# zju3dv/LoG

Hardware: NVIDIA H100
Metric: gaussians_per_s_fwd_bwd (higher is better)
Workload: dtype f32

## Files before the change

include/log_b200_raster.h:

```cpp
#ifndef LOG_B200_RASTER_H
#define LOG_B200_RASTER_H

#include <stdint.h>

#ifdef __cplusplus
extern "C" {
#endif

#define LGR_ABI_VERSION 23
#define LGR_TILE 16

#define LGR_FILTER_ADD 0
#define LGR_FILTER_MAX 1
#define LGR_FILTER_NONE 2

#define LGR_E_BADARG (-1)
#define LGR_E_CAPACITY (-2)
#define LGR_E_UNSUPPORTED (-3)

typedef struct lgr_view {
  int32_t image_height, image_width;
  float tanfovx, tanfovy;
  float scale_modifier;
  int32_t sh_degree;
  int32_t sh_coeffs;
  int32_t filter_mode;
  int32_t want_aux;
  int32_t tile_row_begin, tile_row_end;
  int32_t num_owners;
  int32_t raw_params;
  int32_t* band_ids_d;
  int32_t* band_blk_d;
  int32_t* band_count_d;
  int32_t* band_rows_d;
  float* band_dsplat_d;
  int32_t* tile_rank_d;
  const int64_t* gather_index_d;
  const int32_t* pid_map_d;
  int32_t* contrib_id_d;
  uint32_t* contrib_entry_d;
  int32_t* contrib_count_d;
  const int32_t* last_contrib_d;
  const int32_t* region_count_d;
  int64_t region_cap;
  int32_t num_regions;
  int32_t num_channels;
  int32_t log_depth;
  float* splat_ext_d;
  const float* cov3D_precomp_d;
  float* dcov3D_d;
  const float* viewmatrix_d;
  const float* projmatrix_d;
  const float* campos_d;
  const float* bg_d;
} lgr_view;

#define LGR_SPLAT_FLOATS 12
#define LGR_GRAD_FLOATS 12
#define LGR_TILE_SCRATCH_INTS 33
#define LGR_CONTRIB_MAX_LIST (1 << 24)
#define LGR_META_INTS 8

int lgr_abi_version(void);

int lgr_compute_radius(int64_t n, const float* means3D_d, const float* scales_d, const float* rotations_d,
                       const float* projmatrix_d, const float* viewmatrix_d, float focal_x, float focal_y,
                       float tan_fovx, float tan_fovy, float* radii_d, void* stream);

int lgr_mark_visible(int64_t n, const float* means3D_d, const float* viewmatrix_d, uint8_t* visible_d, void* stream);

int lgr_forward_project(const lgr_view* view, int64_t n, const float* means3D_d, const float* opacities_d,
                        const float* scales_d, const float* rotations_d, const float* colors_precomp_d,
                        const float* shs_d, float* splat_d, int32_t* radii_d, uint8_t* clamped_d,
                        int32_t* tile_start_d, int32_t* tile_cursor_d, int32_t* meta_d, void* stream);

int lgr_forward_render(const lgr_view* view, int64_t n, int64_t num_instances, int32_t max_tile_len,
                       int32_t num_long_tiles, const float* splat_d, const int32_t* radii_d, const int32_t* tile_start_d,
                       int32_t* tile_cursor_d, uint32_t* inst_key_d, uint32_t* inst_val_d, uint32_t* inst_tmp_d,
                       int32_t* sorted_ids_d, float* image_d, float* final_T_d, int32_t* n_contrib_d,
                       int32_t* point_id_pixel_d, float* point_weight_pixel_d, float* point_weight_d,
                       int32_t* point_count_d, void* stream);
int32_t lgr_sort_smem_capacity(void);

int lgr_forward_render_device_sized(const lgr_view* view, int64_t n, int64_t instance_capacity, int32_t* meta_d,
                                    const float* splat_d, const int32_t* radii_d, int32_t* tile_start_d,
                                    int32_t* tile_cursor_d, uint32_t* inst_key_d, uint32_t* inst_val_d,
                                    int32_t* sorted_ids_d, float* image_d, float* final_T_d, int32_t* n_contrib_d,
                                    int32_t* point_id_pixel_d, float* point_weight_pixel_d, float* point_weight_d,
                                    int32_t* point_count_d, void* stream);

int lgr_backward(const lgr_view* view, int64_t n, int64_t num_instances, const float* means3D_d,
                 const float* opacities_d, const float* scales_d, const float* rotations_d,
                 const float* colors_precomp_d, const float* shs_d, const float* splat_d, const int32_t* radii_d,
                 const uint8_t* clamped_d, const int32_t* tile_start_d, const int32_t* sorted_ids_d,
                 const float* image_d, const float* dL_dimage_d, float* dsplat_d,
                 float* dmeans3D_d, float* dmeans2D_d, float* dopacities_d, float* dscales_d, float* drotations_d,
                 float* dcolors_d, float* dshs_d, float* grad_rows_d, void* const* peer_stage_d, int32_t my_rank,
                 int64_t num_rows, void* stream);

#define LGR_STAGE_HEADER_FLOATS 64
#define LGR_ROW_FLOATS 20
#define LGR_OWNER_CHUNK(n, r) ((((n) + (r) - 1) / (r) + 255) / 256 * 256)
int lgr_grad_scatter_add(int64_t num_rows, const float* rows_d, int64_t lo, int64_t hi, float* shard_d, void* stream);
int lgr_grad_scatter_add_staged(const float* stage_d, int32_t num_sources, int64_t owner_chunk, int64_t lo, int64_t hi,
                                float* shard_d, void* stream);

typedef struct lgr_shard_layout {
  int32_t num_ranks, my_rank;
  int64_t cap;
  int64_t off_count, off_splat, off_radii, off_gid, off_dsplat, off_weight, off_pcount;
} lgr_shard_layout;
#define LGR_SHARD_MAX_RANKS 32
#define LGR_SHARD_SEND_INTS(n_local, r) (2 * (int64_t)(r) * ((((n_local) > 0 ? (n_local) : 1) + 255) / 256) + (r))

int lgr_shard_send(const lgr_view* view, const lgr_shard_layout* layout, int64_t n_local, int64_t gid_base,
                   const float* splat_d, const int32_t* radii_d, int32_t* send_scratch_d, void* const* peer_base_d,
                   void* stream);

int lgr_shard_recv_bin(const lgr_view* view, const lgr_shard_layout* layout, float* exchange_d, float* dsplat_d,
                       int32_t* tile_start_d, int32_t* tile_cursor_d, int32_t* meta_d, void* stream);

int lgr_blend_backward(const lgr_view* view, int64_t n, int64_t num_instances, const float* splat_d,
                       const int32_t* tile_start_d, const int32_t* sorted_ids_d, const float* image_d,
                       const float* dL_dimage_d, float* dsplat_d, void* stream);

int lgr_shard_return_rows(const lgr_shard_layout* layout, const float* exchange_d, int64_t total_rows, const void* rows_d,
                          int32_t row_floats, int64_t dst_offset_floats, void* const* peer_base_d, void* stream);

int lgr_shard_gather(const lgr_view* view, const lgr_shard_layout* layout, int64_t n_local, const float* splat_d,
                     const int32_t* radii_d, const int32_t* send_scratch_d, const float* exchange_d,
                     float* dsplat_local_d, float* point_weight_d, int32_t* point_count_d, void* stream);

int lgr_shard_recv_bin_aux(const lgr_view* view, const lgr_shard_layout* layout, float* exchange_d, float* dsplat_d,
                           int32_t* tile_start_d, int32_t* tile_cursor_d, int32_t* meta_d, float* point_weight_rows_d,
                           int32_t* point_count_rows_d, void* stream);
int lgr_shard_return_packed(const lgr_shard_layout* layout, const float* exchange_d, const float* dsplat_rows_d,
                            const float* point_weight_rows_d, const int32_t* point_count_rows_d, void* const* peer_base_d,
                            void* stream);
int lgr_shard_gather_packed(const lgr_view* view, const lgr_shard_layout* layout, int64_t n_local, const float* splat_d,
                            const int32_t* radii_d, const int32_t* send_scratch_d, const float* exchange_d,
                            float* dsplat_local_d, float* point_weight_d, int32_t* point_count_d, void* stream);

typedef struct lgr_tree {
  int64_t num_points, num_nodes;
  int32_t max_child, max_level;
  const int32_t* node_index_d;
  const int32_t* tree_d;
} lgr_tree;
#define LGR_TREE_SCRATCH_INTS(p, s) (8 + 2 * (int64_t)(p) + (int64_t)(s) + 2 * (((int64_t)(s) + 255) / 256) + 2 + ((int64_t)(s) + 3) / 4)
int lgr_tree_traverse(const lgr_tree* tree, const float* xyz_d, const float* scaling_raw_d, const float* rotation_raw_d,
                      const float* projmatrix_d, const float* viewmatrix_d, float focal_x, float focal_y, float tan_fovx,
                      float tan_fovy, const int64_t* root_index_d, int64_t num_roots, float min_resolution_pixel,
                      int32_t max_depth, int32_t* scratch_d, int64_t* index_out_d, int64_t* count_out_d, void* stream);

typedef struct lgr_prepare {
  int64_t num_points, num_roots;
  const float* xyz_d;
  const float* full_proj_d;
  float bound_lo, bound_hi;
  const int32_t* root_index_d;
  const int32_t* node_index_d;
  const int8_t* depth_d;
  int32_t opt_all_levels, current_depth;
  uint8_t* flag_d;
  int64_t* in_range_d;
  int64_t* roots_d;
  int64_t* index_all_d, *leaf_d, *node_d;
  int64_t* result_d;
  int32_t* scratch_d;
} lgr_prepare;
// ... 106 lines not shown
```

log_b200/_capi.py:

```python
import ctypes
import os

from .build import LIB_PATH

_i32, _i64, _f32, _vp = ctypes.c_int32, ctypes.c_int64, ctypes.c_float, ctypes.c_void_p

LGR_FILTER_ADD, LGR_FILTER_MAX, LGR_FILTER_NONE = 0, 1, 2
LGR_SPLAT_FLOATS = 12
LGR_GRAD_FLOATS = 12
LGR_META_INTS = 8
LGR_TILE_SCRATCH_INTS = 33
LGR_ABI_VERSION = 23
LGR_CONTRIB_MAX_LIST = 1 << 24
LGR_STAGE_HEADER_FLOATS = 64
LGR_ROW_FLOATS = 20

EXPORTS = ('lgr_abi_version', 'lgr_sort_smem_capacity', 'lgr_compute_radius', 'lgr_forward_project',
           'lgr_forward_render', 'lgr_forward_render_device_sized', 'lgr_backward', 'lgr_grad_scatter_add', 'lgr_grad_scatter_add_staged', 'lgr_point_compact', 'lgr_sparse_adam', 'lgr_profile_enable', 'lgr_profile_collect',
           'lgr_profile_kernel_name', 'lgr_shard_send', 'lgr_shard_recv_bin', 'lgr_blend_backward', 'lgr_shard_return_rows',
           'lgr_shard_gather', 'lgr_shard_recv_bin_aux', 'lgr_shard_return_packed', 'lgr_shard_gather_packed', 'lgr_tree_traverse', 'lgr_mark_visible',
           'lgr_ssim_forward', 'lgr_ssim_backward', 'lgr_depth_loss_forward', 'lgr_depth_loss_backward', 'lgr_depth_vis',
           'lgr_counter_update', 'lgr_log_step', 'lgr_prepare_cull', 'lgr_prepare_select')
LGR_SHARD_MAX_RANKS = 32
LGR_PROFILE_KERNELS = 12


class LgrView(ctypes.Structure):
    _fields_ = [('image_height', _i32), ('image_width', _i32), ('tanfovx', _f32), ('tanfovy', _f32),
                ('scale_modifier', _f32), ('sh_degree', _i32), ('sh_coeffs', _i32), ('filter_mode', _i32),
                ('want_aux', _i32), ('tile_row_begin', _i32), ('tile_row_end', _i32),
                ('num_owners', _i32), ('raw_params', _i32), ('band_ids_d', _vp), ('band_blk_d', _vp), ('band_count_d', _vp), ('band_rows_d', _vp), ('band_dsplat_d', _vp), ('tile_rank_d', _vp), ('gather_index_d', _vp), ('pid_map_d', _vp), ('contrib_id_d', _vp), ('contrib_entry_d', _vp), ('contrib_count_d', _vp), ('last_contrib_d', _vp),
                ('region_count_d', _vp), ('region_cap', _i64), ('num_regions', _i32), ('num_channels', _i32), ('log_depth', _i32), ('splat_ext_d', _vp), ('cov3D_precomp_d', _vp), ('dcov3D_d', _vp),
                ('viewmatrix_d', _vp), ('projmatrix_d', _vp), ('campos_d', _vp), ('bg_d', _vp)]


class LgrShardLayout(ctypes.Structure):
    _fields_ = [('num_ranks', _i32), ('my_rank', _i32), ('cap', _i64), ('off_count', _i64), ('off_splat', _i64),
                ('off_radii', _i64), ('off_gid', _i64), ('off_dsplat', _i64), ('off_weight', _i64), ('off_pcount', _i64)]


class LgrTree(ctypes.Structure):
    _fields_ = [('num_points', _i64), ('num_nodes', _i64), ('max_child', _i32), ('max_level', _i32),
                ('node_index_d', _vp), ('tree_d', _vp)]


def tree_scratch_ints(num_points, slots):
    return 8 + 2 * num_points + slots + 2 * ((slots + 255) // 256) + 2 + (slots + 3) // 4


class LgrPrepare(ctypes.Structure):
    _fields_ = [('num_points', _i64), ('num_roots', _i64), ('xyz_d', _vp), ('full_proj_d', _vp), ('bound_lo', _f32),
                ('bound_hi', _f32), ('root_index_d', _vp), ('node_index_d', _vp), ('depth_d', _vp), ('opt_all_levels', _i32),
                ('current_depth', _i32), ('flag_d', _vp), ('in_range_d', _vp), ('roots_d', _vp), ('index_all_d', _vp),
                ('leaf_d', _vp), ('node_d', _vp), ('result_d', _vp), ('scratch_d', _vp)]


LGR_PREPARE_RESULTS = 8
(LGR_PREPARE_IN_RANGE, LGR_PREPARE_ROOTS, LGR_PREPARE_WALK, LGR_PREPARE_LEAVES, LGR_PREPARE_NODES, LGR_PREPARE_STATUS,
 LGR_PREPARE_INSTANCES, LGR_PREPARE_OVERFLOW) = range(8)
LGR_PREPARE_ROOT_ORDER = 1


def prepare_scratch_ints(num_points, slots):
    return 2 * num_points + 2 * ((num_points + 255) // 256) + 2 + (num_points + 3) // 4 + tree_scratch_ints(num_points, slots)


LGR_SSIM_WINDOW = 11
LGR_SSIM_TILE = 32


def ssim_scratch_doubles(b, c, h, w):
    return b * c * ((h - LGR_SSIM_WINDOW + LGR_SSIM_TILE) // LGR_SSIM_TILE) * ((w - LGR_SSIM_WINDOW + LGR_SSIM_TILE) // LGR_SSIM_TILE)


def ssim_map_floats(b, c, h, w):
    return 3 * b * c * (h - LGR_SSIM_WINDOW + 1) * (w - LGR_SSIM_WINDOW + 1)


LGR_DEPTH_PATCHES = 64
LGR_DEPTH_PATCH = 64
LGR_DEPTH_STAT_DOUBLES_PER_PATCH = 8
LGR_DEPTH_STAT_DOUBLES = LGR_DEPTH_STAT_DOUBLES_PER_PATCH * LGR_DEPTH_PATCHES + 8
LGR_DEPTH_GRAD_SCRATCH_FLOATS = LGR_DEPTH_PATCHES * LGR_DEPTH_PATCH * LGR_DEPTH_PATCH
LGR_DEPTH_VIS_GRID = 264
LGR_DEPTH_VIS_SCRATCH_FLOATS = 2 * LGR_DEPTH_VIS_GRID


def shard_send_ints(n_local, r):
    return 2 * r * ((max(n_local, 1) + 255) // 256) + r


class LgrCounter(ctypes.Structure):
    _fields_ = [('create_steps_d', _vp), ('visible_count_d', _vp), ('weights_max_d', _vp), ('weights_sum_d', _vp),
                ('radii_max_d', _vp), ('area_sum_d', _vp), ('grad_sum_d', _vp), ('radii_max_max_d', _vp)]


LGR_STEP_MAX_KEYS = 8


class LgrStepKey(ctypes.Structure):
    _fields_ = [('param_d', _vp), ('exp_avg_d', _vp), ('exp_avg_sq_d', _vp), ('max_exp_avg_sq_d', _vp), ('grad_d', _vp),
                ('row_floats', _i32), ('prefix', _i32), ('neg_step_size', _f32), ('bc2_sqrt', _f32), ('clamp', _i32)]


class LgrStep(ctypes.Structure):
    _fields_ = [('keys', LgrStepKey * LGR_STEP_MAX_KEYS), ('num_keys', _i32), ('row_floats', _i32), ('beta1', _f32),
                ('beta2', _f32), ('one_minus_beta1', _f32), ('one_minus_beta2', _f32), ('eps', _f32),
                ('radius3d_min_d', _vp), ('radius3d_max_d', _vp)]


class LgrError(RuntimeError):
    pass


_lib = None


def bind(lib):
    lib.lgr_abi_version.restype = ctypes.c_int
    lib.lgr_sort_smem_capacity.restype = _i32
    lib.lgr_mark_visible.restype = ctypes.c_int
    lib.lgr_mark_visible.argtypes = [_i64, _vp, _vp, _vp, _vp]
    lib.lgr_compute_radius.restype = ctypes.c_int
    lib.lgr_compute_radius.argtypes = [_i64, _vp, _vp, _vp, _vp, _vp, _f32, _f32, _f32, _f32, _vp, _vp]
    lib.lgr_forward_project.restype = ctypes.c_int
    lib.lgr_forward_project.argtypes = [ctypes.POINTER(LgrView), _i64] + [_vp] * 13
    lib.lgr_forward_render.restype = ctypes.c_int
    lib.lgr_forward_render.argtypes = [ctypes.POINTER(LgrView), _i64, _i64, _i32, _i32] + [_vp] * 16
    lib.lgr_forward_render_device_sized.restype = ctypes.c_int
    lib.lgr_forward_render_device_sized.argtypes = [ctypes.POINTER(LgrView), _i64, _i64] + [_vp] * 16
    lib.lgr_sparse_adam.restype = ctypes.c_int
    lib.lgr_sparse_adam.argtypes = [_i64, _i32, _vp, _vp, _vp, _vp, _vp, _vp, _i64, ctypes.c_double, ctypes.c_double,
                                    ctypes.c_double, ctypes.c_double, _vp]
    lib.lgr_point_compact.restype = ctypes.c_int
    lib.lgr_point_compact.argtypes = [_i64, _vp, _vp, _vp, _vp, _vp, _vp]
    lib.lgr_backward.restype = ctypes.c_int
    lib.lgr_backward.argtypes = [ctypes.POINTER(LgrView), _i64, _i64] + [_vp] * 23 + [_i32, _i64, _vp]
    lib.lgr_grad_scatter_add_staged.restype = ctypes.c_int
    lib.lgr_grad_scatter_add_staged.argtypes = [_vp, _i32, _i64, _i64, _i64, _vp, _vp]
    lib.lgr_grad_scatter_add.restype = ctypes.c_int
    lib.lgr_grad_scatter_add.argtypes = [_i64, _vp, _i64, _i64, _vp, _vp]
    lay = ctypes.POINTER(LgrShardLayout)
    lib.lgr_shard_send.restype = ctypes.c_int
    lib.lgr_shard_send.argtypes = [ctypes.POINTER(LgrView), lay, _i64, _i64, _vp, _vp, _vp, _vp, _vp]
    lib.lgr_shard_recv_bin.restype = ctypes.c_int
    lib.lgr_shard_recv_bin.argtypes = [ctypes.POINTER(LgrView), lay, _vp, _vp, _vp, _vp, _vp, _vp]
    lib.lgr_blend_backward.restype = ctypes.c_int
    lib.lgr_blend_backward.argtypes = [ctypes.POINTER(LgrView), _i64, _i64, _vp, _vp, _vp, _vp, _vp, _vp, _vp]
    lib.lgr_shard_return_rows.restype = ctypes.c_int
    lib.lgr_shard_return_rows.argtypes = [lay, _vp, _i64, _vp, _i32, _i64, _vp, _vp]
    lib.lgr_shard_gather.restype = ctypes.c_int
    lib.lgr_shard_gather.argtypes = [ctypes.POINTER(LgrView), lay, _i64, _vp, _vp, _vp, _vp, _vp, _vp, _vp, _vp]
    lib.lgr_shard_recv_bin_aux.restype = ctypes.c_int
    lib.lgr_shard_recv_bin_aux.argtypes = [ctypes.POINTER(LgrView), lay, _vp, _vp, _vp, _vp, _vp, _vp, _vp, _vp]
    lib.lgr_shard_return_packed.restype = ctypes.c_int
    lib.lgr_shard_return_packed.argtypes = [lay, _vp, _vp, _vp, _vp, _vp, _vp]
    lib.lgr_shard_gather_packed.restype = ctypes.c_int
    lib.lgr_shard_gather_packed.argtypes = [ctypes.POINTER(LgrView), lay, _i64, _vp, _vp, _vp, _vp, _vp, _vp, _vp, _vp]
    lib.lgr_tree_traverse.restype = ctypes.c_int
    lib.lgr_tree_traverse.argtypes = [ctypes.POINTER(LgrTree), _vp, _vp, _vp, _vp, _vp, _f32, _f32, _f32, _f32, _vp, _i64, _f32,
                                      _i32, _vp, _vp, _vp, _vp]
    lib.lgr_prepare_cull.restype = ctypes.c_int
    lib.lgr_prepare_cull.argtypes = [ctypes.POINTER(LgrPrepare), _vp]
    lib.lgr_prepare_select.restype = ctypes.c_int
    lib.lgr_prepare_select.argtypes = [ctypes.POINTER(LgrPrepare), ctypes.POINTER(LgrTree), _vp, _vp, _vp, _vp, _f32, _f32, _f32, _f32,
                                       _f32, _i32, _vp, _vp, _vp]
    lib.lgr_ssim_forward.restype = ctypes.c_int
    lib.lgr_ssim_forward.argtypes = [_i32, _i32, _i32, _i32, _vp, _vp, _vp, _vp, _vp, _vp, _vp, _vp]
    lib.lgr_ssim_backward.restype = ctypes.c_int
    lib.lgr_ssim_backward.argtypes = [_i32, _i32, _i32, _i32, _vp, _vp, _vp, _vp, _vp, _vp, _vp, _vp]
    lib.lgr_depth_loss_forward.restype = ctypes.c_int
    lib.lgr_depth_loss_forward.argtypes = [_i32, _i32, _i32, _i32] + [_vp] * 11
    lib.lgr_depth_loss_backward.restype = ctypes.c_int
    lib.lgr_depth_loss_backward.argtypes = [_i32, _i32, _i32, _i32] + [_vp] * 13
    lib.lgr_depth_vis.restype = ctypes.c_int
    lib.lgr_depth_vis.argtypes = [_i32, _i32] + [_vp] * 7
    lib.lgr_counter_update.restype = ctypes.c_int
    lib.lgr_counter_update.argtypes = [ctypes.POINTER(LgrCounter), _i64, _i64] + [_vp] * 6 + [_i64, _vp, _vp, _i32, _i32,
                                                                                              _vp, _vp]
    lib.lgr_log_step.restype = ctypes.c_int
    lib.lgr_log_step.argtypes = [ctypes.POINTER(LgrStep), _i64, _i64, _vp, _vp, _vp, _vp]
    lib.lgr_profile_enable.restype = ctypes.c_int
    lib.lgr_profile_enable.argtypes = [ctypes.c_int]
    lib.lgr_profile_collect.restype = ctypes.c_int
    lib.lgr_profile_collect.argtypes = [_vp, _vp, _i32]
    lib.lgr_profile_kernel_name.restype = ctypes.c_char_p
    lib.lgr_profile_kernel_name.argtypes = [ctypes.c_int]
    return lib


def load():
    global _lib
    if _lib is not None:
        return _lib
    if not os.path.exists(LIB_PATH):
        raise LgrError(f'{LIB_PATH} not found: run `python -m log_b200.build` (or __graft_entry__.build()). '
                       'log_b200 has no CPU fallback.')
    lib = bind(ctypes.CDLL(LIB_PATH))
    if lib.lgr_abi_version() != LGR_ABI_VERSION:
        raise LgrError('liblog_b200_raster.so ABI version mismatch: rebuild with `python -m log_b200.build --force`')
    _lib = lib
    return lib


def current_stream(device=None):
    import torch
    return ctypes.c_void_p(torch.cuda.current_stream(device).cuda_stream)


def require_cuda(t, name):
    if not t.is_cuda:
        raise LgrError(f'{name} is on {t.device}: log_b200 rasterises on CUDA only (no CPU fallback)')

# ... 25 lines not shown
```

log_b200/csrc/lgr_bin.cu:

```cuda
#include "lgr_common.cuh"
#include "lgr_prof.cuh"

namespace lgr {

constexpr int SCAN_THREADS = 1024;
constexpr int SORT_CAP_SMALL_FWD = 4096;

__global__ void __launch_bounds__(SCAN_THREADS)
tile_scan_kernel(int ntiles, int32_t* __restrict__ tile_start ,
                 int32_t* __restrict__ cursor ,
                 int32_t* __restrict__ meta, int small_cap, int ranked) {
  __shared__ int warp_sum[SCAN_THREADS / 32];
  __shared__ int carry_s, maxl_s, nbig_s;
  const int tid = threadIdx.x, lane = tid & 31, wid = tid >> 5;
  if (tid == 0) { carry_s = 0; maxl_s = 0; nbig_s = 0; }
  __syncthreads();
  int local_max = 0;
  for (int base = 0; base < ntiles; base += SCAN_THREADS) {
    const int i = base + tid;
    const int c = (i < ntiles) ? cursor[i * CSTRIDE] + cursor[i * CSTRIDE + 1] : 0;
    local_max = max(local_max, c);
    int x = c;
#pragma unroll
    for (int o = 1; o < 32; o <<= 1) { const int y = __shfl_up_sync(0xffffffffu, x, o); if (lane >= o) x += y; }
    if (lane == 31) warp_sum[wid] = x;
    __syncthreads();
    if (wid == 0) {
      int w = warp_sum[lane];
#pragma unroll
      for (int o = 1; o < 32; o <<= 1) { const int y = __shfl_up_sync(0xffffffffu, w, o); if (lane >= o) w += y; }
      warp_sum[lane] = w;
    }
    __syncthreads();
    const int carry = carry_s;
    const int excl = carry + (wid ? warp_sum[wid - 1] : 0) + x - c;
    if (i < ntiles) {
      tile_start[i] = excl; cursor[i * CSTRIDE + ranked] = 0;
      if (c > small_cap) cursor[CSTRIDE * ntiles + atomicAdd(&nbig_s, 1)] = i;
    }
    __syncthreads();
    if (tid == SCAN_THREADS - 1) carry_s = carry + warp_sum[31];
    __syncthreads();
  }
#pragma unroll
  for (int o = 16; o > 0; o >>= 1) local_max = max(local_max, __shfl_xor_sync(0xffffffffu, local_max, o));
  if (lane == 0) atomicMax(&maxl_s, local_max);
  __syncthreads();
  if (tid == 0) { tile_start[ntiles] = carry_s; meta[0] = carry_s; meta[1] = maxl_s; meta[5] = nbig_s; }
}

constexpr int SCATTER_THREADS = 256;

__global__ void __launch_bounds__(SCATTER_THREADS)
bin_scatter_kernel(View v, int64_t n, const float* __restrict__ splat, const int32_t* __restrict__ radii,
                   const int32_t* __restrict__ tile_start, int32_t* __restrict__ cursor, uint32_t* __restrict__ inst_key,
                   uint32_t* __restrict__ inst_val, int64_t capacity ) {
  __shared__ int64_t s_first[LGR_SHARD_MAX_RANKS + 1];
  const int64_t total = v.region_count ? region_setup(v, s_first) : n;
  for (int64_t base = (int64_t)blockIdx.x * SCATTER_THREADS; base < total; base += (int64_t)gridDim.x * SCATTER_THREADS) {
  int64_t i = base + threadIdx.x;
  bool live = i < total;
  if (live && v.region_count) i = region_row(v, s_first, i);
  if (live && v.num_owners > 0) {
    const int b = (int)(i / 256), sl = (int)(i % 256);
    if (sl >= v.band_blk[b]) live = false;
    else {
      const int id = v.band_ids[i];
      v.band_rows[v.band_blk[v.band_blocks + b] + sl] = id;
      if (v.band_dsplat) {
        float4* z = reinterpret_cast<float4*>(v.band_dsplat + (int64_t)id * LGR_GRAD_FLOATS);
        z[0] = z[1] = z[2] = make_float4(0.f, 0.f, 0.f, 0.f);
      }
      i = id;
    }
  }
  int rad = 0;
  float4 r0 = make_float4(0.f, 0.f, 0.f, 0.f), r1 = r0;
  float depth = 0.f;
  int4 rk = make_int4(-1, -1, -1, -1);
  if (live) {
    rad = radii[i];
    r0 = ldg4(splat + i * LGR_SPLAT_FLOATS);
    r1 = ldg4(splat + i * LGR_SPLAT_FLOATS + 4);
    depth = __ldg(splat + i * LGR_SPLAT_FLOATS + 11);
    if (v.tile_rank) rk = __ldg(reinterpret_cast<const int4*>(v.tile_rank + 4 * i));
    live = rad > 0;
  }
  if (live && v.num_owners == 0 && v.band_dsplat) {
    float4* z = reinterpret_cast<float4*>(v.band_dsplat + i * LGR_GRAD_FLOATS);
    z[0] = z[1] = z[2] = make_float4(0.f, 0.f, 0.f, 0.f);
  }
  int x0 = 0, y0 = 0, x1 = 0, y1 = 0;
  uint32_t key = 0;
  if (live) {
    live = r1.z > 0.f;
    if (live) {
      key = __float_as_uint(depth);
      tile_rect_tight(r0.x, r0.y, rad, r1.z, r1.w, v.gx, v.gy, v.row0, v.row1, x0, y0, x1, y1);
    }
  }
  const int w = x1 - x0, cnt = live ? w * (y1 - y0) : 0;
  if (cnt > 0 && cnt <= 4) {
    int t[4], slot[4];
#pragma unroll
    for (int k = 0; k < 4; k++) {
      const int ty = y0 + k / max(w, 1), tx = x0 + k % max(w, 1);
      t[k] = k < cnt ? (ty - v.row0) * v.gx + tx : -1;
    }
    if (v.tile_rank) {
      slot[0] = rk.x; slot[1] = rk.y; slot[2] = rk.z; slot[3] = rk.w;
    } else {
#pragma unroll
      for (int k = 0; k < 4; k++) slot[k] = t[k] >= 0 ? atomicAdd(cursor + t[k] * CSTRIDE, 1) : 0;
    }
#pragma unroll
    for (int k = 0; k < 4; k++)
      if (t[k] >= 0) {
        const int pos = __ldg(tile_start + t[k]) + slot[k];
        if (pos < capacity) { inst_key[pos] = key; inst_val[pos] = (uint32_t)i; }
      }
  }
  const int lane = threadIdx.x & 31, big = v.tile_rank ? 1 : 0;
  unsigned todo = __ballot_sync(0xffffffffu, cnt > 4);
  while (todo) {
    const int src = __ffs(todo) - 1;
    todo &= todo - 1;
    const int bx0 = __shfl_sync(0xffffffffu, x0, src), by0 = __shfl_sync(0xffffffffu, y0, src);
    const int bw = __shfl_sync(0xffffffffu, w, src), bcnt = __shfl_sync(0xffffffffu, cnt, src);
    const uint32_t bkey = __shfl_sync(0xffffffffu, key, src);
    const uint32_t bid = (uint32_t)__shfl_sync(0xffffffffu, (int)i, src);
    for (int k = lane; k < bcnt; k += 32) {
      const int t = (by0 + k / bw - v.row0) * v.gx + bx0 + k % bw;
      const int pos = tile_start[t] + (big ? cursor[t * CSTRIDE] : 0) + atomicAdd(cursor + t * CSTRIDE + big, 1);
      if (pos < capacity) { inst_key[pos] = bkey; inst_val[pos] = bid; }
    }
  }
  }
}

constexpr int SORT_THREADS = 256;
constexpr int SORT_WARPS = SORT_THREADS / 32;
constexpr int RADIX_BITS = 8;
constexpr int RADIX = 1 << RADIX_BITS;
constexpr int SORT_CAP_SMALL = SORT_CAP_SMALL_FWD;
constexpr int SORT_CAP_LARGE = 13312;

__device__ __forceinline__ bool radix_pass(const uint32_t* __restrict__ kin, const uint32_t* __restrict__ vin,
                                           uint32_t* __restrict__ kout, uint32_t* __restrict__ vout, int len, int shift,
                                           bool on_val, int* __restrict__ whist) {
  const int tid = threadIdx.x, lane = tid & 31, wid = tid >> 5;
  const int seg = ((len + SORT_WARPS * 32 - 1) / (SORT_WARPS * 32)) * 32;
  const int beg = min(len, wid * seg), end = min(len, beg + seg);
  for (int j = tid; j < SORT_WARPS * RADIX; j += SORT_THREADS) whist[j] = 0;
  __syncthreads();
  int* myh = whist + wid * RADIX;
  for (int i = beg + lane; i < end; i += 32) {
    const uint32_t d = ((on_val ? vin[i] : kin[i]) >> shift) & (RADIX - 1);
    atomicAdd(myh + d, 1);
  }
  __syncthreads();
  {
    const int d = tid;
    int tot = 0;
#pragma unroll
    for (int w = 0; w < SORT_WARPS; w++) tot += whist[w * RADIX + d];
    int x = tot;
#pragma unroll
    for (int o = 1; o < 32; o <<= 1) { const int y = __shfl_up_sync(0xffffffffu, x, o); if (lane >= o) x += y; }
    __shared__ int wsum[SORT_WARPS];
    if (lane == 31) wsum[wid] = x;
    __syncthreads();
    int base = x - tot;
#pragma unroll
    for (int w = 0; w < SORT_WARPS; w++) if (w < wid) base += wsum[w];
#pragma unroll
    for (int w = 0; w < SORT_WARPS; w++) { const int c = whist[w * RADIX + d]; whist[w * RADIX + d] = base; base += c; }
    if (__syncthreads_or(tot == len)) return true;
  }
  for (int i0 = beg; i0 < end; i0 += 32) {
    const int i = i0 + lane;
    const bool ok = i < end;
    uint32_t k = 0, val = 0;
    if (ok) { k = kin[i]; val = vin[i]; }
    const uint32_t d = ok ? (((on_val ? val : k) >> shift) & (RADIX - 1)) : (RADIX + lane);
    const uint32_t peers = __match_any_sync(0xffffffffu, d);
    const int rank = __popc(peers & ((1u << lane) - 1u));
    int base = 0;
    if (ok) base = myh[d];
    __syncwarp();
    if (ok && rank == 0) myh[d] = base + __popc(peers);
    __syncwarp();
    if (ok) { kout[base + rank] = k; vout[base + rank] = val; }
  }
  __syncthreads();
  return false;
}

__device__ __forceinline__ void sort_tile(uint32_t* kA, uint32_t* vA, uint32_t* kB, uint32_t* vB, int len, int id_bits,
                                          int* whist) {
  uint32_t *ki = kA, *vi = vA, *ko = kB, *vo = vB;
  auto run = [&](int shift, bool on_val) {
    const bool ident = radix_pass(ki, vi, ko, vo, len, shift, on_val, whist);
    if (!ident) { uint32_t* t = ki; ki = ko; ko = t; t = vi; vi = vo; vo = t; }
  };
  for (int s = 0; s < 32; s += RADIX_BITS) run(s, false);
  int my_tie = 0;
  for (int i = threadIdx.x + 1; i < len; i += SORT_THREADS) if (ki[i] == ki[i - 1]) my_tie = 1;
  if (__syncthreads_or(my_tie)) {
    for (int s = 0; s < id_bits; s += RADIX_BITS) run(s, true);
    for (int s = 0; s < 32; s += RADIX_BITS) run(s, false);
  }
  if (ki != kA) {
    for (int i = threadIdx.x; i < len; i += SORT_THREADS) { kA[i] = ki[i]; vA[i] = vi[i]; }
    __syncthreads();
  }
}

#ifndef LGR_ON_LSD_FALLBACK
#define LGR_ON_LSD_FALLBACK()
#endif
constexpr int MSD_SMALL = 96;
constexpr int MSD_STACK = 512;

struct MsdShared {
  int hist[RADIX];
  int bstart[RADIX + 1];
  alignas(16) int wsum[SORT_WARPS];
  unsigned long long wmin[SORT_WARPS], wmax[SORT_WARPS];
  int stack_beg[MSD_STACK], stack_len[MSD_STACK];
  int top, shift, overflow;
};

__device__ __forceinline__ unsigned long long composite(uint32_t k, uint32_t v) { return ((unsigned long long)k << 32) | v; }

__device__ __forceinline__ bool sort_tile_msd(uint32_t* kA, uint32_t* vA, uint32_t* kB, uint32_t* vB, int len, MsdShared& sh) {
  const int tid = threadIdx.x, lane = tid & 31, wid = tid >> 5;
  if (tid == 0) { sh.stack_beg[0] = 0; sh.stack_len[0] = len; sh.top = 1; sh.overflow = 0; }
  __syncthreads();
  while (true) {
    const int top = sh.top;
    if (top == 0 || sh.overflow) break;
    const int beg = sh.stack_beg[top - 1], n = sh.stack_len[top - 1];
    __syncthreads();
    if (tid == 0) sh.top = top - 1;
    unsigned long long mn = ~0ull, mx = 0ull;
    for (int i = tid; i < n; i += SORT_THREADS) {
      const unsigned long long c = composite(kA[beg + i], vA[beg + i]);
      mn = min(mn, c); mx = max(mx, c);
    }
#pragma unroll
    for (int o = 16; o > 0; o >>= 1) {
      mn = min(mn, __shfl_xor_sync(0xffffffffu, mn, o));
      mx = max(mx, __shfl_xor_sync(0xffffffffu, mx, o));
    }
    if (lane == 0) { sh.wmin[wid] = mn; sh.wmax[wid] = mx; }
    sh.hist[tid] = 0;
    __syncthreads();
    if (tid == 0) {
      unsigned long long a = sh.wmin[0], b = sh.wmax[0];
#pragma unroll
      for (int w = 1; w < SORT_WARPS; w++) { a = min(a, sh.wmin[w]); b = max(b, sh.wmax[w]); }
      const int hb = 63 - __clzll((long long)(a ^ b));
      sh.shift = max(0, hb - (RADIX_BITS - 1));
    }
    __syncthreads();
    const int shift = sh.shift;
    for (int i = tid; i < n; i += SORT_THREADS)
      atomicAdd(&sh.hist[(int)((composite(kA[beg + i], vA[beg + i]) >> shift) & (RADIX - 1))], 1);
    __syncthreads();
    {
      const int c = sh.hist[tid];
      int x = c;
#pragma unroll
      for (int o = 1; o < 32; o <<= 1) { const int y = __shfl_up_sync(0xffffffffu, x, o); if (lane >= o) x += y; }
      if (lane == 31) sh.wsum[wid] = x;
      __syncthreads();
      int base = x - c;
#pragma unroll
      for (int w = 0; w < SORT_WARPS; w++) if (w < wid) base += sh.wsum[w];
      sh.bstart[tid] = base;
      sh.hist[tid] = base;
      if (tid == RADIX - 1) sh.bstart[RADIX] = base + c;
    }
    __syncthreads();
    for (int i = tid; i < n; i += SORT_THREADS) {
      const uint32_t k = kA[beg + i], v = vA[beg + i];
      const int slot = atomicAdd(&sh.hist[(int)((composite(k, v) >> shift) & (RADIX - 1))], 1);
      kB[beg + slot] = k; vB[beg + slot] = v;
    }
    __syncthreads();
    for (int i = tid; i < n; i += SORT_THREADS) {
      const uint32_t k = kB[beg + i], v = vB[beg + i];
      const int d = (int)((composite(k, v) >> shift) & (RADIX - 1));
      const int b0 = sh.bstart[d], bn = sh.bstart[d + 1] - b0;
      int dst = i;
      if (bn <= MSD_SMALL) {
        const uint32_t* kb = kB + beg + b0;
        const uint32_t* vb = vB + beg + b0;
        int rank = 0, eq = 0;
#pragma unroll 8
        for (int j = 0; j < bn; j++) {
          const uint32_t kj = kb[j];
          rank += (kj < k) ? 1 : 0;
          eq += (kj == k) ? 1 : 0;
        }
        if (eq > 1)
          for (int j = 0; j < bn; j++) rank += (kb[j] == k && vb[j] < v) ? 1 : 0;
        dst = b0 + rank;
      }
      kA[beg + dst] = k; vA[beg + dst] = v;
    }
    {
      const int b0 = sh.bstart[tid], bn = sh.bstart[tid + 1] - b0;
      if (bn > MSD_SMALL) {
        const int slot = atomicAdd(&sh.top, 1);
        if (slot < MSD_STACK) { sh.stack_beg[slot] = beg + b0; sh.stack_len[slot] = bn; }
// ... 50 lines not shown
  if ((int64_t)meta[0] <= capacity) return;
  for (int i = blockIdx.x * 256 + threadIdx.x; i <= ntiles; i += gridDim.x * 256) tile_start[i] = 0;
  if (blockIdx.x == 0 && threadIdx.x == 0) atomicOr(meta + 6, 1);
}


int sort_smem_capacity() { return SORT_CAP_LARGE; }

constexpr int PC_THREADS = 1024;

__global__ void __launch_bounds__(PC_THREADS)
pc_block_count_kernel(int64_t n, const int32_t* __restrict__ count, int32_t* __restrict__ blk) {
  const int64_t i = (int64_t)blockIdx.x * PC_THREADS + threadIdx.x;
  const int c = __syncthreads_count(i < n && count[i] > 0);
  if (threadIdx.x == 0) blk[blockIdx.x] = c;
}

__global__ void __launch_bounds__(1024)
pc_scan_kernel(int nb, int32_t* __restrict__ blk , int32_t* __restrict__ num_out) {
  __shared__ int warp_sum[32];
  __shared__ int carry_s;
  const int tid = threadIdx.x, lane = tid & 31, wid = tid >> 5;
  if (tid == 0) carry_s = 0;
  __syncthreads();
  for (int base = 0; base < nb; base += 1024) {
    const int b = base + tid;
    const int c = b < nb ? blk[b] : 0;
    int x = c;
#pragma unroll
    for (int o = 1; o < 32; o <<= 1) { const int y = __shfl_up_sync(0xffffffffu, x, o); if (lane >= o) x += y; }
    if (lane == 31) warp_sum[wid] = x;
    __syncthreads();
    if (wid == 0) {
      int w = warp_sum[lane];
#pragma unroll
      for (int o = 1; o < 32; o <<= 1) { const int y = __shfl_up_sync(0xffffffffu, w, o); if (lane >= o) w += y; }
      warp_sum[lane] = w;
    }
    __syncthreads();
    const int carry = carry_s;
    if (b < nb) blk[nb + b] = carry + (wid ? warp_sum[wid - 1] : 0) + x - c;
    __syncthreads();
    if (tid == 1023) carry_s = carry + warp_sum[31];
    __syncthreads();
  }
  if (tid == 0) { blk[2 * nb] = carry_s; *num_out = carry_s; }
}

__global__ void __launch_bounds__(PC_THREADS)
pc_compact_kernel(int64_t n, const int32_t* __restrict__ count, const int32_t* __restrict__ blk, int nb,
                  int32_t* __restrict__ ids_out, int32_t* __restrict__ counts_out) {
  __shared__ int wsum[PC_THREADS / 32];
  const int64_t i = (int64_t)blockIdx.x * PC_THREADS + threadIdx.x;
  const int lane = threadIdx.x & 31, wid = threadIdx.x >> 5;
  const int c = i < n ? count[i] : 0;
  const unsigned bal = __ballot_sync(0xffffffffu, c > 0);
  if (lane == 0) wsum[wid] = __popc(bal);
  __syncthreads();
  int base = blk[nb + blockIdx.x];
  for (int w = 0; w < wid; w++) base += wsum[w];
  if (c > 0) {
    const int pos = base + __popc(bal & ((1u << lane) - 1u));
    ids_out[pos] = (int32_t)i;
    counts_out[pos] = c;
  }
}

int launch_point_compact(int64_t n, const int32_t* count, int32_t* blk, int32_t* ids_out, int32_t* counts_out, int32_t* num_out,
                         cudaStream_t st) {
  const int nb = (int)((n + PC_THREADS - 1) / PC_THREADS);
  if (nb == 0) {
    cudaError_t e = cudaMemsetAsync(num_out, 0, sizeof(int32_t), st);
    return e == cudaSuccess ? 0 : (int)e;
  }
  pc_block_count_kernel<<<nb, PC_THREADS, 0, st>>>(n, count, blk);
  LGR_CHECK_LAUNCH();
  pc_scan_kernel<<<1, 1024, 0, st>>>(nb, blk, num_out);
  LGR_CHECK_LAUNCH();
  pc_compact_kernel<<<nb, PC_THREADS, 0, st>>>(n, count, blk, nb, ids_out, counts_out);
  LGR_CHECK_LAUNCH();
  return 0;
}

int launch_tile_scan(int ntiles, int32_t* tile_start, int32_t* cursor, int32_t* meta, bool ranked, cudaStream_t st) {
  ProfScope ps(K_TILE_SCAN, st);
  tile_scan_kernel<<<1, SCAN_THREADS, 0, st>>>(ntiles, tile_start, cursor, meta, SORT_CAP_SMALL_FWD, ranked ? 1 : 0);
  LGR_CHECK_LAUNCH();
  return 0;
}

constexpr int LONG_SORT_GRID = 132;

int launch_bin_and_sort(const View& v, int64_t n, int64_t num_inst, int max_len, int num_long, const float* splat,
                        const int32_t* radii, int32_t* tile_start, int32_t* cursor, uint32_t* inst_key,
                        uint32_t* inst_val, uint32_t* inst_tmp, int32_t* sorted_ids, int32_t* meta_dev, cudaStream_t st) {
  if (n == 0) return 0;
  if (meta_dev) {
    const int nt = v.gx * (v.row1 - v.row0);
    clamp_lists_kernel<<<(nt + 256) / 256, 256, 0, st>>>(nt, num_inst, tile_start, meta_dev);
    LGR_CHECK_LAUNCH();
  }
  if (num_inst == 0 && v.num_owners == 0 && v.band_dsplat == nullptr) return 0;
  const int ntiles = v.gx * (v.row1 - v.row0);
  unsigned blocks = (unsigned)((n + SCATTER_THREADS - 1) / SCATTER_THREADS);
  if (v.region_count && blocks > (unsigned)LGR_REGION_GRID) blocks = (unsigned)LGR_REGION_GRID;
  {
    ProfScope ps(K_BIN_SCATTER, st);
    bin_scatter_kernel<<<blocks, SCATTER_THREADS, 0, st>>>(v, n, splat, radii, tile_start, cursor, inst_key, inst_val,
                                                           meta_dev ? num_inst : (int64_t)0x7fffffffffffffffLL);
  }
  LGR_CHECK_LAUNCH();
  if (num_inst == 0) return 0;
  int id_bits = 8;
  while (id_bits < 32 && (n - 1) >> id_bits) id_bits += 8;
  {
    cudaError_t e = cudaFuncSetAttribute(tile_sort_kernel<0>, cudaFuncAttributeMaxDynamicSharedMemorySize, 16 * SORT_CAP_LARGE);
    if (e != cudaSuccess) return (int)e;
  }
  if (meta_dev) {
    ProfScope ps(K_TILE_SORT, st, 2);
    tile_sort_kernel<0><<<ntiles, SORT_THREADS, 16 * SORT_CAP_SMALL, st>>>(nullptr, tile_start, inst_key, inst_val, inst_tmp, sorted_ids, 0, SORT_CAP_SMALL, id_bits, nullptr, nullptr);
    LGR_CHECK_LAUNCH();
    const int32_t* long_list = cursor + CSTRIDE * ntiles;
    tile_sort_kernel<0><<<LONG_SORT_GRID, SORT_THREADS, 16 * SORT_CAP_LARGE, st>>>(long_list, tile_start, inst_key, inst_val, inst_tmp, sorted_ids, SORT_CAP_SMALL, SORT_CAP_LARGE, id_bits, meta_dev + 5, meta_dev + 6);
    LGR_CHECK_LAUNCH();
    return 0;
  }
  ProfScope ps(K_TILE_SORT, st, 1 + (num_long > 0) + (max_len > SORT_CAP_LARGE));
  const int cap_main = max(256, min(max_len, SORT_CAP_SMALL));
  tile_sort_kernel<0><<<ntiles, SORT_THREADS, 16 * cap_main, st>>>(nullptr, tile_start, inst_key, inst_val, inst_tmp, sorted_ids, 0, cap_main, id_bits, nullptr, nullptr);
  LGR_CHECK_LAUNCH();
  if (num_long > 0) {
    const int32_t* long_list = cursor + CSTRIDE * ntiles;
    const int cap = min(max_len, SORT_CAP_LARGE);
    tile_sort_kernel<0><<<num_long, SORT_THREADS, 16 * cap, st>>>(long_list, tile_start, inst_key, inst_val, inst_tmp, sorted_ids, SORT_CAP_SMALL, cap, id_bits, nullptr, nullptr);
    LGR_CHECK_LAUNCH();
    if (max_len > SORT_CAP_LARGE) {
      if (!inst_tmp) return LGR_E_CAPACITY;
      tile_sort_kernel<1><<<num_long, SORT_THREADS, 0, st>>>(long_list, tile_start, inst_key, inst_val, inst_tmp, sorted_ids, SORT_CAP_LARGE, 0, id_bits, nullptr, nullptr);
      LGR_CHECK_LAUNCH();
    }
  }
  return 0;
}

}
```

log_b200/csrc/lgr_capi.cu:

```cuda
#include "lgr_common.cuh"
#include "lgr_prof.cuh"
#include <math.h>

namespace lgr {
int launch_mark_visible(int64_t, const float*, const float*, uint8_t*, cudaStream_t);
int launch_compute_radius(int64_t, const float*, const float*, const float*, const float*, const float*, float, float,
                          float, float, float*, cudaStream_t);
int launch_project_fwd(const View&, Colour, bool, int64_t, const float*, const float*, const float*, const float*,
                       const float*, const float*, float*, int32_t*, uint8_t*, int32_t*, int32_t*, cudaStream_t);
int launch_project_bwd(const View&, Colour, bool, bool, int64_t, const float*, const float*, const float*, const float*,
                       const float*, const int32_t*, const uint8_t*, const float*, float*, float*, float*, float*, float*,
                       float*, float*, float*, void* const*, int, cudaStream_t);
int launch_grad_scatter_add(int64_t, const float*, int64_t, int64_t, float*, cudaStream_t);
int launch_grad_scatter_add_staged(const float*, int, int64_t, int64_t, int64_t, float*, cudaStream_t);
int launch_band_scan(const View&, cudaStream_t);
int launch_tile_scan(int, int32_t*, int32_t*, int32_t*, bool, cudaStream_t);
int launch_bin_and_sort(const View&, int64_t, int64_t, int, int, const float*, const int32_t*, int32_t*, int32_t*,
                        uint32_t*, uint32_t*, uint32_t*, int32_t*, int32_t*, cudaStream_t);
int sort_smem_capacity();
int launch_blend_fwd(const View&, const int32_t*, const int32_t*, const float*, float*, float*, int32_t*, int32_t*,
                     float*, float*, int32_t*, cudaStream_t);
int launch_sparse_adam(int64_t, int, const int64_t*, const float*, float*, float*, float*, float*, float, float, float, float,
                       float, float, float, cudaStream_t);
int launch_counter_update(const lgr_counter&, int64_t, int64_t, const int64_t*, const int64_t*, const int32_t*, const float*,
// ... 40 lines not shown
                            v->gather_index_d))
    return false;
  const int lists = (v->contrib_id_d != nullptr) + (v->contrib_entry_d != nullptr) + (v->contrib_count_d != nullptr);
  if (lists != 0 && lists != 3) return false;
  if (v->num_channels != 0 && v->num_channels != 3 && v->num_channels != 6) return false;
  if (v->num_channels == 6 && !v->splat_ext_d) return false;
  if (v->log_depth != 0 && (v->log_depth != 1 || v->num_channels != 6)) return false;
  return true;
}

static int six_channels_check(const lgr_view* v) {
  if (v->num_channels != 6) return 0;
  if (v->num_owners > 0 || v->region_count_d || v->pid_map_d) return LGR_E_UNSUPPORTED;
  if (!v->log_depth && (v->raw_params || v->gather_index_d)) return LGR_E_UNSUPPORTED;
  return 0;
}

static int colour_source(const lgr_view* v, int64_t n, const float* colors_precomp_d, const float* shs_d, Colour* c) {
  const bool six_precomp = v->num_channels == 6 && !v->log_depth;
  if (six_precomp && shs_d) return LGR_E_UNSUPPORTED;
  const bool log_sh = v->raw_params && colors_precomp_d && shs_d;
  if (!log_sh && (colors_precomp_d != nullptr) == (shs_d != nullptr) && n > 0) return LGR_E_BADARG;
  *c = log_sh ? Colour::LOG_SH : shs_d ? Colour::SH : six_precomp ? Colour::RGB6 : Colour::RGB;
  return 0;
}

extern "C" {

int lgr_abi_version(void) { return LGR_ABI_VERSION; }

int32_t lgr_sort_smem_capacity(void) { return sort_smem_capacity(); }

int lgr_compute_radius(int64_t n, const float* means3D_d, const float* scales_d, const float* rotations_d,
                       const float* projmatrix_d, const float* viewmatrix_d, float focal_x, float focal_y,
                       float tan_fovx, float tan_fovy, float* radii_d, void* stream) {
  if (n < 0 || (n > 0 && (!means3D_d || !scales_d || !rotations_d || !radii_d)) || !projmatrix_d || !viewmatrix_d)
    return LGR_E_BADARG;
  return launch_compute_radius(n, means3D_d, scales_d, rotations_d, projmatrix_d, viewmatrix_d, focal_x, focal_y,
                               tan_fovx, tan_fovy, radii_d, (cudaStream_t)stream);
}

int lgr_mark_visible(int64_t n, const float* means3D_d, const float* viewmatrix_d, uint8_t* visible_d, void* stream) {
  if (n < 0 || !viewmatrix_d || (n > 0 && (!means3D_d || !visible_d))) return LGR_E_BADARG;
  return launch_mark_visible(n, means3D_d, viewmatrix_d, visible_d, (cudaStream_t)stream);
}

int lgr_forward_project(const lgr_view* view, int64_t n, const float* means3D_d, const float* opacities_d,
                        const float* scales_d, const float* rotations_d, const float* colors_precomp_d,
                        const float* shs_d, float* splat_d, int32_t* radii_d, uint8_t* clamped_d,
                        int32_t* tile_start_d, int32_t* tile_cursor_d, int32_t* meta_d, void* stream) {
  if (!view_ok(view) || n < 0 || !tile_start_d || !tile_cursor_d || !meta_d) return LGR_E_BADARG;
  if (const int rc6 = six_channels_check(view)) return rc6;
  Colour c;
  if (const int rc = colour_source(view, n, colors_precomp_d, shs_d, &c)) return rc;
  if (view->raw_params && c == Colour::SH) return LGR_E_UNSUPPORTED;
  if (c == Colour::LOG_SH) {
    if (!view->campos_d) return LGR_E_BADARG;
    if (view->sh_degree < 0 || view->sh_degree > 3) return LGR_E_UNSUPPORTED;
    if (view->sh_coeffs < (view->sh_degree + 1) * (view->sh_degree + 1) - 1) return LGR_E_BADARG;
    if (view->num_owners > 0) return LGR_E_UNSUPPORTED;
  } else if (c == Colour::SH) {
    if (!view->campos_d || !clamped_d) return LGR_E_BADARG;
    if (view->sh_degree < 0 || view->sh_degree > 3) return LGR_E_UNSUPPORTED;
    if (view->sh_coeffs < (view->sh_degree + 1) * (view->sh_degree + 1)) return LGR_E_BADARG;
  }
  const bool cov3d = view->cov3D_precomp_d != nullptr;
  if (n > 0 && (!means3D_d || !opacities_d || (!cov3d && (!scales_d || !rotations_d)) || !splat_d || !radii_d)) return LGR_E_BADARG;
  if (cov3d && (view->raw_params || view->num_owners > 0)) return LGR_E_UNSUPPORTED;
  if (n > 0x7fffffffLL) return LGR_E_UNSUPPORTED;
  cudaStream_t st = (cudaStream_t)stream;
  const View v = make_view(view, n);
  const int ntiles = v.gx * (v.row1 - v.row0);
  if (v.num_owners > 0 && shs_d) return LGR_E_UNSUPPORTED;
  if (c == Colour::LOG_SH && view->sh_degree == 0) c = Colour::RGB;
  cudaError_t e = cudaMemsetAsync(tile_cursor_d, 0, sizeof(int32_t) * (size_t)ntiles * CSTRIDE, st);
  if (e != cudaSuccess) return (int)e;
  e = cudaMemsetAsync(meta_d, 0, sizeof(int32_t) * LGR_META_INTS, st);
  if (e != cudaSuccess) return (int)e;
  int rc = launch_project_fwd(v, c, cov3d, n, means3D_d, opacities_d, scales_d, rotations_d, colors_precomp_d, shs_d, splat_d,
                              radii_d, clamped_d, tile_cursor_d, meta_d, st);
  if (rc) return rc;
  rc = launch_band_scan(v, st);
  if (rc) return rc;
  return launch_tile_scan(ntiles, tile_start_d, tile_cursor_d, meta_d, view->tile_rank_d != nullptr, st);
}

int lgr_forward_render(const lgr_view* view, int64_t n, int64_t num_instances, int32_t max_tile_len,
                       int32_t num_long_tiles, const float* splat_d, const int32_t* radii_d, const int32_t* tile_start_d,
                       int32_t* tile_cursor_d, uint32_t* inst_key_d, uint32_t* inst_val_d, uint32_t* inst_tmp_d,
                       int32_t* sorted_ids_d, float* image_d, float* final_T_d, int32_t* n_contrib_d,
                       int32_t* point_id_pixel_d, float* point_weight_pixel_d, float* point_weight_d,
                       int32_t* point_count_d, void* stream) {
  if (!view_ok(view) || n < 0 || num_instances < 0 || num_long_tiles < 0 || !tile_start_d || !tile_cursor_d || !image_d || !final_T_d ||
      !n_contrib_d)
    return LGR_E_BADARG;
  if (num_instances > 0 && (!inst_key_d || !inst_val_d || !sorted_ids_d || !splat_d || !radii_d)) return LGR_E_BADARG;
  if (const int rc6 = six_channels_check(view)) return rc6;
  if (view->want_aux && (!point_id_pixel_d || !point_weight_pixel_d || (n > 0 && !point_weight_d))) return LGR_E_BADARG;
  if (num_instances > 0x7fffffffLL) return LGR_E_UNSUPPORTED;
  if (view->contrib_id_d && max_tile_len > LGR_CONTRIB_MAX_LIST) return LGR_E_UNSUPPORTED;
  cudaStream_t st = (cudaStream_t)stream;
  const View v = make_view(view, n);
  int rc = launch_bin_and_sort(v, n, num_instances, max_tile_len, num_long_tiles, splat_d, radii_d, const_cast<int32_t*>(tile_start_d), tile_cursor_d,
                               inst_key_d, inst_val_d, inst_tmp_d, sorted_ids_d, nullptr, st);
  if (rc) return rc;
  return launch_blend_fwd(v, tile_start_d, sorted_ids_d, splat_d, image_d, final_T_d, n_contrib_d, point_id_pixel_d,
                          point_weight_pixel_d, point_weight_d, view->want_aux ? point_count_d : nullptr, st);
}

int lgr_forward_render_device_sized(const lgr_view* view, int64_t n, int64_t instance_capacity, int32_t* meta_d,
                                    const float* splat_d, const int32_t* radii_d, int32_t* tile_start_d,
                                    int32_t* tile_cursor_d, uint32_t* inst_key_d, uint32_t* inst_val_d,
                                    int32_t* sorted_ids_d, float* image_d, float* final_T_d, int32_t* n_contrib_d,
                                    int32_t* point_id_pixel_d, float* point_weight_pixel_d, float* point_weight_d,
                                    int32_t* point_count_d, void* stream) {
  if (!view_ok(view) || n < 0 || instance_capacity <= 0 || !meta_d || !tile_start_d || !tile_cursor_d || !image_d || !final_T_d ||
      !n_contrib_d || !inst_key_d || !inst_val_d || !sorted_ids_d)
    return LGR_E_BADARG;
  if (n > 0 && (!splat_d || !radii_d)) return LGR_E_BADARG;
  if (const int rc6 = six_channels_check(view)) return rc6;
  if (view->want_aux && (!point_id_pixel_d || !point_weight_pixel_d || (n > 0 && !point_weight_d))) return LGR_E_BADARG;
  if (instance_capacity > 0x7fffffffLL) return LGR_E_UNSUPPORTED;
  cudaStream_t st = (cudaStream_t)stream;
  const View v = make_view(view, n);
  int rc = launch_bin_and_sort(v, n, instance_capacity, 0, 0, splat_d, radii_d, tile_start_d, tile_cursor_d, inst_key_d, inst_val_d,
                               nullptr, sorted_ids_d, meta_d, st);
  if (rc) return rc;
  return launch_blend_fwd(v, tile_start_d, sorted_ids_d, splat_d, image_d, final_T_d, n_contrib_d, point_id_pixel_d,
                          point_weight_pixel_d, point_weight_d, view->want_aux ? point_count_d : nullptr, st);
}

int lgr_backward(const lgr_view* view, int64_t n, int64_t num_instances, const float* means3D_d,
                 const float* opacities_d, const float* scales_d, const float* rotations_d,
                 const float* colors_precomp_d, const float* shs_d, const float* splat_d, const int32_t* radii_d,
                 const uint8_t* clamped_d, const int32_t* tile_start_d, const int32_t* sorted_ids_d,
                 const float* image_d, const float* dL_dimage_d, float* dsplat_d,
                 float* dmeans3D_d, float* dmeans2D_d, float* dopacities_d, float* dscales_d, float* drotations_d,
                 float* dcolors_d, float* dshs_d, float* grad_rows_d, void* const* peer_stage_d, int32_t my_rank,
                 int64_t num_rows, void* stream) {
  if (!view_ok(view) || n < 0 || !tile_start_d || !image_d || !dL_dimage_d) return LGR_E_BADARG;
  if (const int rc6 = six_channels_check(view)) return rc6;
  const bool rows_mode = grad_rows_d || peer_stage_d;
  if (view->num_channels == 6 && rows_mode) return LGR_E_UNSUPPORTED;
  Colour c;
  if (const int rc = colour_source(view, n, colors_precomp_d, shs_d, &c)) return rc;
  if (n == 0) return 0;
  if (c == Colour::LOG_SH && (!dshs_d || !view->campos_d || view->num_owners > 0)) return LGR_E_BADARG;
  const bool cov3d = view->cov3D_precomp_d != nullptr;
  if (!means3D_d || (!cov3d && (!scales_d || !rotations_d)) || !splat_d || !radii_d || !dsplat_d) return LGR_E_BADARG;
  if (cov3d && (!view->dcov3D_d || view->raw_params || view->num_owners > 0 || grad_rows_d || peer_stage_d)) return LGR_E_BADARG;
  if (view->raw_params && (!opacities_d || c == Colour::SH)) return LGR_E_BADARG;
  if (rows_mode) {
    if (view->num_owners <= 0 || c == Colour::SH) return LGR_E_BADARG;
    if (peer_stage_d && (my_rank < 0 || my_rank >= view->num_owners)) return LGR_E_BADARG;
    if (num_rows < 0 || num_rows > n) return LGR_E_BADARG;
  } else {
    if (view->num_owners > 0) return LGR_E_BADARG;
    if (!dmeans3D_d || !dmeans2D_d || !dopacities_d || (!cov3d && (!dscales_d || !drotations_d))) return LGR_E_BADARG;
    if (c == Colour::SH ? (!dshs_d || !clamped_d || !view->campos_d) : !dcolors_d) return LGR_E_BADARG;
  }
  if (num_instances > 0 && !sorted_ids_d) return LGR_E_BADARG;
  cudaStream_t st = (cudaStream_t)stream;
  const View v = make_view(view, n);
  int rc = 0;
  if (num_instances > 0) rc = launch_blend_bwd(v, tile_start_d, sorted_ids_d, splat_d, image_d, dL_dimage_d, dsplat_d, st);
  if (rc) return rc;
  return launch_project_bwd(v, c, cov3d, rows_mode, rows_mode ? num_rows : n, means3D_d, opacities_d, scales_d, rotations_d, shs_d, radii_d, clamped_d, dsplat_d,
                            dmeans3D_d, dmeans2D_d, dopacities_d, dscales_d, drotations_d, dcolors_d, dshs_d, grad_rows_d, peer_stage_d, my_rank, st);
}

int lgr_sparse_adam(int64_t rows, int32_t row_floats, const int64_t* index_d, const float* grad_d, float* param_d,
                    float* exp_avg_d, float* exp_avg_sq_d, float* max_exp_avg_sq_d, int64_t step, double lr, double beta1,
                    double beta2, double eps, void* stream) {
  if (rows < 0 || row_floats <= 0 || step < 1) return LGR_E_BADARG;
  if (rows > 0 && (!index_d || !grad_d || !param_d || !exp_avg_d || !exp_avg_sq_d)) return LGR_E_BADARG;
  const double bc1 = 1.0 - pow(beta1, (double)step), bc2 = 1.0 - pow(beta2, (double)step);
  const double step_size = lr / bc1;
  return launch_sparse_adam(rows, row_floats, index_d, grad_d, param_d, exp_avg_d, exp_avg_sq_d, max_exp_avg_sq_d,
                            (float)beta1, (float)beta2, (float)(1.0 - beta1), (float)(1.0 - beta2), (float)sqrt(bc2),
                            (float)(-step_size), (float)eps, (cudaStream_t)stream);
}

int lgr_counter_update(const lgr_counter* counter, int64_t num_leaf, int64_t num_node, const int64_t* index_leaf_d,
                       const int64_t* index_node_d, const int32_t* radii_d, const float* point_weight_d, const float* grad_d,
                       const int64_t* grad_strides, int64_t num_points, const void* point_id_d, const void* point_count_d,
                       int32_t id_bytes, int32_t count_bytes, uint8_t* flag_vis_d, void* stream) {
  if (!counter || num_leaf < 0 || num_node < 0 || num_points < 0 || !grad_strides) return LGR_E_BADARG;
  if ((id_bytes != 4 && id_bytes != 8) || (count_bytes != 4 && count_bytes != 8)) return LGR_E_BADARG;
  if ((num_leaf > 0 && !index_leaf_d) || (num_node > 0 && !index_node_d)) return LGR_E_BADARG;
  const lgr_counter& c = *counter;
  if (!c.create_steps_d || !c.visible_count_d || !c.weights_max_d || !c.weights_sum_d || !c.radii_max_d || !c.area_sum_d ||
      !c.grad_sum_d || !c.radii_max_max_d)
    return LGR_E_BADARG;
  if (num_leaf + num_node > 0 && (!radii_d || !point_weight_d || !flag_vis_d)) return LGR_E_BADARG;
  if (num_points > 0 && (!point_id_d || !point_count_d || !grad_d || grad_strides[0] < 0 || grad_strides[1] < 0))
    return LGR_E_BADARG;
  return launch_counter_update(c, num_leaf, num_node, index_leaf_d, index_node_d, radii_d, point_weight_d, grad_d,
                               grad_strides, num_points, point_id_d, point_count_d, id_bytes, count_bytes, flag_vis_d,
                               (cudaStream_t)stream);
}

int lgr_log_step(const lgr_step* step, int64_t num_leaf, int64_t num_node, const int64_t* index_leaf_d,
                 const int64_t* index_node_d, const uint8_t* flag_vis_d, void* stream) {
  if (!step || num_leaf < 0 || num_node < 0 || step->num_keys < 1 || step->num_keys > LGR_STEP_MAX_KEYS) return LGR_E_BADARG;
  if ((num_leaf > 0 && !index_leaf_d) || (num_node > 0 && !index_node_d) || (num_leaf + num_node > 0 && !flag_vis_d))
    return LGR_E_BADARG;
  int32_t prefix = 0;
  for (int k = 0; k < step->num_keys; k++) {
    const lgr_step_key& key = step->keys[k];
// ... 71 lines not shown
                               (cudaStream_t)stream);
}

int lgr_depth_vis(int32_t height, int32_t width, const float* pred_d, const int64_t* pred_strides, const float* accmap_d,
                  const int64_t* acc_strides, float* scratch_d, float* vis_d, void* stream) {
  if (height < 1 || width < 1 || !pred_d || !pred_strides || !accmap_d || !acc_strides || !scratch_d || !vis_d)
    return LGR_E_BADARG;
  for (int k = 0; k < 2; k++)
    if (pred_strides[k] < 0 || acc_strides[k] < 0) return LGR_E_BADARG;
  return launch_depth_vis(height, width, pred_d, pred_strides, accmap_d, acc_strides, scratch_d, vis_d, (cudaStream_t)stream);
}

int lgr_point_compact(int64_t n, const int32_t* point_count_d, int32_t* scratch_d, int32_t* ids_out_d,
                      int32_t* counts_out_d, int32_t* num_out_d, void* stream) {
  if (n < 0 || !num_out_d || (n > 0 && (!point_count_d || !scratch_d || !ids_out_d || !counts_out_d))) return LGR_E_BADARG;
  return launch_point_compact(n, point_count_d, scratch_d, ids_out_d, counts_out_d, num_out_d, (cudaStream_t)stream);
}

int lgr_grad_scatter_add_staged(const float* stage_d, int32_t num_sources, int64_t owner_chunk, int64_t lo, int64_t hi,
                                float* shard_d, void* stream) {
  if (!stage_d || !shard_d || num_sources <= 0 || owner_chunk <= 0 || hi < lo) return LGR_E_BADARG;
  return launch_grad_scatter_add_staged(stage_d, num_sources, owner_chunk, lo, hi, shard_d, (cudaStream_t)stream);
}

int lgr_grad_scatter_add(int64_t num_rows, const float* rows_d, int64_t lo, int64_t hi, float* shard_d, void* stream) {
  if (num_rows < 0 || hi < lo || (num_rows > 0 && (!rows_d || !shard_d))) return LGR_E_BADARG;
  return launch_grad_scatter_add(num_rows, rows_d, lo, hi, shard_d, (cudaStream_t)stream);
}

static bool layout_ok(const lgr_shard_layout* l) {
  if (!l || l->num_ranks <= 0 || l->num_ranks > LGR_SHARD_MAX_RANKS || l->my_rank < 0 || l->my_rank >= l->num_ranks) return false;
  if (l->cap <= 0 || l->cap % 256) return false;
  const int64_t offs[7] = {l->off_count, l->off_splat, l->off_radii, l->off_gid, l->off_dsplat, l->off_weight, l->off_pcount};
  for (int k = 0; k < 7; k++) if (offs[k] < 0 || offs[k] % 4) return false;
  return true;
}

static ShardLayout make_layout(const lgr_shard_layout* l) {
  ShardLayout o;
  o.R = l->num_ranks; o.me = l->my_rank; o.cap = l->cap;
  o.off_count = l->off_count; o.off_splat = l->off_splat; o.off_radii = l->off_radii; o.off_gid = l->off_gid;
  o.off_dsplat = l->off_dsplat; o.off_weight = l->off_weight; o.off_pcount = l->off_pcount;
  return o;
}

int lgr_shard_send(const lgr_view* view, const lgr_shard_layout* layout, int64_t n_local, int64_t gid_base,
                   const float* splat_d, const int32_t* radii_d, int32_t* send_scratch_d, void* const* peer_base_d,
                   void* stream) {
  if (!view_ok(view) || !layout_ok(layout) || n_local < 0 || gid_base < 0 || !send_scratch_d || !peer_base_d) return LGR_E_BADARG;
  if (view->num_channels == 6) return LGR_E_UNSUPPORTED;
  if (n_local > layout->cap || (n_local > 0 && (!splat_d || !radii_d))) return LGR_E_BADARG;
  if (view->num_owners != 0 || view->tile_row_begin != 0 || (view->tile_row_end != 0 && view->tile_row_end != (view->image_height + TILE - 1) / TILE))
    return LGR_E_BADARG;
  if (gid_base + n_local > 0x7fffffffLL) return LGR_E_UNSUPPORTED;
  return launch_shard_send(make_view(view, n_local), make_layout(layout), n_local, gid_base, splat_d, radii_d, send_scratch_d,
                           peer_base_d, (cudaStream_t)stream);
}

int lgr_shard_recv_bin(const lgr_view* view, const lgr_shard_layout* layout, float* exchange_d, float* dsplat_d,
                       int32_t* tile_start_d, int32_t* tile_cursor_d, int32_t* meta_d, void* stream) {
  return lgr_shard_recv_bin_aux(view, layout, exchange_d, dsplat_d, tile_start_d, tile_cursor_d, meta_d, nullptr, nullptr, stream);
}

int lgr_shard_recv_bin_aux(const lgr_view* view, const lgr_shard_layout* layout, float* exchange_d, float* dsplat_d,
                           int32_t* tile_start_d, int32_t* tile_cursor_d, int32_t* meta_d, float* point_weight_rows_d,
                           int32_t* point_count_rows_d, void* stream) {
  if (!view_ok(view) || !layout_ok(layout) || !exchange_d || !dsplat_d || !tile_start_d || !tile_cursor_d || !meta_d) return LGR_E_BADARG;
  if (view->num_channels == 6) return LGR_E_UNSUPPORTED;
  if (view->num_owners != 0) return LGR_E_BADARG;
  if (view->region_count_d != reinterpret_cast<const int32_t*>(exchange_d + layout->off_count) || view->region_cap != layout->cap ||
      view->num_regions != layout->num_ranks)
    return LGR_E_BADARG;
  if ((int64_t)layout->num_ranks * layout->cap > 0x7fffffffLL) return LGR_E_UNSUPPORTED;
  cudaStream_t st = (cudaStream_t)stream;
  const View v = make_view(view, (int64_t)layout->num_ranks * layout->cap);
  const int ntiles = v.gx * (v.row1 - v.row0);
  cudaError_t e = cudaMemsetAsync(tile_cursor_d, 0, sizeof(int32_t) * (size_t)(ntiles > 0 ? ntiles : 1) * CSTRIDE, st);
  if (e != cudaSuccess) return (int)e;
  e = cudaMemsetAsync(meta_d, 0, sizeof(int32_t) * LGR_META_INTS, st);
  if (e != cudaSuccess) return (int)e;
  int rc = launch_shard_recv_count(v, make_layout(layout), exchange_d, dsplat_d, tile_cursor_d, meta_d, point_weight_rows_d,
                                   point_count_rows_d, st);
  if (rc) return rc;
  return launch_tile_scan(ntiles, tile_start_d, tile_cursor_d, meta_d, view->tile_rank_d != nullptr, st);
}

int lgr_blend_backward(const lgr_view* view, int64_t n, int64_t num_instances, const float* splat_d,
                       const int32_t* tile_start_d, const int32_t* sorted_ids_d, const float* image_d,
                       const float* dL_dimage_d, float* dsplat_d, void* stream) {
  if (!view_ok(view) || n < 0 || num_instances < 0 || !tile_start_d || !image_d || !dL_dimage_d) return LGR_E_BADARG;
  if (const int rc6 = six_channels_check(view)) return rc6;
  if (num_instances == 0 || n == 0) return 0;
  if (!splat_d || !sorted_ids_d || !dsplat_d) return LGR_E_BADARG;
  return launch_blend_bwd(make_view(view, n), tile_start_d, sorted_ids_d, splat_d, image_d, dL_dimage_d, dsplat_d,
                          (cudaStream_t)stream);
}

int lgr_shard_return_rows(const lgr_shard_layout* layout, const float* exchange_d, int64_t total_rows, const void* rows_d,
                          int32_t row_floats, int64_t dst_offset_floats, void* const* peer_base_d, void* stream) {
  if (!layout_ok(layout) || !exchange_d || !peer_base_d || total_rows < 0 || row_floats <= 0) return LGR_E_BADARG;
  if (dst_offset_floats < 0 || dst_offset_floats % 4 || (total_rows > 0 && !rows_d)) return LGR_E_BADARG;
  return launch_shard_return(make_layout(layout), exchange_d, total_rows, rows_d, row_floats, dst_offset_floats, peer_base_d,
                             (cudaStream_t)stream);
}

int lgr_shard_gather(const lgr_view* view, const lgr_shard_layout* layout, int64_t n_local, const float* splat_d,
                     const int32_t* radii_d, const int32_t* send_scratch_d, const float* exchange_d,
                     float* dsplat_local_d, float* point_weight_d, int32_t* point_count_d, void* stream) {
  if (!view_ok(view) || !layout_ok(layout) || n_local < 0 || n_local > layout->cap) return LGR_E_BADARG;
  if (view->num_channels == 6) return LGR_E_UNSUPPORTED;
  if (n_local == 0) return 0;
  if (!splat_d || !radii_d || !send_scratch_d || !exchange_d || !dsplat_local_d) return LGR_E_BADARG;
  return launch_shard_gather(make_view(view, n_local), make_layout(layout), n_local, splat_d, radii_d, send_scratch_d, exchange_d,
                             dsplat_local_d, point_weight_d, point_count_d, 0, (cudaStream_t)stream);
}

int lgr_shard_gather_packed(const lgr_view* view, const lgr_shard_layout* layout, int64_t n_local, const float* splat_d,
                            const int32_t* radii_d, const int32_t* send_scratch_d, const float* exchange_d,
                            float* dsplat_local_d, float* point_weight_d, int32_t* point_count_d, void* stream) {
  if (!view_ok(view) || !layout_ok(layout) || n_local < 0 || n_local > layout->cap) return LGR_E_BADARG;
  if (view->num_channels == 6) return LGR_E_UNSUPPORTED;
  if (n_local == 0) return 0;
  if (!splat_d || !radii_d || !send_scratch_d || !exchange_d || !dsplat_local_d) return LGR_E_BADARG;
  return launch_shard_gather(make_view(view, n_local), make_layout(layout), n_local, splat_d, radii_d, send_scratch_d, exchange_d,
                             dsplat_local_d, point_weight_d, point_count_d, 1, (cudaStream_t)stream);
}

int lgr_shard_return_packed(const lgr_shard_layout* layout, const float* exchange_d, const float* dsplat_rows_d,
                            const float* point_weight_rows_d, const int32_t* point_count_rows_d, void* const* peer_base_d,
                            void* stream) {
  if (!layout_ok(layout) || !exchange_d || !dsplat_rows_d || !peer_base_d) return LGR_E_BADARG;
  return launch_shard_return_packed(make_layout(layout), exchange_d, dsplat_rows_d, point_weight_rows_d, point_count_rows_d,
                                    peer_base_d, (cudaStream_t)stream);
}

int lgr_tree_traverse(const lgr_tree* tree, const float* xyz_d, const float* scaling_raw_d, const float* rotation_raw_d,
                      const float* projmatrix_d, const float* viewmatrix_d, float focal_x, float focal_y, float tan_fovx,
                      float tan_fovy, const int64_t* root_index_d, int64_t num_roots, float min_resolution_pixel,
                      int32_t max_depth, int32_t* scratch_d, int64_t* index_out_d, int64_t* count_out_d, void* stream) {
  if (!tree || tree->num_points < 0 || tree->num_nodes < 0 || tree->max_child <= 0 || tree->max_level < 0) return LGR_E_BADARG;
  if (num_roots < 0 || num_roots > tree->num_points || max_depth < 0 || !scratch_d || !count_out_d) return LGR_E_BADARG;
  if (!projmatrix_d || !viewmatrix_d) return LGR_E_BADARG;
  if (tree->num_points > 0 && (!tree->node_index_d || !xyz_d || !scaling_raw_d || !rotation_raw_d || !index_out_d)) return LGR_E_BADARG;
  if (tree->num_nodes > 0 && !tree->tree_d) return LGR_E_BADARG;
  if (num_roots > 0 && !root_index_d) return LGR_E_BADARG;
  if (tree->num_points > 0x7fffffffLL || tree->num_nodes * tree->max_child > 0x7fffffffLL) return LGR_E_UNSUPPORTED;
  TreeArgs a;
  a.node_index = tree->node_index_d; a.tree = tree->tree_d; a.C = tree->max_child;
  a.xyz = xyz_d; a.scaling_raw = scaling_raw_d; a.rotation_raw = rotation_raw_d; a.view = viewmatrix_d; a.proj = projmatrix_d;
  a.fx = focal_x; a.fy = focal_y; a.tanfovx = tan_fovx; a.tanfovy = tan_fovy; a.min_px = min_resolution_pixel;
  const int levels = tree->max_level < max_depth ? tree->max_level : max_depth;
  return launch_tree_traverse(a, tree->num_points, tree->num_nodes, root_index_d, num_roots, nullptr, levels, scratch_d, index_out_d,
                              count_out_d, (cudaStream_t)stream);
}

static bool prepare_ok(const lgr_prepare* p) {
  if (!p || p->num_points < 0 || p->num_roots < 0 || p->num_roots > p->num_points || !p->result_d) return false;
  if (p->num_points > 0 && (!p->xyz_d || !p->full_proj_d || !p->flag_d || !p->in_range_d || !p->scratch_d)) return false;
  if (p->num_roots > 0 && !p->root_index_d) return false;
  return true;
}

int lgr_prepare_cull(const lgr_prepare* prep, void* stream) {
  if (!prepare_ok(prep)) return LGR_E_BADARG;
  if (prep->num_points > 0x7fffffffLL) return LGR_E_UNSUPPORTED;
  return launch_prepare_cull(*prep, (cudaStream_t)stream);
}
// ... 53 lines not shown
```

log_b200/csrc/lgr_common.cuh:

```cuda
#pragma once
#include <cuda_runtime.h>
#include <stdint.h>

#include "../../include/log_b200_raster.h"

namespace lgr {

constexpr int TILE = LGR_TILE;
constexpr int TILE_PIX = TILE * TILE;
constexpr float NEAR_Z = 0.2f;
constexpr float ALPHA_MAX = 0.99f;
constexpr float ALPHA_MIN = 1.0f / 255.0f;
constexpr float T_STOP = 1e-4f;
constexpr float FILTER_VAR = 0.3f;
constexpr float CLAMP_FOV = 1.3f;
constexpr int CSTRIDE = 32;
constexpr float LOG2E = 1.4426950408889634f;
constexpr float LN2 = 0.6931471805599453f;

enum class Colour { RGB, SH, LOG_SH, RGB6 };

struct View {
  int H, W, gx, gy;
  int row0, row1;
  float tanfovx, tanfovy, fx, fy, scale_mod;
  int sh_degree, sh_K, filter_mode, want_aux;
  int raw_params;
  int num_owners, owner_chunk;
  int32_t* band_ids;
  int32_t* band_blk;
  int32_t* band_count;
  int32_t* band_rows;
  float* band_dsplat;
  int32_t* tile_rank;
  const int64_t* gather;
  const int32_t* pid_map;
  int32_t* contrib_id;
  uint32_t* contrib_entry;
  int32_t* contrib_count;
  const int32_t* last_contrib;
  const int32_t* region_count;
  int64_t region_cap;
  int regions;
  const float* cov3d;
  float* dcov3d;
  int band_blocks;
  const float* view;
  const float* proj;
  const float* campos;
  const float* bg;
  int num_channels;
  int log_depth;
  float* splat_ext;
};

inline View make_view(const lgr_view* v, int64_t n = 0) {
  View o;
  o.num_owners = v->num_owners; o.band_ids = v->band_ids_d; o.band_blk = v->band_blk_d; o.band_count = v->band_count_d; o.band_rows = v->band_rows_d; o.band_dsplat = v->band_dsplat_d; o.tile_rank = v->tile_rank_d; o.gather = v->gather_index_d; o.pid_map = v->pid_map_d; o.contrib_id = v->contrib_id_d; o.contrib_entry = v->contrib_entry_d; o.contrib_count = v->contrib_count_d; o.last_contrib = v->last_contrib_d;
  o.region_count = v->region_count_d; o.region_cap = v->region_cap; o.regions = v->region_count_d ? v->num_regions : 0;
  o.cov3d = v->cov3D_precomp_d; o.dcov3d = v->dcov3D_d;
  o.owner_chunk = o.num_owners > 0 ? (int)LGR_OWNER_CHUNK(n, (int64_t)o.num_owners) : 256;
  if (o.owner_chunk < 256) o.owner_chunk = 256;
  o.band_blocks = (int)((n + 255) / 256);
  o.H = v->image_height; o.W = v->image_width;
  o.gx = (o.W + TILE - 1) / TILE; o.gy = (o.H + TILE - 1) / TILE;
  o.row0 = v->tile_row_begin; o.row1 = v->tile_row_end;
  if (o.row0 == 0 && o.row1 == 0) o.row1 = o.gy;
  o.tanfovx = v->tanfovx; o.tanfovy = v->tanfovy;
  o.fx = o.W / (2.0f * v->tanfovx); o.fy = o.H / (2.0f * v->tanfovy);
  o.scale_mod = v->scale_modifier;
  o.sh_degree = v->sh_degree; o.sh_K = v->sh_coeffs; o.filter_mode = v->filter_mode; o.want_aux = v->want_aux;
  o.raw_params = v->raw_params;
  o.view = v->viewmatrix_d; o.proj = v->projmatrix_d; o.campos = v->campos_d; o.bg = v->bg_d;
  o.num_channels = v->num_channels == 6 ? 6 : 3; o.splat_ext = v->splat_ext_d; o.log_depth = v->log_depth ? 1 : 0;
  return o;
}

struct ShardLayout {
  int R, me;
  int64_t cap;
  int64_t off_count, off_splat, off_radii, off_gid, off_dsplat, off_weight, off_pcount;
};

struct TreeArgs {
  const int32_t* node_index;
  const int32_t* tree;
  int C;
  const float* xyz;
  const float* scaling_raw;
  const float* rotation_raw;
  const float* view;
  const float* proj;
  float fx, fy, tanfovx, tanfovy, min_px;
};


__device__ __forceinline__ float4 ldg4(const float* p) { return __ldg(reinterpret_cast<const float4*>(p)); }

struct Cov2D {
  float a, b, c;
  float a_raw, c_raw;
  float t[3];
  float T[6];
  bool inx, iny;
};

__device__ __forceinline__ void quat_to_R(const float4 q, float R[9]) {
  const float r = q.x, x = q.y, y = q.z, z = q.w;
  R[0] = 1.f - 2.f * (y * y + z * z); R[1] = 2.f * (x * y - r * z); R[2] = 2.f * (x * z + r * y);
  R[3] = 2.f * (x * y + r * z); R[4] = 1.f - 2.f * (x * x + z * z); R[5] = 2.f * (y * z - r * x);
  R[6] = 2.f * (x * z - r * y); R[7] = 2.f * (y * z + r * x); R[8] = 1.f - 2.f * (x * x + y * y);
}

__device__ __forceinline__ void cov3d(const float s[3], const float R[9], float Sg[9]) {
  float M[9];
#pragma unroll
  for (int i = 0; i < 3; i++)
#pragma unroll
    for (int k = 0; k < 3; k++) M[i * 3 + k] = R[i * 3 + k] * s[k];
#pragma unroll
  for (int i = 0; i < 3; i++)
#pragma unroll
    for (int j = 0; j < 3; j++) Sg[i * 3 + j] = M[i * 3] * M[j * 3] + M[i * 3 + 1] * M[j * 3 + 1] + M[i * 3 + 2] * M[j * 3 + 2];
}

__device__ __forceinline__ void cov2d(const float* __restrict__ V, const float p[3], const float Sg[9], float fx, float fy,
                                      float tanfovx, float tanfovy, int filter_mode, Cov2D& o) {
#pragma unroll
  for (int j = 0; j < 3; j++) o.t[j] = p[0] * V[j] + p[1] * V[4 + j] + p[2] * V[8 + j] + V[12 + j];
  const float limx = CLAMP_FOV * tanfovx, limy = CLAMP_FOV * tanfovy;
  const float itz = 1.0f / o.t[2];
  const float txtz = o.t[0] * itz, tytz = o.t[1] * itz;
  o.inx = (txtz >= -limx) && (txtz <= limx);
  o.iny = (tytz >= -limy) && (tytz <= limy);
  const float txc = fminf(limx, fmaxf(-limx, txtz)) * o.t[2];
  const float tyc = fminf(limy, fmaxf(-limy, tytz)) * o.t[2];
  const float J00 = fx * itz, J02 = -(fx * txc) * itz * itz, J11 = fy * itz, J12 = -(fy * tyc) * itz * itz;
#pragma unroll
  for (int j = 0; j < 3; j++) {
    o.T[j] = J00 * V[j * 4 + 0] + J02 * V[j * 4 + 2];
    o.T[3 + j] = J11 * V[j * 4 + 1] + J12 * V[j * 4 + 2];
// ... 7 lines not shown
  o.b = TS[0] * o.T[3] + TS[1] * o.T[4] + TS[2] * o.T[5];
  o.c_raw = TS[3] * o.T[3] + TS[4] * o.T[4] + TS[5] * o.T[5];
  o.a = o.a_raw; o.c = o.c_raw;
  if (filter_mode == LGR_FILTER_ADD) { o.a += FILTER_VAR; o.c += FILTER_VAR; }
  else if (filter_mode == LGR_FILTER_MAX) { o.a = fmaxf(o.a, FILTER_VAR); o.c = fmaxf(o.c, FILTER_VAR); }
}

__device__ __forceinline__ float act_sigmoid(float x) { return 1.0f / (1.0f + expf(-x)); }
__device__ __forceinline__ float4 act_normalize(float4 q, float& inv_norm) {
  inv_norm = 1.0f / fmaxf(sqrtf(q.x * q.x + q.y * q.y + q.z * q.z + q.w * q.w), 1e-12f);
  return make_float4(q.x * inv_norm, q.y * inv_norm, q.z * inv_norm, q.w * inv_norm);
}

__device__ __forceinline__ float radius_from_cov(float a, float b, float c, float& det) {
  det = a * c - b * b;
  const float mid = 0.5f * (a + c);
  const float root = sqrtf(fmaxf(0.1f, mid * mid - det));
  return 3.0f * sqrtf(fmaxf(mid + root, mid - root));
}

__device__ __forceinline__ bool ndc_inside(const float p[3], const float* __restrict__ P) {
  float hom[4];
#pragma unroll
  for (int k = 0; k < 4; k++) hom[k] = p[0] * P[k] + p[1] * P[4 + k] + p[2] * P[8 + k] + P[12 + k];
  const float pw = 1.0f / (hom[3] + 0.0000001f);
  const float nx = hom[0] * pw, ny = hom[1] * pw;
  return !(nx < -1.3f || nx > 1.3f || ny < -1.3f || ny > 1.3f);
}
__device__ __forceinline__ float projected_radius(const float p[3], const float s[3], const float4 q, const float* __restrict__ V,
                                                  float fx, float fy, float tanfovx, float tanfovy) {
  float R[9], Sg[9];
  quat_to_R(q, R);
  cov3d(s, R, Sg);
  Cov2D cv;
  cov2d(V, p, Sg, fx, fy, tanfovx, tanfovy, LGR_FILTER_MAX, cv);
  float det;
  const float rad = radius_from_cov(cv.a, cv.b, cv.c, det);
  return det != 0.0f ? rad : 0.0f;
}

__device__ __forceinline__ void tile_rect(float px, float py, int rad, int gx, int gy, int& x0, int& y0, int& x1, int& y1) {
  x0 = min(gx, max(0, (int)((px - rad) / TILE)));
  x1 = min(gx, max(0, (int)((px + rad + TILE - 1) / TILE)));
  y0 = min(gy, max(0, (int)((py - rad) / TILE)));
  y1 = min(gy, max(0, (int)((py + rad + TILE - 1) / TILE)));
}

__device__ __forceinline__ void tile_rect_tight(float px, float py, int rad, float hx, float hy, int gx, int gy, int row0,
                                                int row1, int& x0, int& y0, int& x1, int& y1) {
  tile_rect(px, py, rad, gx, gy, x0, y0, x1, y1);
  const int tx0 = (int)ceilf((px - hx - (TILE - 1)) * (1.0f / TILE));
  const int tx1 = (int)floorf((px + hx) * (1.0f / TILE)) + 1;
  const int ty0 = (int)ceilf((py - hy - (TILE - 1)) * (1.0f / TILE));
  const int ty1 = (int)floorf((py + hy) * (1.0f / TILE)) + 1;
  x0 = max(x0, tx0); x1 = min(x1, tx1);
  y0 = max(max(y0, ty0), row0); y1 = min(min(y1, ty1), row1);
  if (x1 < x0) x1 = x0;
  if (y1 < y0) y1 = y0;
}

#ifndef LGR_REGION_GRID
#define LGR_REGION_GRID (132 * 16)
#endif

__device__ __forceinline__ int64_t region_setup(const View& v, int64_t* first) {
  if (threadIdx.x == 0) {
    int64_t acc = 0;
    for (int s = 0; s < v.regions; s++) {
      first[s] = acc;
      const int64_t c = v.region_count[s];
      acc += c < 0 ? 0 : (c > v.region_cap ? v.region_cap : c);
    }
    first[v.regions] = acc;
  }
  __syncthreads();
  return first[v.regions];
}
__device__ __forceinline__ int64_t region_row(const View& v, const int64_t* first, int64_t t) {
  int s = 0;
  while (s + 1 < v.regions && t >= first[s + 1]) s++;
  return (int64_t)s * v.region_cap + (t - first[s]);
}

__device__ __forceinline__ bool count_small_tiles(const View& v, int32_t* __restrict__ tile_count, int64_t row, int x0, int y0, int x1,
                                                  int y1) {
  const int w = x1 - x0, cnt = w * (y1 - y0);
  if (cnt > 4) return true;
  if (v.tile_rank == nullptr) {
    for (int k = 0; k < cnt; k++) atomicAdd(tile_count + ((y0 + k / w - v.row0) * v.gx + x0 + k % w) * CSTRIDE, 1);
    return false;
  }
  int r[4];
#pragma unroll
  for (int k = 0; k < 4; k++) {
    r[k] = -1;
    if (k < cnt) r[k] = atomicAdd(tile_count + ((y0 + k / max(w, 1) - v.row0) * v.gx + x0 + k % max(w, 1)) * CSTRIDE, 1);
  }
  *reinterpret_cast<int4*>(v.tile_rank + 4 * row) = make_int4(r[0], r[1], r[2], r[3]);
  return false;
}

__device__ __forceinline__ void warp_count_big_tiles(const View& v, int32_t* __restrict__ tile_count, bool big, int x0, int y0, int x1,
                                                     int y1) {
  const int lane = threadIdx.x & 31;
  const int slot = v.tile_rank ? 1 : 0;
  unsigned todo = __ballot_sync(0xffffffffu, big);
  while (todo) {
    const int src = __ffs(todo) - 1;
    todo &= todo - 1;
    const int bx0 = __shfl_sync(0xffffffffu, x0, src), by0 = __shfl_sync(0xffffffffu, y0, src);
    const int bx1 = __shfl_sync(0xffffffffu, x1, src), by1 = __shfl_sync(0xffffffffu, y1, src);
    const int w = bx1 - bx0, cnt = w * (by1 - by0);
    for (int k = lane; k < cnt; k += 32) atomicAdd(tile_count + ((by0 + k / w - v.row0) * v.gx + bx0 + k % w) * CSTRIDE + slot, 1);
  }
}

constexpr float SH_C0 = 0.28209479177387814f;
constexpr float SH_C1 = 0.4886025119029199f;
__device__ __constant__ const float SH_C2[5] = {1.0925484305920792f, -1.0925484305920792f, 0.31539156525252005f,
                                                 -1.0925484305920792f, 0.5462742152960396f};
__device__ __constant__ const float SH_C3[7] = {-0.5900435899266435f, 2.890611442640554f, -0.4570457994644658f,
                                                 0.3731763325901154f, -0.4570457994644658f, 1.445305721320277f,
                                                 -0.5900435899266435f};

__device__ __forceinline__ void sh_basis(int deg, float x, float y, float z, float B[16]) {
  B[0] = SH_C0;
  if (deg > 0) {
    B[1] = -SH_C1 * y; B[2] = SH_C1 * z; B[3] = -SH_C1 * x;
    if (deg > 1) {
      const float xx = x * x, yy = y * y, zz = z * z, xy = x * y, yz = y * z, xz = x * z;
      B[4] = SH_C2[0] * xy; B[5] = SH_C2[1] * yz; B[6] = SH_C2[2] * (2.f * zz - xx - yy);
      B[7] = SH_C2[3] * xz; B[8] = SH_C2[4] * (xx - yy);
      if (deg > 2) {
        B[9] = SH_C3[0] * y * (3.f * xx - yy); B[10] = SH_C3[1] * xy * z; B[11] = SH_C3[2] * y * (4.f * zz - xx - yy);
        B[12] = SH_C3[3] * z * (2.f * zz - 3.f * xx - 3.f * yy); B[13] = SH_C3[4] * x * (4.f * zz - xx - yy);
        B[14] = SH_C3[5] * z * (xx - yy); B[15] = SH_C3[6] * x * (xx - 3.f * yy);
      }
    }
  }
}

}

#define LGR_CHECK_LAUNCH()                     \
  do {                                         \
    cudaError_t e__ = cudaGetLastError();      \
    if (e__ != cudaSuccess) return (int)e__;   \
  } while (0)
```

log_b200/csrc/lgr_project.cu:

```cuda
#include "lgr_common.cuh"
#include "lgr_prof.cuh"

namespace lgr {

constexpr int PROJ_THREADS = 256;

__device__ __forceinline__ void load3(const float* __restrict__ p, int64_t i, float o[3]) {
  o[0] = __ldg(p + 3 * i); o[1] = __ldg(p + 3 * i + 1); o[2] = __ldg(p + 3 * i + 2);
}

__device__ __forceinline__ void load_cov3d(const float* cov, int64_t i, float Sg[9]) {
  const float* c6 = cov + 6 * i;
  const float cxx = __ldg(c6), cxy = __ldg(c6 + 1), cxz = __ldg(c6 + 2), cyy = __ldg(c6 + 3), cyz = __ldg(c6 + 4), czz = __ldg(c6 + 5);
  Sg[0] = cxx; Sg[1] = cxy; Sg[2] = cxz; Sg[3] = cxy; Sg[4] = cyy; Sg[5] = cyz; Sg[6] = cxz; Sg[7] = cyz; Sg[8] = czz;
}

__device__ __forceinline__ void sh_dir_basis(const float p[3], const float* cam, int deg, float B[16]) {
  const float d[3] = {p[0] - cam[0], p[1] - cam[1], p[2] - cam[2]};
  const float inv = 1.0f / sqrtf(d[0] * d[0] + d[1] * d[1] + d[2] * d[2]);
  sh_basis(deg, d[0] * inv, d[1] * inv, d[2] * inv, B);
}

__device__ __forceinline__ void sh_accumulate(const float* sh, const float B[16], int first, int nb, float rgb[3]) {
  for (int k = first; k < nb; k++) {
// ... 112 lines not shown
    if (src < 0) work = false;
  }
  if (work) {
    float p[3], Sg[9];
    load3(means, src, p);
    if (COV3D) {
      load_cov3d(v.cov3d, src, Sg);
    } else {
      float s[3], R[9];
      load3(scales, src, s);
      float4 q = ldg4(rots + 4 * src);
      if (v.raw_params) {
        float inv;
#pragma unroll
        for (int k = 0; k < 3; k++) s[k] = expf(s[k]);
        q = act_normalize(q, inv);
      }
#pragma unroll
      for (int k = 0; k < 3; k++) s[k] *= v.scale_mod;
      quat_to_R(q, R);
      cov3d(s, R, Sg);
    }
    Cov2D cv;
    cov2d(sV, p, Sg, v.fx, v.fy, v.tanfovx, v.tanfovy, v.filter_mode, cv);
    float det;
    const float radf = radius_from_cov(cv.a, cv.b, cv.c, det);
    float4 r0 = make_float4(0.f, 0.f, 0.f, 0.f), r1 = r0, r2 = r0, r3 = r0;
    if (cv.t[2] > NEAR_Z && det > 0.0f) {
      float hom[4];
#pragma unroll
      for (int k = 0; k < 4; k++) hom[k] = p[0] * sP[k] + p[1] * sP[4 + k] + p[2] * sP[8 + k] + sP[12 + k];
      const float pw = 1.0f / (hom[3] + 0.0000001f);
      const float px = ((hom[0] * pw + 1.0f) * v.W - 1.0f) * 0.5f;
      const float py = ((hom[1] * pw + 1.0f) * v.H - 1.0f) * 0.5f;
      const int rad = (int)ceilf(radf);
      int x0, y0, x1, y1;
      tile_rect(px, py, rad, v.gx, v.gy, x0, y0, x1, y1);
      if ((x1 - x0) * (y1 - y0) > 0) {
        rad_out = rad;
        stock_tiles = (unsigned long long)((x1 - x0) * (max(0, min(y1, v.row1) - max(y0, v.row0))));
        in_band = stock_tiles > 0;
        const float idet = 1.0f / det;
        const float o = v.raw_params ? act_sigmoid(__ldg(opac + src)) : __ldg(opac + src);
        float hx = 0.f, hy = 0.f;
        bool reach = o * 255.0f >= 1.0f;
        if (reach) {
          const float q = 2.0f * logf(o * 255.0f) * 1.004f + 1e-3f;
          hx = sqrtf(q * cv.a) * 1.001f + 1e-3f;
          hy = sqrtf(q * cv.c) * 1.001f + 1e-3f;
        }
        float rgb[3];
        if (USE_SH) {
          float B[16];
          sh_dir_basis(p, sCam, v.sh_degree, B);
          rgb[0] = rgb[1] = rgb[2] = 0.5f;
          sh_accumulate(shs + src * v.sh_K * 3, B, 0, (v.sh_degree + 1) * (v.sh_degree + 1), rgb);
          uint8_t cl = 0;
#pragma unroll
          for (int ch = 0; ch < 3; ch++) if (rgb[ch] < 0.0f) { cl |= (uint8_t)(1u << ch); rgb[ch] = 0.0f; }
          clamped[i] = cl;
        } else if (SIX) {
          const float* c6 = colors + 6 * src;
          rgb[0] = __ldg(c6); rgb[1] = __ldg(c6 + 1); rgb[2] = __ldg(c6 + 2);
          r3 = make_float4(__ldg(c6 + 3), __ldg(c6 + 4), __ldg(c6 + 5), 0.f);
        } else {
          load3(colors, src, rgb);
          if (v.raw_params) {
#pragma unroll
            for (int ch = 0; ch < 3; ch++) rgb[ch] = fmaf(SH_C0, rgb[ch], 0.5f);
          }
          if (LOG_SH && v.sh_degree > 0) {
            float B[16];
            sh_dir_basis(p, sCam, v.sh_degree, B);
            sh_accumulate(shs + src * v.sh_K * 3, B, 1, (v.sh_degree + 1) * (v.sh_degree + 1), rgb);
          }
        }
        const float kdet = LOG2E * idet;
        r0 = make_float4(px, py, cv.c * kdet, -cv.b * kdet);
        r1 = make_float4(cv.a * kdet, o, hx, hy);
        r2 = make_float4(rgb[0], rgb[1], rgb[2], cv.t[2]);
        if (DEPTH) r3 = make_float4(cv.t[2], p[2], 1.0f, 0.f);
        if (reach) {
          tile_rect_tight(px, py, rad, hx, hy, v.gx, v.gy, v.row0, v.row1, x0, y0, x1, y1);
          big_splat = count_small_tiles(v, tile_count, i, x0, y0, x1, y1);
          bx0 = x0; by0 = y0; bx1 = x1; by1 = y1;
        }
      }
    }
    if (v.num_owners == 0 || in_band) {
      float4* dst = reinterpret_cast<float4*>(splat + i * LGR_SPLAT_FLOATS);
      dst[0] = r0; dst[1] = r1; dst[2] = r2;
      if (SIX || DEPTH) reinterpret_cast<float4*>(v.splat_ext)[i] = r3;
    }
    radii[i] = rad_out;
    if (USE_SH && rad_out == 0) clamped[i] = 0;
  } else if (i < n) {
    radii[i] = 0;
  }
  warp_count_big_tiles(v, tile_count, big_splat, bx0, by0, bx1, by1);
  if (v.num_owners > 0) {
    __shared__ int sCnt[PROJ_THREADS / 32];
    const int lane = threadIdx.x & 31, wid = threadIdx.x >> 5;
    const unsigned bal = __ballot_sync(0xffffffffu, in_band);
    if (lane == 0) sCnt[wid] = __popc(bal);
    __syncthreads();
    int base = 0, total = 0;
#pragma unroll
    for (int w = 0; w < PROJ_THREADS / 32; w++) { const int c = sCnt[w]; if (w < wid) base += c; total += c; }
    if (in_band) v.band_ids[(int64_t)blockIdx.x * PROJ_THREADS + base + __popc(bal & ((1u << lane) - 1u))] = (int)i;
    if (threadIdx.x == 0) v.band_blk[blockIdx.x] = total;
    __syncthreads();
  }
  {
    const unsigned st_w = __reduce_add_sync(0xffffffffu, (unsigned)stock_tiles);
    const int vis_w = __popc(__ballot_sync(0xffffffffu, rad_out > 0));
    if ((threadIdx.x & 31) == 0) { sStock[threadIdx.x >> 5] = st_w; sVis[threadIdx.x >> 5] = vis_w; }
    __syncthreads();
    if (threadIdx.x == 0) {
      unsigned long long a = 0; int b = 0;
#pragma unroll
      for (int w = 0; w < PROJ_THREADS / 32; w++) { a += sStock[w]; b += sVis[w]; }
      if (a) atomicAdd(reinterpret_cast<unsigned long long*>(meta + 2), a);
      if (b) atomicAdd(meta + 4, b);
    }
  }
}

template <Colour C, bool COV3D, bool DEPTH, bool ROWS>
__global__ void __launch_bounds__(PROJ_THREADS)
project_bwd_kernel(View v, int64_t n, const float* __restrict__ means, const float* __restrict__ opac,
                   const float* __restrict__ scales, const float* __restrict__ rots, const float* __restrict__ shs, const int32_t* __restrict__ radii,
                   const uint8_t* __restrict__ clamped, const float* __restrict__ dsplat, float* __restrict__ dmeans,
                   float* __restrict__ dmeans2D, float* __restrict__ dopac, float* __restrict__ dscales,
                   float* __restrict__ drots, float* __restrict__ dcolors, float* __restrict__ dshs,
                   float* __restrict__ grad_rows, void* const* __restrict__ peer_stage, int my_rank) {
  static_assert(!(C == Colour::RGB6 && DEPTH), "the depth pass generates channels 3..5: colours are (N,3)");
  static_assert(!(C == Colour::LOG_SH && COV3D), "LoG's raw parameters come with scales and rotations");
  static_assert(!ROWS || (C == Colour::RGB && !COV3D && !DEPTH), "band mode rows carry three precomputed colours only");
  constexpr bool USE_SH = C == Colour::SH, LOG_SH = C == Colour::LOG_SH, SIX = C == Colour::RGB6;
  __shared__ float sV[16], sP[16], sCam[3];
  if (threadIdx.x < 16) { sV[threadIdx.x] = v.view[threadIdx.x]; sP[threadIdx.x] = v.proj[threadIdx.x]; }
  if ((USE_SH || LOG_SH) && threadIdx.x < 3) sCam[threadIdx.x] = v.campos[threadIdx.x];
  __syncthreads();
  int64_t blk = blockIdx.x;
  if (ROWS && peer_stage) {
    int64_t first = 0;
    for (int o = 0; o <= my_rank && o < v.num_owners - 1; o++) first += v.band_count[o];
    if (my_rank == v.num_owners - 1) first = 0;
    blk = (blk + first / PROJ_THREADS) % gridDim.x;
  }
  int64_t i = blk * PROJ_THREADS + threadIdx.x;
  const bool active = i < n;
  if (!ROWS && !active) return;
  int64_t row = 0;
  if (ROWS && active) {
    row = i;
    i = v.band_rows[row];
  }
  float dm[3] = {0.f, 0.f, 0.f}, dm2[2] = {0.f, 0.f}, dop = 0.f, dsc[3] = {0.f, 0.f, 0.f}, dq[4] = {0.f, 0.f, 0.f, 0.f};
  float drgb[3] = {0.f, 0.f, 0.f}, dext[3] = {0.f, 0.f, 0.f};
  const bool live = active && radii[i] > 0;
  const int64_t src = (v.gather && live) ? v.gather[i] : i;
  const int K = v.sh_K;
  if (live) {
    const float4 g0 = ldg4(dsplat + i * LGR_GRAD_FLOATS);
    const float4 g1 = ldg4(dsplat + i * LGR_GRAD_FLOATS + 4);
    const float4 g2 = ldg4(dsplat + i * LGR_GRAD_FLOATS + 8);
// ... 400 lines not shown
```

log_b200/csrc/lgr_shard.cu:

```cuda
#include "lgr_common.cuh"
#include "lgr_prof.cuh"

namespace lgr {

constexpr int SHARD_THREADS = 256;
constexpr int SHARD_WARPS = SHARD_THREADS / 32;
constexpr int SHARD_MAX_RANKS = 32;
constexpr unsigned FULLMASK = 0xffffffffu;


__device__ __forceinline__ int owner_of_row(int y, int gy, int R) {
  const int base = gy / R, extra = gy - base * R;
  const int split = extra * (base + 1);
  return y < split ? y / (base + 1) : extra + (y - split) / max(base, 1);
}

__device__ __forceinline__ bool owner_range(const View& v, int R, const float* __restrict__ splat,
                                            const int32_t* __restrict__ radii, int64_t i, int64_t n, int& o0, int& o1) {
  o0 = 0; o1 = -1;
  if (i >= n) return false;
  const int rad = radii[i];
  if (rad <= 0) return false;
  const float4 r0 = ldg4(splat + i * LGR_SPLAT_FLOATS);
  const float4 r1 = ldg4(splat + i * LGR_SPLAT_FLOATS + 4);
// ... 54 lines not shown
      for (int k = 1; k < 32; k <<= 1) { const int y = __shfl_up_sync(FULLMASK, w, k); if (lane >= k) w += y; }
      warp_sum[lane] = w;
    }
    __syncthreads();
    const int carry = carry_s;
    if (b < B) pre[b] = carry + (wid ? warp_sum[wid - 1] : 0) + x - c;
    __syncthreads();
    if (tid == 1023) carry_s = carry + warp_sum[31];
    __syncthreads();
  }
  if (tid == 0) {
    const int total = carry_s;
    send_blk[(int64_t)2 * L.R * B + o] = total;
    reinterpret_cast<int32_t*>(reinterpret_cast<float*>(peer_base[o]) + L.off_count)[L.me] = total;
  }
}

__global__ void __launch_bounds__(SHARD_THREADS)
shard_push_kernel(View v, ShardLayout L, int64_t n, int64_t gid_base, const float* __restrict__ splat,
                  const int32_t* __restrict__ radii, const int32_t* __restrict__ send_blk, int B,
                  void* const* __restrict__ peer_base) {
  __shared__ __align__(16) int sW[SHARD_MAX_RANKS][SHARD_WARPS];
  __shared__ float4 sRows[SHARD_THREADS * 3];
  const int lane = threadIdx.x & 31, wid = threadIdx.x >> 5;
  const int64_t i = (int64_t)blockIdx.x * SHARD_THREADS + threadIdx.x;
  int o0, o1;
  const bool valid = owner_range(v, L.R, splat, radii, i, n, o0, o1);
  count_owner_hits(valid, o0, o1, L.R, sW);
  float4 r0, r1, r2;
  int rad = 0;
  if (valid) {
    r0 = ldg4(splat + i * LGR_SPLAT_FLOATS); r1 = ldg4(splat + i * LGR_SPLAT_FLOATS + 4);
    r2 = ldg4(splat + i * LGR_SPLAT_FLOATS + 8);
    rad = radii[i];
  }
  for (int o = 0; o < L.R; o++) {
    int cnt = 0, before = 0;
#pragma unroll
    for (int w = 0; w < SHARD_WARPS; w++) { const int c = sW[o][w]; if (w < wid) before += c; cnt += c; }
    if (cnt == 0) continue;
    const bool t = valid && o0 <= o && o <= o1;
    const unsigned bal = __ballot_sync(FULLMASK, t);
    const int first = send_blk[(int64_t)(L.R + o) * B + blockIdx.x];
    float* base = reinterpret_cast<float*>(peer_base[o]);
    const int64_t row0 = (int64_t)L.me * L.cap + first;
    if (t) {
      const int r = before + __popc(bal & ((1u << lane) - 1u));
      sRows[3 * r] = r0; sRows[3 * r + 1] = r1; sRows[3 * r + 2] = r2;
      reinterpret_cast<int32_t*>(base + L.off_radii)[row0 + r] = rad;
      reinterpret_cast<int32_t*>(base + L.off_gid)[row0 + r] = (int32_t)(gid_base + i);
    }
    __syncthreads();
    float4* dst = reinterpret_cast<float4*>(base + L.off_splat + row0 * LGR_SPLAT_FLOATS);
    for (int k = threadIdx.x; k < cnt * 3; k += SHARD_THREADS) dst[k] = sRows[k];
    __syncthreads();
  }
}

__global__ void __launch_bounds__(SHARD_THREADS)
shard_recv_count_kernel(View v, ShardLayout L, float* __restrict__ xbuf, float* __restrict__ dsplat,
                        int32_t* __restrict__ tile_count, int32_t* __restrict__ meta, float* __restrict__ pw_rows,
                        int32_t* __restrict__ pc_rows) {
  __shared__ __align__(16) unsigned sStock[SHARD_WARPS];
  __shared__ __align__(16) int sVis[SHARD_WARPS];
  __shared__ int64_t s_first[LGR_SHARD_MAX_RANKS + 1];
  const int64_t total = region_setup(v, s_first);
  const int32_t* radii = reinterpret_cast<const int32_t*>(xbuf + L.off_radii);
  unsigned stock = 0;
  int vis = 0;
  for (int64_t base = (int64_t)blockIdx.x * SHARD_THREADS; base < total; base += (int64_t)gridDim.x * SHARD_THREADS) {
    bool big_splat = false;
    int bx0 = 0, by0 = 0, bx1 = 0, by1 = 0;
    if (base + threadIdx.x < total) {
      const int64_t slot = region_row(v, s_first, base + threadIdx.x);
      const float* rec = xbuf + L.off_splat + slot * LGR_SPLAT_FLOATS;
      const float4 r0 = *reinterpret_cast<const float4*>(rec);
      const float4 r1 = *reinterpret_cast<const float4*>(rec + 4);
      const int rad = radii[slot];
      int x0, y0, x1, y1;
      tile_rect(r0.x, r0.y, rad, v.gx, v.gy, x0, y0, x1, y1);
      stock += (unsigned)((x1 - x0) * max(0, min(y1, v.row1) - max(y0, v.row0)));
      vis += 1;
      tile_rect_tight(r0.x, r0.y, rad, r1.z, r1.w, v.gx, v.gy, v.row0, v.row1, x0, y0, x1, y1);
      big_splat = count_small_tiles(v, tile_count, slot, x0, y0, x1, y1);
      bx0 = x0; by0 = y0; bx1 = x1; by1 = y1;
      float4* z = reinterpret_cast<float4*>(dsplat + slot * LGR_GRAD_FLOATS);
      z[0] = z[1] = z[2] = make_float4(0.f, 0.f, 0.f, 0.f);
      if (pw_rows) pw_rows[slot] = 0.f;
      if (pc_rows) pc_rows[slot] = 0;
    }
    warp_count_big_tiles(v, tile_count, big_splat, bx0, by0, bx1, by1);
  }
  const unsigned st_w = __reduce_add_sync(FULLMASK, stock);
  const int vis_w = __reduce_add_sync(FULLMASK, vis);
  if ((threadIdx.x & 31) == 0) { sStock[threadIdx.x >> 5] = st_w; sVis[threadIdx.x >> 5] = vis_w; }
  __syncthreads();
  if (threadIdx.x == 0) {
    unsigned long long a = 0; int b = 0;
#pragma unroll
    for (int w = 0; w < SHARD_WARPS; w++) { a += sStock[w]; b += sVis[w]; }
    if (a) atomicAdd(reinterpret_cast<unsigned long long*>(meta + 2), a);
    if (b) atomicAdd(meta + 4, b);
  }
}

template <typename T>
__global__ void __launch_bounds__(SHARD_THREADS)
shard_return_kernel(ShardLayout L, const float* __restrict__ xbuf, const T* __restrict__ rows, int items_per_row,
                    int64_t dst_off_floats, void* const* __restrict__ peer_base) {
  const int32_t* count = reinterpret_cast<const int32_t*>(xbuf + L.off_count);
  int64_t total = 0;
  for (int s = 0; s < L.R; s++) total += count[s];
  total *= items_per_row;
  for (int64_t t = (int64_t)blockIdx.x * SHARD_THREADS + threadIdx.x; t < total; t += (int64_t)gridDim.x * SHARD_THREADS) {
    int s = 0;
    int64_t first = 0;
    while (s + 1 < L.R && t >= first + (int64_t)count[s] * items_per_row) { first += (int64_t)count[s] * items_per_row; s++; }
    const int64_t k = t - first;
    T* dst = reinterpret_cast<T*>(reinterpret_cast<float*>(peer_base[s]) + dst_off_floats) +
             (int64_t)L.me * L.cap * items_per_row + k;
    *dst = rows[(int64_t)s * L.cap * items_per_row + k];
  }
}

__global__ void __launch_bounds__(SHARD_THREADS)
shard_return_packed_kernel(ShardLayout L, const float* __restrict__ xbuf, const float* __restrict__ dsplat_rows,
                           const float* __restrict__ pw_rows, const int32_t* __restrict__ pc_rows,
                           void* const* __restrict__ peer_base) {
  __shared__ int64_t first[SHARD_MAX_RANKS + 1];
  if (threadIdx.x == 0) {
    const int32_t* count = reinterpret_cast<const int32_t*>(xbuf + L.off_count);
    int64_t acc = 0;
    for (int s = 0; s < L.R; s++) { first[s] = acc; acc += (int64_t)count[s] * 3; }
    first[L.R] = acc;
  }
  __syncthreads();
  const int64_t total = first[L.R], stride = (int64_t)gridDim.x * SHARD_THREADS;
  constexpr int U = 4;
  for (int64_t t0 = (int64_t)blockIdx.x * SHARD_THREADS + threadIdx.x; t0 < total; t0 += U * stride) {
    float4 val[U];
    float4* dst[U];
#pragma unroll
    for (int u = 0; u < U; u++) {
      const int64_t t = t0 + u * stride;
      dst[u] = nullptr;
      if (t < total) {
        int s = 0;
        while (s + 1 < L.R && t >= first[s + 1]) s++;
        const int64_t k = t - first[s];
        const int64_t row = (int64_t)s * L.cap + k / 3;
        const int part = (int)(k % 3);
        val[u] = reinterpret_cast<const float4*>(dsplat_rows)[row * 3 + part];
        if (part == 2) {
          val[u].y = pw_rows ? pw_rows[row] : 0.f;
          val[u].z = pc_rows ? __int_as_float(pc_rows[row]) : 0.f;
        }
        dst[u] = reinterpret_cast<float4*>(reinterpret_cast<float*>(peer_base[s]) + L.off_dsplat) + (int64_t)L.me * L.cap * 3 + k;
      }
    }
#pragma unroll
    for (int u = 0; u < U; u++)
      if (dst[u]) *dst[u] = val[u];
  }
}

__global__ void __launch_bounds__(SHARD_THREADS)
shard_gather_kernel(View v, ShardLayout L, int64_t n, const float* __restrict__ splat, const int32_t* __restrict__ radii,
// ... 118 lines not shown
```

log_b200/rasterizer.py:

```python
import ctypes
from typing import NamedTuple, Optional

import torch
import torch.nn as nn

from . import _capi
from ._capi import LGR_FILTER_ADD, LGR_FILTER_MAX, LGR_FILTER_NONE, LgrView

PREZERO_DSPLAT = bool(int(__import__('os').environ.get('LGR_PREZERO_DSPLAT', '0')))
RANKED_BIN = bool(int(__import__('os').environ.get('LGR_RANKED_BIN', '1')))
CONTRIB_BITS = bool(int(__import__('os').environ.get('LGR_CONTRIB_BITS', '1')))
FLAVOUR_STOCK = 'stock'
FLAVOUR_FORK = 'fork'


class GaussianRasterizationSettings(NamedTuple):
    image_height: int
    image_width: int
    tanfovx: float
    tanfovy: float
    bg: torch.Tensor
    scale_modifier: float
    viewmatrix: torch.Tensor
    projmatrix: torch.Tensor
    sh_degree: int
    campos: torch.Tensor
    prefiltered: bool
    debug: bool


def _ptr(t: Optional[torch.Tensor]):
    return None if t is None or t.numel() == 0 else ctypes.c_void_p(t.data_ptr())


def _f32c(t: Optional[torch.Tensor], name: str, device=None):
    if t is None:
        return None
    _capi.require_cuda(t, name)
    if device is not None and t.device != device:
        raise _capi.LgrError(f'{name} is on {t.device}, expected {device}')
    if t.dtype != torch.float32:
        raise TypeError(f'{name} must be float32, got {t.dtype}')
    t = t.detach()
    if not t.is_contiguous():
        t = t.contiguous()
    if t.data_ptr() % 16:
        t = t.clone()
    return t


def _stream(device=None):
    return _capi.current_stream(device)


def _make_view(s: GaussianRasterizationSettings, filter_mode: int, want_aux: bool, sh_coeffs: int, tile_rows, keep,
               num_owners=0, band_ids=None, band_count=None, band_blk=None, band_rows=None, band_dsplat=None,
               raw_params=False, tile_rank=None, gather_index=None, pid_map=None, cov3D_precomp=None, splat_ext=None,
               log_depth=False):
    dev = s.viewmatrix.device
    vm, pm = _f32c(s.viewmatrix, 'viewmatrix'), _f32c(s.projmatrix, 'projmatrix', dev)
    bg = _f32c(s.bg, 'bg', dev)
    cp = _f32c(s.campos, 'campos', dev) if s.campos is not None else None
    keep.extend([vm, pm, bg, cp])
    v = LgrView()
    v.image_height, v.image_width = int(s.image_height), int(s.image_width)
    v.tanfovx, v.tanfovy = float(s.tanfovx), float(s.tanfovy)
    v.scale_modifier = float(s.scale_modifier)
    v.sh_degree, v.sh_coeffs = int(s.sh_degree), int(sh_coeffs)
    v.filter_mode, v.want_aux = int(filter_mode), int(bool(want_aux))
    v.tile_row_begin, v.tile_row_end = (0, 0) if tile_rows is None else (int(tile_rows[0]), int(tile_rows[1]))
    v.num_owners = int(num_owners)
    v.raw_params = int(bool(raw_params))
    v.band_ids_d = band_ids.data_ptr() if band_ids is not None else None
    v.band_count_d = band_count.data_ptr() if band_count is not None else None
    v.band_blk_d = band_blk.data_ptr() if band_blk is not None else None
    v.band_rows_d = band_rows.data_ptr() if band_rows is not None else None
    v.band_dsplat_d = band_dsplat.data_ptr() if band_dsplat is not None else None
    v.tile_rank_d = tile_rank.data_ptr() if tile_rank is not None else None
    v.gather_index_d = gather_index.data_ptr() if gather_index is not None else None
    v.pid_map_d = pid_map.data_ptr() if pid_map is not None else None
    v.cov3D_precomp_d = cov3D_precomp.data_ptr() if cov3D_precomp is not None else None
    if splat_ext is not None:
        v.num_channels, v.splat_ext_d = 6, splat_ext.data_ptr()
        v.log_depth = int(bool(log_depth))
    v.viewmatrix_d, v.projmatrix_d = vm.data_ptr(), pm.data_ptr()
    v.campos_d = cp.data_ptr() if cp is not None else None
    v.bg_d = bg.data_ptr()
    return v


def set_contrib_lists(view, buf, D, n_contrib):
    if buf is None:
        view.contrib_id_d = view.contrib_entry_d = view.contrib_count_d = view.last_contrib_d = None
        return
    p = buf.data_ptr()
    view.contrib_id_d, view.contrib_entry_d, view.contrib_count_d = p, p + 4 * D, p + 8 * D
    view.last_contrib_d = n_contrib.data_ptr()


def colour_channels(colors_precomp, settings, shs=None, raw_params=False, gather_index=None, num_owners=0, log_depth=False):
    width = None
    if colors_precomp is not None:
        width = int(colors_precomp.shape[-1]) if colors_precomp.dim() > 0 else 0
        if width not in (3, 6):
            raise _capi.LgrError(f'colors_precomp must have 3 or 6 channels per Gaussian, got shape {tuple(colors_precomp.shape)}')
    if log_depth:
        if width == 6:
            raise _capi.LgrError('render_depth generates the depth channels itself: pass three-channel colors_precomp (N,3), '
                                 'not (N,6)')
        if num_owners > 0:
            raise _capi.LgrError('render_depth is not available in band mode (num_owners > 0)')
        return 6
    if width is None or width == 3:
        return 3
    if colors_precomp.dim() != 2:
        raise _capi.LgrError(f'six-channel colors_precomp must be (N,6), got shape {tuple(colors_precomp.shape)}')
    for what, used in (('shs', shs is not None), ('raw_params', raw_params), ('gather_index (render_gathered)', gather_index is not None),
                       ('band mode (num_owners > 0)', num_owners > 0)):
        if used:
            raise _capi.LgrError(f'six colour channels (colors_precomp (N,6)) are not available with {what}')
    if settings.bg.numel() != 6:
        raise _capi.LgrError(f'six colour channels need a background of 6 entries (raster_settings.bg), got {settings.bg.numel()}')
    return 6


def use_contrib_lists(D, max_tile_len):
    return CONTRIB_BITS and D > 0 and (max_tile_len is None or max_tile_len <= _capi.LGR_CONTRIB_MAX_LIST)


class RasterState:
    __slots__ = ('view', 'keep', 'n', 'num_instances', 'max_tile_len', 'stock_instances', 'num_visible', 'splat',
                 'radii', 'clamped', 'tile_start', 'sorted_ids', 'final_T', 'n_contrib', 'image', 'sh', 'num_owners',
                 'band_ids', 'band_count', 'band_counts_host', 'point_count', 'meta', 'cov3D', 'dcov3D', 'contrib',
                 'channels', 'splat_ext', 'log_depth')

    def read_stats(self):
        m = self.meta.tolist()
        return dict(num_instances=int(m[0]), max_tile_len=int(m[1]), stock_instances=(m[2] & 0xffffffff) | ((m[3] & 0xffffffff) << 32),
                    num_visible=int(m[4]), overflow=int(m[6]))

    def contrib_lists(self):
        if self.contrib is None:
            return None
        D = self.num_instances
        return self.contrib[:D], self.contrib[D:2 * D], self.contrib[2 * D:]


def rasterize_forward(settings, means3D, opacities, scales, rotations, colors_precomp, shs, filter_mode, want_aux,
                      tile_rows=None, num_owners=0, raw_params=False, prezero_dsplat=None, gather_index=None,
                      instance_capacity=None, cov3D_precomp=None, log_depth=False):
    channels = colour_channels(colors_precomp, settings, shs, raw_params, gather_index, num_owners, log_depth)
    if log_depth:
        bg3 = settings.bg.reshape(-1)[:3]
        settings = settings._replace(bg=torch.cat([bg3, bg3]))
    lib = _capi.load()
    dev = means3D.device
    if cov3D_precomp is not None and (raw_params or num_owners > 0):
        raise _capi.LgrError('cov3D_precomp is not available with raw_params or in band mode')
    for name, t in (('opacities', opacities), ('scales', scales), ('rotations', rotations), ('colors_precomp', colors_precomp),
                    ('shs', shs), ('cov3D_precomp', cov3D_precomp), ('viewmatrix', settings.viewmatrix), ('projmatrix', settings.projmatrix), ('bg', settings.bg)):
        if t is not None and t.device != dev:
            raise _capi.LgrError(f'{name} is on {t.device}, means3D on {dev}: all inputs of a call must share one device')
    n = int(means3D.shape[0])
    keep = []
    if gather_index is not None:
        if gather_index.dtype != torch.int64 or gather_index.device != dev or gather_index.dim() != 1:
            raise _capi.LgrError('gather_index must be a 1-D int64 tensor on the inputs\' device')
        if num_owners > 0:
            raise _capi.LgrError('gather_index is not available in band mode')
        gather_index = gather_index.contiguous()
        keep.append(gather_index)
        n = int(gather_index.shape[0])
    K = 0 if shs is None else int(shs.shape[1])
    band_ids = band_count = band_blk = band_rows = band_dsplat = None
    if prezero_dsplat is None:
        prezero_dsplat = PREZERO_DSPLAT and torch.is_grad_enabled()
    if num_owners == 0 and prezero_dsplat:
        band_dsplat = torch.empty((max(n, 1), _capi.LGR_GRAD_FLOATS), dtype=torch.float32, device=dev)
    if num_owners > 0:
        band_rows = torch.empty((max(n, 1),), dtype=torch.int32, device=dev)
        band_dsplat = torch.empty((max(n, 1), _capi.LGR_GRAD_FLOATS), dtype=torch.float32, device=dev)
        nb = (n + 255) // 256
        band_ids = torch.empty((max(256 * nb, 1),), dtype=torch.int32, device=dev)
        band_blk = torch.empty((2 * nb + 1,), dtype=torch.int32, device=dev)
        band_count = torch.empty((num_owners,), dtype=torch.int32, device=dev)
    tile_rank = torch.empty((max(n, 1), 4), dtype=torch.int32, device=dev) if RANKED_BIN else None
    keep.append(tile_rank)
    splat_ext = torch.empty((max(n, 1), 4), dtype=torch.float32, device=dev) if channels == 6 else None
    keep.append(splat_ext)
    view = _make_view(settings, filter_mode, want_aux, K, tile_rows, keep, num_owners, band_ids, band_count, band_blk, band_rows, band_dsplat,
                      raw_params, tile_rank, gather_index, cov3D_precomp=cov3D_precomp, splat_ext=splat_ext, log_depth=log_depth)
    H, W = view.image_height, view.image_width
    gx, gy = (W + 15) // 16, (H + 15) // 16
    rows = gy if tile_rows is None else int(tile_rows[1]) - int(tile_rows[0])
    ntiles = gx * rows
    i32 = dict(dtype=torch.int32, device=dev)
    f32 = dict(dtype=torch.float32, device=dev)
    splat = torch.empty((n, _capi.LGR_SPLAT_FLOATS), **f32)
    radii = torch.empty((n,), **i32)
    clamped = torch.empty((n,), dtype=torch.uint8, device=dev) if shs is not None else None
    tile_start = torch.empty((ntiles + 1,), **i32)
    tile_cursor = torch.empty((_capi.LGR_TILE_SCRATCH_INTS * max(ntiles, 1),), **i32)
    meta = torch.empty((_capi.LGR_META_INTS,), **i32)
    st = _stream(dev)
    _capi.check(lib.lgr_forward_project(ctypes.byref(view), n, _ptr(means3D), _ptr(opacities), _ptr(scales),
                                        _ptr(rotations), _ptr(colors_precomp), _ptr(shs), _ptr(splat), _ptr(radii),
                                        _ptr(clamped), _ptr(tile_start), _ptr(tile_cursor), _ptr(meta), st),
                'lgr_forward_project')
    u32 = dict(dtype=torch.int32, device=dev)
    image = torch.empty((channels, H, W), **f32) if tile_rows is None else torch.zeros((channels, H, W), **f32)
    final_T = torch.empty((H, W), **f32) if tile_rows is None else torch.ones((H, W), **f32)
    n_contrib = torch.empty((H, W), **i32) if tile_rows is None else torch.zeros((H, W), **i32)
    pid = pwp = pw = pc = None
    if want_aux:
        pc = torch.zeros((n,), **i32)
        pid = torch.empty((H, W), **i32) if tile_rows is None else torch.full((H, W), -1, **i32)
        pwp = torch.empty((H, W), **f32) if tile_rows is None else torch.zeros((H, W), **f32)
        pw = torch.zeros((n,), **f32)
    if instance_capacity:
        if num_owners > 0:
            raise _capi.LgrError('instance_capacity (device-sized call) is not available in band mode')
        D, max_len, num_long, stock_D, m = int(instance_capacity), None, None, None, None
        inst_key, inst_val = torch.empty((D,), **u32), torch.empty((D,), **u32)
        sorted_ids = torch.empty((D,), **i32)
        contrib = torch.empty((2 * D + ntiles,), **i32) if use_contrib_lists(D, None) else None
        keep.append(contrib)
        set_contrib_lists(view, contrib, D, n_contrib)
        _capi.check(lib.lgr_forward_render_device_sized(ctypes.byref(view), n, D, _ptr(meta), _ptr(splat), _ptr(radii), _ptr(tile_start),
                                                        _ptr(tile_cursor), _ptr(inst_key), _ptr(inst_val), _ptr(sorted_ids), _ptr(image),
                                                        _ptr(final_T), _ptr(n_contrib), _ptr(pid), _ptr(pwp), _ptr(pw), _ptr(pc), st),
                    'lgr_forward_render_device_sized')
    else:
        m = (meta if band_count is None else torch.cat([meta, band_count])).tolist()
        D, max_len, num_long = int(m[0]), int(m[1]), int(m[5])
        stock_D = (m[2] & 0xffffffff) | ((m[3] & 0xffffffff) << 32)
        if D < 0 or stock_D > 0x7fffffff:
            raise _capi.LgrError(f'this view needs {stock_D} (Gaussian, tile) instances by the stock rule (D = {m[0] & 0xffffffff} binned, '
                                 f'{m[4]} of {n} Gaussians visible, longest tile list {max_len}): more than 2^31 - 1 is unsupported')
        inst_key = torch.empty((D,), **u32)
        inst_val = torch.empty((D,), **u32)
        inst_tmp = torch.empty((2 * D,), **u32) if max_len > lib.lgr_sort_smem_capacity() else None
        sorted_ids = torch.empty((D,), **i32)
        contrib = torch.empty((2 * D + ntiles,), **i32) if use_contrib_lists(D, max_len) else None
        keep.append(contrib)
        set_contrib_lists(view, contrib, D, n_contrib)
        _capi.check(lib.lgr_forward_render(ctypes.byref(view), n, D, max_len, num_long, _ptr(splat), _ptr(radii), _ptr(tile_start),
                                           _ptr(tile_cursor), _ptr(inst_key), _ptr(inst_val), _ptr(inst_tmp),
                                           _ptr(sorted_ids), _ptr(image), _ptr(final_T), _ptr(n_contrib), _ptr(pid),
                                           _ptr(pwp), _ptr(pw), _ptr(pc), st), 'lgr_forward_render')
    s = RasterState()
    s.view, s.keep, s.n, s.num_instances, s.max_tile_len = view, keep, n, D, max_len
    s.stock_instances, s.num_visible = stock_D, (int(m[4]) if m is not None else None)
    s.meta = meta
    s.cov3D, s.dcov3D = cov3D_precomp, None
    s.splat, s.radii, s.clamped, s.tile_start, s.sorted_ids = splat, radii, clamped, tile_start, sorted_ids
    s.final_T, s.n_contrib, s.image, s.sh = final_T, n_contrib, image, shs is not None
    s.point_count = pc
    s.contrib = contrib
    s.channels, s.splat_ext, s.log_depth = channels, splat_ext, bool(log_depth)
    s.num_owners, s.band_ids, s.band_count = num_owners, (band_ids, band_blk, band_rows, band_dsplat), band_count
    s.band_counts_host = [int(x) for x in m[_capi.LGR_META_INTS:]] if num_owners > 0 else None
    return image, radii, pid, pwp, pw, s


def rasterize_backward(state: RasterState, grad_image, means3D, opacities, scales, rotations, colors_precomp, shs,
                       peer_stage=None, my_rank=0):
    lib = _capi.load()
    dev = means3D.device
    n = state.n
    f32 = dict(dtype=torch.float32, device=dev)
    g = _f32c(grad_image, 'grad_image', dev)
    if state.band_ids[3] is not None:
        dsplat = state.band_ids[3]
        state.band_ids = state.band_ids[:3] + (None,)
    else:
        dsplat = torch.zeros((n, _capi.LGR_GRAD_FLOATS), **f32)
    if state.num_owners > 0:
        m_rows = sum(state.band_counts_host)
        if peer_stage is not None:
            _capi.check(lib.lgr_backward(ctypes.byref(state.view), n, state.num_instances, _ptr(means3D), _ptr(opacities),
                                         _ptr(scales), _ptr(rotations), _ptr(colors_precomp), None, _ptr(state.splat),
                                         _ptr(state.radii), None, _ptr(state.tile_start), _ptr(state.sorted_ids),
                                         _ptr(state.image), _ptr(g), _ptr(dsplat), None, None, None, None, None, None, None,
                                         None, ctypes.c_void_p(peer_stage.data_ptr()), int(my_rank), m_rows, _stream(dev)), 'lgr_backward')
            return None
        rows = torch.empty((m_rows, _capi.LGR_ROW_FLOATS), **f32)
        _capi.check(lib.lgr_backward(ctypes.byref(state.view), n, state.num_instances, _ptr(means3D), _ptr(opacities),
                                     _ptr(scales), _ptr(rotations), _ptr(colors_precomp), None, _ptr(state.splat),
                                     _ptr(state.radii), None, _ptr(state.tile_start), _ptr(state.sorted_ids),
                                     _ptr(state.image), _ptr(g), _ptr(dsplat), None, None, None, None, None, None, None,
                                     ctypes.c_void_p(rows.data_ptr()) if rows.numel() else _ptr(dsplat), None, 0, m_rows, _stream(dev)),
                    'lgr_backward')
        return rows
    dmeans3D = torch.empty((n, 3), **f32)
    dmeans2D = torch.empty((n, 3), **f32)
    dopac = torch.empty((n,), **f32)
    cov = state.cov3D is not None
    dscales = None if cov else torch.empty((n, 3), **f32)
    drot = None if cov else torch.empty((n, 4), **f32)
    if cov:
        state.dcov3D = torch.empty((n, 6), **f32)
        state.view.dcov3D_d = state.dcov3D.data_ptr()
    dcolors = torch.empty((n, 3 if state.log_depth else state.channels), **f32) if colors_precomp is not None else None
    dshs = torch.empty((n,) + tuple(shs.shape[1:]), **f32) if shs is not None else None
    _capi.check(lib.lgr_backward(ctypes.byref(state.view), n, state.num_instances, _ptr(means3D), _ptr(opacities),
                                 _ptr(scales), _ptr(rotations), _ptr(colors_precomp), _ptr(shs), _ptr(state.splat),
                                 _ptr(state.radii), _ptr(state.clamped), _ptr(state.tile_start), _ptr(state.sorted_ids),
                                 _ptr(state.image), _ptr(g), _ptr(dsplat), _ptr(dmeans3D),
                                 _ptr(dmeans2D), _ptr(dopac), _ptr(dscales), _ptr(drot), _ptr(dcolors), _ptr(dshs), None,
                                 None, 0, 0, _stream(dev)), 'lgr_backward')
    return dmeans3D, dmeans2D, dopac, dscales, drot, dcolors, dshs


def point_id_count(point_count: torch.Tensor):
    lib = _capi.load()
    n = int(point_count.shape[0])
    dev = point_count.device
    i32 = dict(dtype=torch.int32, device=dev)
    scratch = torch.empty((2 * ((n + 1023) // 1024) + 1,), **i32)
    ids = torch.empty((n,), **i32)
    cnt = torch.empty((n,), **i32)
    num = torch.empty((1,), **i32)
    _capi.check(lib.lgr_point_compact(n, _ptr(point_count), _ptr(scratch), _ptr(ids), _ptr(cnt),
                                      ctypes.c_void_p(num.data_ptr()), _stream(dev)), 'lgr_point_compact')
# ... 126 lines not shown
```

log_b200/sharded.py:

```python
from typing import List, Tuple

import torch
import torch.distributed as dist

GRAD_FLOATS_PRECOMP = 17


def tile_row_partition(image_height: int, world_size: int) -> List[Tuple[int, int]]:
    gy = (image_height + 15) // 16
    base, extra = divmod(gy, world_size)
    out, start = [], 0
    for r in range(world_size):
        n = base + (1 if r < extra else 0)
        out.append((start, start + n))
        start += n
    return out


def owner_chunk(num_gaussians: int, world_size: int) -> int:
    return ((num_gaussians + world_size - 1) // world_size + 255) // 256 * 256


def owner_partition(num_gaussians: int, world_size: int) -> List[Tuple[int, int]]:
    chunk = owner_chunk(num_gaussians, world_size)
# ... 126 lines not shown
class SplatExchange:

    def __init__(self, num_gaussians: int, image_height: int, rank: int, world: int, own_buffer, peer_ptrs, barrier):
        from . import _capi
        self.n, self.rank, self.world = int(num_gaussians), int(rank), int(world)
        if not 0 < self.world <= _capi.LGR_SHARD_MAX_RANKS:
            raise ValueError(f'shard mode supports 1..{_capi.LGR_SHARD_MAX_RANKS} ranks, got {world}')
        self.layout, self.floats = shard_layout(self.n, self.world, self.rank)
        self.cap = int(self.layout.cap)
        self.lo, self.hi = owner_partition(self.n, self.world)[self.rank]
        self.band = tile_row_partition(image_height, self.world)[self.rank]
        self.image_height = int(image_height)
        peer_ptrs = [int(p) for p in peer_ptrs]
        _capi.require_cuda(own_buffer, 'the exchange buffer')
        if own_buffer.dtype != torch.float32 or own_buffer.numel() < self.floats:
            raise ValueError(f'the exchange buffer must be a float32 tensor of >= {self.floats} elements')
        if len(peer_ptrs) != self.world or peer_ptrs[self.rank] != own_buffer.data_ptr():
            raise ValueError('peer_ptrs needs one address per rank, entry `rank` being own_buffer')
        self.buf, self.barrier = own_buffer, barrier
        dev = self.buf.device
        self.peer_ptrs = torch.tensor(peer_ptrs, dtype=torch.int64, device=dev)
        L, rows = self.layout, self.world * self.cap
        self.count = self.buf[L.off_count:L.off_count + self.world].view(torch.int32)
        self.header = self.buf[L.off_count:L.off_count + 40].view(torch.int32)
        self.meta = self.header[32:40]
        self.recv_splat = self.buf[L.off_splat:L.off_splat + rows * 12].view(rows, 12)
        self.recv_radii = self.buf[L.off_radii:L.off_radii + rows].view(torch.int32)
        self.recv_gid = self.buf[L.off_gid:L.off_gid + rows].view(torch.int32)
        self.dsplat_rows = torch.empty((rows, _capi.LGR_GRAD_FLOATS), dtype=torch.float32, device=dev)
        self.count.zero_()
        self.recv_radii.zero_()
        self._cache = {}
        self._in_flight = False
        import os
        self.sync_free = bool(int(os.environ.get('LGR_SYNC_FREE', '0')))
        self._inst_cap = 0

    def _scratch(self, name: str, shape, dtype):
        need = 1
        for d in shape:
            need *= int(d)
        t = self._cache.get(name)
        if t is None or t.numel() < need or t.dtype != dtype:
            t = torch.empty((max(need, 1) * 5 // 4 + 64,), dtype=dtype, device=self.buf.device)
            self._cache[name] = t
        return t[:need].view(*shape)

    @classmethod
    def over_symmetric_memory(cls, num_gaussians: int, image_height: int, group=None):
        import torch.distributed._symmetric_memory as symm
        group = group if group is not None else dist.group.WORLD
        world, rank = dist.get_world_size(group), dist.get_rank(group)
        _, floats = shard_layout(num_gaussians, world, rank)
        dev = torch.device('cuda', torch.cuda.current_device())
        buf = symm.empty(floats, dtype=torch.float32, device=dev)
        handle = symm.rendezvous(buf, group)
        self = cls(num_gaussians, image_height, rank, world, buf, list(handle.buffer_ptrs), handle.barrier)
        self.handle = handle
        handle.barrier()
        return self

    def project_and_send(self, settings, means3D, opacities, scales, rotations, colors_precomp=None, shs=None,
                         filter_mode=None, want_aux=True, raw_params=False, render_depth=False) -> ShardStep:
        import ctypes
        from . import _capi
        from .rasterizer import _f32c, _make_view, _ptr, _stream
        lib = _capi.load()
        if render_depth:
            raise _capi.LgrError('render_depth is not available in shard mode: the exchange moves three-channel records only')
        if colors_precomp is not None and int(colors_precomp.shape[-1]) != 3:
            raise _capi.LgrError(f'shard mode renders three precomputed colour channels, got colors_precomp {tuple(colors_precomp.shape)}')
        filter_mode = _capi.LGR_FILTER_MAX if filter_mode is None else filter_mode
        dev = self.buf.device
        n = int(means3D.shape[0])
        if n != self.hi - self.lo:
            raise ValueError(f'rank {self.rank} owns Gaussians [{self.lo},{self.hi}): expected {self.hi - self.lo} rows, got {n}')
        s = ShardStep()
        s.inputs = tuple(_f32c(t, k, dev) for k, t in (('means3D', means3D), ('opacities', opacities), ('scales', scales),
                                                       ('rotations', rotations), ('colors_precomp', colors_precomp), ('shs', shs)))
        m, o, sc, r, c, sh = s.inputs
        s.keep, s.n, s.want_aux, s.settings = [], n, bool(want_aux), settings
        K = 0 if sh is None else int(sh.shape[1])
        s.view_full = _make_view(settings, filter_mode, want_aux, K, None, s.keep, raw_params=raw_params)
        from .rasterizer import RANKED_BIN
        rank_rows = self._scratch('tile_rank', (self.world * self.cap, 4), torch.int32) if RANKED_BIN else None
        s.view_band = _make_view(settings, filter_mode, want_aux, K, self.band, s.keep, raw_params=raw_params, tile_rank=rank_rows,
                                 pid_map=self.recv_gid)
        s.view_band.region_count_d = self.buf.data_ptr() + 4 * int(self.layout.off_count)
        s.view_band.region_cap, s.view_band.num_regions = self.cap, self.world
        H, W = s.view_full.image_height, s.view_full.image_width
        if H != self.image_height:
            raise ValueError('image height differs from the one the bands were cut for')
        gx, gy = (W + 15) // 16, (H + 15) // 16
        i32 = dict(dtype=torch.int32, device=dev)
        s.splat = self._scratch('splat', (n, _capi.LGR_SPLAT_FLOATS), torch.float32)
        s.radii = torch.empty((n,), **i32)
        s.clamped = self._scratch('clamped', (n,), torch.uint8) if sh is not None else None
        s.tile_start_full = self._scratch('tile_start_full', (gx * gy + 1,), torch.int32)
        cursor = self._scratch('cursor_full', (_capi.LGR_TILE_SCRATCH_INTS * gx * gy,), torch.int32)
        meta = self._scratch('meta_full', (_capi.LGR_META_INTS,), torch.int32)
        st = _stream()
        _capi.check(lib.lgr_forward_project(ctypes.byref(s.view_full), n, _ptr(m), _ptr(o), _ptr(sc), _ptr(r), _ptr(c), _ptr(sh),
                                            _ptr(s.splat), _ptr(s.radii), _ptr(s.clamped), _ptr(s.tile_start_full), _ptr(cursor),
                                            _ptr(meta), st), 'lgr_forward_project')
        s.send_scratch = self._scratch('send', (_capi.shard_send_ints(n, self.world),), torch.int32)
        _capi.check(lib.lgr_shard_send(ctypes.byref(s.view_full), ctypes.byref(self.layout), n, self.lo, _ptr(s.splat),
                                       _ptr(s.radii), _ptr(s.send_scratch), ctypes.c_void_p(self.peer_ptrs.data_ptr()), st),
                    'lgr_shard_send')
        return s

    def receive_and_render(self, s: ShardStep):
        import ctypes
        from . import _capi
        from .rasterizer import _ptr, _stream, set_contrib_lists, use_contrib_lists
        lib = _capi.load()
        dev = self.buf.device
        v = s.view_band
        H, W = v.image_height, v.image_width
        gx = (W + 15) // 16
        ntiles = gx * (self.band[1] - self.band[0])
        rows = self.world * self.cap
        i32, f32 = dict(dtype=torch.int32, device=dev), dict(dtype=torch.float32, device=dev)
        s.tile_start = self._scratch('tile_start', (ntiles + 1,), torch.int32)
        cursor = self._scratch('cursor', (_capi.LGR_TILE_SCRATCH_INTS * max(ntiles, 1),), torch.int32)
        meta = self.meta
        st = _stream()
        s.pw_rows = s.pc_rows = None
        if s.want_aux:
            s.pw_rows = self._scratch('pw_rows', (rows,), torch.float32)
            s.pc_rows = self._scratch('pc_rows', (rows,), torch.int32)
        _capi.check(lib.lgr_shard_recv_bin_aux(ctypes.byref(v), ctypes.byref(self.layout), _ptr(self.buf), _ptr(self.dsplat_rows),
                                               _ptr(s.tile_start), _ptr(cursor), _ptr(meta), _ptr(s.pw_rows), _ptr(s.pc_rows), st),
                    'lgr_shard_recv_bin_aux')
        s.image = torch.zeros((3, H, W), **f32)
        final_T = self._scratch('final_T', (H, W), torch.float32)
        n_contrib = self._scratch('n_contrib', (H, W), torch.int32)
        pid = pwp = None
        if s.want_aux:
            pid = torch.full((H, W), -1, **i32)
            pwp = torch.zeros((H, W), **f32)
        if self.sync_free and self._inst_cap > 0:
            cap = self._inst_cap
            inst_key = self._scratch('inst_key', (cap,), torch.int32)
            inst_val = self._scratch('inst_val', (cap,), torch.int32)
            s.sorted_ids = self._scratch('sorted_ids', (cap,), torch.int32)
            set_contrib_lists(v, self._scratch('contrib', (2 * cap + ntiles,), torch.int32) if use_contrib_lists(cap, None) else None,
                              cap, n_contrib)
            s.num_instances, s.max_tile_len, s.num_rows, s.stock_instances = cap, None, None, None
            _capi.check(lib.lgr_forward_render_device_sized(ctypes.byref(v), rows, cap, _ptr(meta), _ptr(self.recv_splat), _ptr(self.recv_radii),
                                                            _ptr(s.tile_start), _ptr(cursor), _ptr(inst_key), _ptr(inst_val), _ptr(s.sorted_ids),
                                                            _ptr(s.image), _ptr(final_T), _ptr(n_contrib), _ptr(pid), _ptr(pwp),
                                                            _ptr(s.pw_rows), _ptr(s.pc_rows), st), 'lgr_forward_render_device_sized')
            return s.image, s.radii, pid, pwp
        h = self.header.tolist()
        m = h[32:40]
        D, max_len, num_long = int(m[0]), int(m[1]), int(m[5])
        s.num_instances, s.max_tile_len, s.num_rows = D, max_len, int(sum(h[:self.world]))
        s.stock_instances = (m[2] & 0xffffffff) | ((m[3] & 0xffffffff) << 32)
        if max_len <= lib.lgr_sort_smem_capacity():
            self._inst_cap = max(self._inst_cap, D + D // 4 + 4096)
        inst_key = self._scratch('inst_key', (D,), torch.int32)
        inst_val = self._scratch('inst_val', (D,), torch.int32)
        inst_tmp = self._scratch('inst_tmp', (2 * D,), torch.int32) if max_len > lib.lgr_sort_smem_capacity() else None
        s.sorted_ids = self._scratch('sorted_ids', (D,), torch.int32)
        set_contrib_lists(v, self._scratch('contrib', (2 * D + ntiles,), torch.int32) if use_contrib_lists(D, max_len) else None,
                          D, n_contrib)
        _capi.check(lib.lgr_forward_render(ctypes.byref(v), rows, D, max_len, num_long, _ptr(self.recv_splat), _ptr(self.recv_radii),
                                           _ptr(s.tile_start), _ptr(cursor), _ptr(inst_key), _ptr(inst_val), _ptr(inst_tmp),
                                           _ptr(s.sorted_ids), _ptr(s.image), _ptr(final_T), _ptr(n_contrib), _ptr(pid), _ptr(pwp),
                                           _ptr(s.pw_rows), _ptr(s.pc_rows), st), 'lgr_forward_render')
        return s.image, s.radii, pid, pwp

    def stats(self):
        h = self.header.tolist()
        m = h[32:40]
        return dict(num_rows=int(sum(h[:self.world])), num_instances=int(m[0]), max_tile_len=int(m[1]),
                    stock_instances=(m[2] & 0xffffffff) | ((m[3] & 0xffffffff) << 32), overflow=int(m[6]))

    def check_overflow(self):
        st = self.stats()
        if st['overflow']:
            self._inst_cap = 0
            raise RuntimeError(f'shard-mode step outgrew its device-sized buffers (flags {st["overflow"]}, D = {st["num_instances"]}, '
                               f'longest tile list {st["max_tile_len"]}): its outputs are invalid, redo the step')
        return st

    def blend_backward_and_return(self, s: ShardStep, grad_image):
        import ctypes
        from . import _capi
        from .rasterizer import _f32c, _ptr, _stream
        lib = _capi.load()
        s.grad_image = _f32c(grad_image, 'grad_image', self.buf.device)
        st, L, peers = _stream(), self.layout, ctypes.c_void_p(self.peer_ptrs.data_ptr())
        rows = self.world * self.cap
        _capi.check(lib.lgr_blend_backward(ctypes.byref(s.view_band), rows, s.num_instances, _ptr(self.recv_splat),
                                           _ptr(s.tile_start), _ptr(s.sorted_ids), _ptr(s.image), _ptr(s.grad_image),
                                           _ptr(self.dsplat_rows), st), 'lgr_blend_backward')
        _capi.check(lib.lgr_shard_return_packed(ctypes.byref(L), _ptr(self.buf), _ptr(self.dsplat_rows), _ptr(s.pw_rows), _ptr(s.pc_rows),
                                                peers, st), 'lgr_shard_return_packed')

    def gather_and_project_backward(self, s: ShardStep):
        import ctypes
        from . import _capi
        from .rasterizer import _ptr, _stream
        lib = _capi.load()
        dev = self.buf.device
        n = s.n
        m, o, sc, r, c, sh = s.inputs
        f32 = dict(dtype=torch.float32, device=dev)
        dsplat = self._scratch('dsplat_local', (n, _capi.LGR_GRAD_FLOATS), torch.float32)
        pw = torch.empty((n,), **f32) if s.want_aux else None
        pc = torch.empty((n,), dtype=torch.int32, device=dev) if s.want_aux else None
        st = _stream()
        _capi.check(lib.lgr_shard_gather_packed(ctypes.byref(s.view_full), ctypes.byref(self.layout), n, _ptr(s.splat), _ptr(s.radii),
                                                _ptr(s.send_scratch), _ptr(self.buf), _ptr(dsplat), _ptr(pw), _ptr(pc), st),
                    'lgr_shard_gather_packed')
        dmeans3D, dmeans2D = torch.empty((n, 3), **f32), torch.empty((n, 3), **f32)
        dopac, dscales, drot = torch.empty((n,), **f32), torch.empty((n, 3), **f32), torch.empty((n, 4), **f32)
        dcolors = torch.empty((n, 3), **f32) if c is not None else None
        dshs = torch.empty_like(sh) if sh is not None else None
        if n:
            _capi.check(lib.lgr_backward(ctypes.byref(s.view_full), n, 0, _ptr(m), _ptr(o), _ptr(sc), _ptr(r), _ptr(c), _ptr(sh),
                                         _ptr(s.splat), _ptr(s.radii), _ptr(s.clamped), _ptr(s.tile_start_full), None,
                                         _ptr(s.image), _ptr(s.grad_image), _ptr(dsplat), _ptr(dmeans3D), _ptr(dmeans2D),
                                         _ptr(dopac), _ptr(dscales), _ptr(drot), _ptr(dcolors), _ptr(dshs), None, None, 0, 0, st),
                        'lgr_backward')
        return (dmeans3D, dmeans2D, dopac, dscales, drot, dcolors, dshs), pw, pc

    def forward(self, settings, means3D, opacities, scales, rotations, colors_precomp=None, shs=None, **kw):
        if self._in_flight:
            self.barrier()
        self._in_flight = True
        s = self.project_and_send(settings, means3D, opacities, scales, rotations, colors_precomp, shs, **kw)
        self.barrier()
        return self.receive_and_render(s) + (s,)

    def backward(self, s: ShardStep, grad_image):
        self.blend_backward_and_return(s, grad_image)
        self.barrier()
        self._in_flight = False
        return self.gather_and_project_backward(s)


class _ShardRasterize(torch.autograd.Function):

    @staticmethod
# ... 20 lines not shown
```

Measured before the change: 1.688 billion.

## Replace ranked bin scatter with two-pass row-partition and windowed tile placement

Drops the precomputed per-Gaussian tile-rank path and the per-instance global atomic scatter. Binning becomes a partition kernel that buffers small-footprint instances in shared memory, groups them by tile row, and writes them contiguously into a staging buffer. A placement kernel then buckets them per tile within a shared-memory window, so it uses fewer global atomics and writes more coalesced keys and values. Small instance counts still use the direct atomic path. The cost is an extra kernel and a staging buffer (inst_tmp) that is now always allocated, which adds memory traffic.

```diff
diff --git a/include/log_b200_raster.h b/include/log_b200_raster.h
--- a/include/log_b200_raster.h
+++ b/include/log_b200_raster.h
@@ -7,7 +7,7 @@
 extern "C" {
 #endif
 
-#define LGR_ABI_VERSION 23
+#define LGR_ABI_VERSION 24
 #define LGR_TILE 16
 
 #define LGR_FILTER_ADD 0
@@ -85,7 +85,7 @@
 int lgr_forward_render_device_sized(const lgr_view* view, int64_t n, int64_t instance_capacity, int32_t* meta_d,
                                     const float* splat_d, const int32_t* radii_d, int32_t* tile_start_d,
                                     int32_t* tile_cursor_d, uint32_t* inst_key_d, uint32_t* inst_val_d,
-                                    int32_t* sorted_ids_d, float* image_d, float* final_T_d, int32_t* n_contrib_d,
+                                    uint32_t* inst_tmp_d, int32_t* sorted_ids_d, float* image_d, float* final_T_d, int32_t* n_contrib_d,
                                     int32_t* point_id_pixel_d, float* point_weight_pixel_d, float* point_weight_d,
                                     int32_t* point_count_d, void* stream);
 
diff --git a/log_b200/_capi.py b/log_b200/_capi.py
--- a/log_b200/_capi.py
+++ b/log_b200/_capi.py
@@ -10,7 +10,7 @@
 LGR_GRAD_FLOATS = 12
 LGR_META_INTS = 8
 LGR_TILE_SCRATCH_INTS = 33
-LGR_ABI_VERSION = 23
+LGR_ABI_VERSION = 24
 LGR_CONTRIB_MAX_LIST = 1 << 24
 LGR_STAGE_HEADER_FLOATS = 64
 LGR_ROW_FLOATS = 20
@@ -128,7 +128,7 @@
     lib.lgr_forward_render.restype = ctypes.c_int
     lib.lgr_forward_render.argtypes = [ctypes.POINTER(LgrView), _i64, _i64, _i32, _i32] + [_vp] * 16
     lib.lgr_forward_render_device_sized.restype = ctypes.c_int
-    lib.lgr_forward_render_device_sized.argtypes = [ctypes.POINTER(LgrView), _i64, _i64] + [_vp] * 16
+    lib.lgr_forward_render_device_sized.argtypes = [ctypes.POINTER(LgrView), _i64, _i64] + [_vp] * 17
     lib.lgr_sparse_adam.restype = ctypes.c_int
     lib.lgr_sparse_adam.argtypes = [_i64, _i32, _vp, _vp, _vp, _vp, _vp, _vp, _i64, ctypes.c_double, ctypes.c_double,
                                     ctypes.c_double, ctypes.c_double, _vp]
diff --git a/log_b200/csrc/lgr_bin.cu b/log_b200/csrc/lgr_bin.cu
--- a/log_b200/csrc/lgr_bin.cu
+++ b/log_b200/csrc/lgr_bin.cu
@@ -9,7 +9,7 @@
 __global__ void __launch_bounds__(SCAN_THREADS)
 tile_scan_kernel(int ntiles, int32_t* __restrict__ tile_start ,
                  int32_t* __restrict__ cursor ,
-                 int32_t* __restrict__ meta, int small_cap, int ranked) {
+                 int32_t* __restrict__ meta, int small_cap) {
   __shared__ int warp_sum[SCAN_THREADS / 32];
   __shared__ int carry_s, maxl_s, nbig_s;
   const int tid = threadIdx.x, lane = tid & 31, wid = tid >> 5;
@@ -35,7 +35,7 @@
     const int carry = carry_s;
     const int excl = carry + (wid ? warp_sum[wid - 1] : 0) + x - c;
     if (i < ntiles) {
-      tile_start[i] = excl; cursor[i * CSTRIDE + ranked] = 0;
+      tile_start[i] = excl; cursor[i * CSTRIDE] = 0;
       if (c > small_cap) cursor[CSTRIDE * ntiles + atomicAdd(&nbig_s, 1)] = i;
     }
     __syncthreads();
@@ -49,92 +49,273 @@
   if (tid == 0) { tile_start[ntiles] = carry_s; meta[0] = carry_s; meta[1] = maxl_s; meta[5] = nbig_s; }
 }
 
-constexpr int SCATTER_THREADS = 256;
-
-__global__ void __launch_bounds__(SCATTER_THREADS)
-bin_scatter_kernel(View v, int64_t n, const float* __restrict__ splat, const int32_t* __restrict__ radii,
-                   const int32_t* __restrict__ tile_start, int32_t* __restrict__ cursor, uint32_t* __restrict__ inst_key,
-                   uint32_t* __restrict__ inst_val, int64_t capacity ) {
+constexpr int BIN_THREADS = 256;
+constexpr int PART_ROUNDS = 8;
+constexpr int PLACE_GRID = 132 * 4;
+constexpr int PART_CAP = 2048;
+constexpr int PART_FLUSH_AT = PART_CAP - 4 * BIN_THREADS;
+constexpr int PLACE_ITEMS = 8;
+constexpr int PLACE_CHUNK = PLACE_ITEMS * BIN_THREADS;
+#ifndef LGR_BIN_DIRECT_MAX
+#define LGR_BIN_DIRECT_MAX (1 << 16)
+#endif
+constexpr int64_t BIN_DIRECT_MAX = LGR_BIN_DIRECT_MAX;
+constexpr int PLACE_WINDOW = 2047;
+
+__device__ __forceinline__ unsigned long long composite(uint32_t k, uint32_t v) { return ((unsigned long long)k << 32) | v; }
+
+int part_smem_bytes(int rows) { return 3 * (int)sizeof(int32_t) * max(rows, 1); }
+
+__device__ __forceinline__ void block_exclusive_scan(const int* in, int* out, int len, int* wsum) {
+  const int tid = threadIdx.x, lane = tid & 31, wid = tid >> 5;
+  int carry = 0;
+  for (int base = 0; base < len; base += BIN_THREADS) {
+    const int c = base + tid < len ? in[base + tid] : 0;
+    int x = c;
+#pragma unroll
+    for (int o = 1; o < 32; o <<= 1) { const int y = __shfl_up_sync(0xffffffffu, x, o); if (lane >= o) x += y; }
+    if (lane == 31) wsum[wid] = x;
+    __syncthreads();
+    int before = carry, all = carry;
+#pragma unroll
+    for (int w = 0; w < BIN_THREADS / 32; w++) { if (w < wid) before += wsum[w]; all += wsum[w]; }
+    if (base + tid < len) out[base + tid] = before + x - c;
+    carry = all;
+    __syncthreads();
+  }
+}
+
+__global__ void __launch_bounds__(BIN_THREADS, 6)
+bin_partition_kernel(View v, int64_t n, const float* __restrict__ splat, const int32_t* __restrict__ radii,
+                     const int32_t* __restrict__ tile_start, int32_t* __restrict__ cursor, unsigned long long* __restrict__ stage,
+                     int32_t* __restrict__ stage_tile, int64_t capacity ,
+                     int rounds ,
+                     uint32_t* __restrict__ direct_key, uint32_t* __restrict__ direct_val ) {
+  extern __shared__ int32_t row_tab[];
+  __shared__ uint32_t s_key[PART_CAP], s_id[PART_CAP];
+  __shared__ int32_t s_tile[PART_CAP];
+  __shared__ uint16_t s_perm[PART_CAP];
+  __shared__ int s_fill;
+  __shared__ int s_wsum[BIN_THREADS / 32];
   __shared__ int64_t s_first[LGR_SHARD_MAX_RANKS + 1];
+  const int rows = v.row1 - v.row0, lane = threadIdx.x & 31;
+  int32_t* r_cnt = row_tab;
+  int32_t* r_off = row_tab + rows;
+  int32_t* r_base = row_tab + 2 * rows;
+  for (int r = threadIdx.x; r < rows; r += BIN_THREADS) r_cnt[r] = 0;
+  if (threadIdx.x == 0) s_fill = 0;
   const int64_t total = v.region_count ? region_setup(v, s_first) : n;
-  for (int64_t base = (int64_t)blockIdx.x * SCATTER_THREADS; base < total; base += (int64_t)gridDim.x * SCATTER_THREADS) {
-  int64_t i = base + threadIdx.x;
-  bool live = i < total;
-  if (live && v.region_count) i = region_row(v, s_first, i);
-  if (live && v.num_owners > 0) {
-    const int b = (int)(i / 256), sl = (int)(i % 256);
-    if (sl >= v.band_blk[b]) live = false;
-    else {
-      const int id = v.band_ids[i];
-      v.band_rows[v.band_blk[v.band_blocks + b] + sl] = id;
-      if (v.band_dsplat) {
-        float4* z = reinterpret_cast<float4*>(v.band_dsplat + (int64_t)id * LGR_GRAD_FLOATS);
+  __syncthreads();
+  auto flush = [&]() {
+    const int held = s_fill;
+    if (direct_key) {
+      for (int e = threadIdx.x; e < held; e += BIN_THREADS) {
+        const int t = s_tile[e];
+        const int64_t pos = (int64_t)tile_start[t] + atomicAdd(cursor + t * CSTRIDE, 1);
+        if (pos < capacity) { direct_key[pos] = s_key[e]; direct_val[pos] = s_id[e]; }
+      }
+      __syncthreads();
+      for (int r = threadIdx.x; r < rows; r += BIN_THREADS) r_cnt[r] = 0;
+      if (threadIdx.x == 0) s_fill = 0;
+      __syncthreads();
+      return;
+    }
+    for (int r = threadIdx.x; r < rows; r += BIN_THREADS) {
+      const int c = r_cnt[r];
+      if (c > 0) r_base[r] = tile_start[r * v.gx] + atomicAdd(cursor + r * v.gx * CSTRIDE + 2, c);
+    }
+    block_exclusive_scan(r_cnt, r_off, rows, s_wsum);
+    for (int r = threadIdx.x; r < rows; r += BIN_THREADS) r_base[r] -= r_off[r];
+    __syncthreads();
+    for (int e = threadIdx.x; e < held; e += BIN_THREADS) s_perm[atomicAdd(&r_off[s_tile[e] / v.gx], 1)] = (uint16_t)e;
+    __syncthreads();
+    for (int j = threadIdx.x; j < held; j += BIN_THREADS) {
+      const int e = s_perm[j], t = s_tile[e];
+      const int64_t pos = (int64_t)r_base[t / v.gx] + j;
+      if (pos < capacity) { stage[pos] = composite(s_key[e], s_id[e]); stage_tile[pos] = t; }
+    }
+    __syncthreads();
+    for (int r = threadIdx.x; r < rows; r += BIN_THREADS) r_cnt[r] = 0;
+    if (threadIdx.x == 0) s_fill = 0;
+    __syncthreads();
+  };
+  for (int64_t chunk = (int64_t)blockIdx.x * rounds * BIN_THREADS; chunk < total; chunk += (int64_t)gridDim.x * rounds * BIN_THREADS) {
+    for (int round = 0; round < rounds; round++) {
+      int64_t i = chunk + round * BIN_THREADS + threadIdx.x;
+      bool live = i < total;
+      if (live && v.region_count) i = region_row(v, s_first, i);
+      if (live && v.num_owners > 0) {
+        const int b = (int)(i / 256), sl = (int)(i % 256);
+        if (sl >= v.band_blk[b]) live = false;
+        else {
+          const int id = v.band_ids[i];
+          v.band_rows[v.band_blk[v.band_blocks + b] + sl] = id;
+          if (v.band_dsplat) {
+            float4* z = reinterpret_cast<float4*>(v.band_dsplat + (int64_t)id * LGR_GRAD_FLOATS);
+            z[0] = z[1] = z[2] = make_float4(0.f, 0.f, 0.f, 0.f);
+          }
+          i = id;
+        }
+      }
+      int rad = 0;
+      float4 r0 = make_float4(0.f, 0.f, 0.f, 0.f), r1 = r0;
+      float depth = 0.f;
+      if (live) {
+        rad = radii[i];
+        r0 = ldg4(splat + i * LGR_SPLAT_FLOATS);
+        r1 = ldg4(splat + i * LGR_SPLAT_FLOATS + 4);
+        depth = __ldg(splat + i * LGR_SPLAT_FLOATS + 11);
+        live = rad > 0;
+      }
+      if (live && v.num_owners == 0 && v.band_dsplat) {
+        float4* z = reinterpret_cast<float4*>(v.band_dsplat + i * LGR_GRAD_FLOATS);
         z[0] = z[1] = z[2] = make_float4(0.f, 0.f, 0.f, 0.f);
       }
-      i = id;
-    }
-  }
-  int rad = 0;
-  float4 r0 = make_float4(0.f, 0.f, 0.f, 0.f), r1 = r0;
-  float depth = 0.f;
-  int4 rk = make_int4(-1, -1, -1, -1);
-  if (live) {
-    rad = radii[i];
-    r0 = ldg4(splat + i * LGR_SPLAT_FLOATS);
-    r1 = ldg4(splat + i * LGR_SPLAT_FLOATS + 4);
-    depth = __ldg(splat + i * LGR_SPLAT_FLOATS + 11);
-    if (v.tile_rank) rk = __ldg(reinterpret_cast<const int4*>(v.tile_rank + 4 * i));
-    live = rad > 0;
-  }
-  if (live && v.num_owners == 0 && v.band_dsplat) {
-    float4* z = reinterpret_cast<float4*>(v.band_dsplat + i * LGR_GRAD_FLOATS);
-    z[0] = z[1] = z[2] = make_float4(0.f, 0.f, 0.f, 0.f);
-  }
-  int x0 = 0, y0 = 0, x1 = 0, y1 = 0;
-  uint32_t key = 0;
-  if (live) {
-    live = r1.z > 0.f;
-    if (live) {
-      key = __float_as_uint(depth);
-      tile_rect_tight(r0.x, r0.y, rad, r1.z, r1.w, v.gx, v.gy, v.row0, v.row1, x0, y0, x1, y1);
-    }
-  }
-  const int w = x1 - x0, cnt = live ? w * (y1 - y0) : 0;
-  if (cnt > 0 && cnt <= 4) {
-    int t[4], slot[4];
-#pragma unroll
-    for (int k = 0; k < 4; k++) {
-      const int ty = y0 + k / max(w, 1), tx = x0 + k % max(w, 1);
-      t[k] = k < cnt ? (ty - v.row0) * v.gx + tx : -1;
-    }
-    if (v.tile_rank) {
-      slot[0] = rk.x; slot[1] = rk.y; slot[2] = rk.z; slot[3] = rk.w;
-    } else {
-#pragma unroll
-      for (int k = 0; k < 4; k++) slot[k] = t[k] >= 0 ? atomicAdd(cursor + t[k] * CSTRIDE, 1) : 0;
-    }
-#pragma unroll
-    for (int k = 0; k < 4; k++)
-      if (t[k] >= 0) {
-        const int pos = __ldg(tile_start + t[k]) + slot[k];
-        if (pos < capacity) { inst_key[pos] = key; inst_val[pos] = (uint32_t)i; }
-      }
-  }
-  const int lane = threadIdx.x & 31, big = v.tile_rank ? 1 : 0;
-  unsigned todo = __ballot_sync(0xffffffffu, cnt > 4);
-  while (todo) {
-    const int src = __ffs(todo) - 1;
-    todo &= todo - 1;
-    const int bx0 = __shfl_sync(0xffffffffu, x0, src), by0 = __shfl_sync(0xffffffffu, y0, src);
-    const int bw = __shfl_sync(0xffffffffu, w, src), bcnt = __shfl_sync(0xffffffffu, cnt, src);
-    const uint32_t bkey = __shfl_sync(0xffffffffu, key, src);
-    const uint32_t bid = (uint32_t)__shfl_sync(0xffffffffu, (int)i, src);
-    for (int k = lane; k < bcnt; k += 32) {
-      const int t = (by0 + k / bw - v.row0) * v.gx + bx0 + k % bw;
-      const int pos = tile_start[t] + (big ? cursor[t * CSTRIDE] : 0) + atomicAdd(cursor + t * CSTRIDE + big, 1);
-      if (pos < capacity) { inst_key[pos] = bkey; inst_val[pos] = bid; }
-    }
-  }
+      int x0 = 0, y0 = 0, x1 = 0, y1 = 0;
+      uint32_t key = 0;
+      if (live) {
+        live = r1.z > 0.f;
+        if (live) {
+          key = __float_as_uint(depth);
+          tile_rect_tight(r0.x, r0.y, rad, r1.z, r1.w, v.gx, v.gy, v.row0, v.row1, x0, y0, x1, y1);
+        }
+      }
+      const int w = x1 - x0, cnt = live ? w * (y1 - y0) : 0;
+      const int mine = cnt <= 4 ? cnt : 0;
+      int incl = mine;
+#pragma unroll
+      for (int o = 1; o < 32; o <<= 1) { const int y = __shfl_up_sync(0xffffffffu, incl, o); if (lane >= o) incl += y; }
+      int wbase = 0;
+      if (lane == 31 && incl > 0) wbase = atomicAdd(&s_fill, incl);
+      wbase = __shfl_sync(0xffffffffu, wbase, 31);
+      for (int k = 0, s = wbase + incl - mine; k < mine; k++, s++) {
+        const int ty = y0 + k / w, tx = x0 + k % w;
+        s_key[s] = key; s_id[s] = (uint32_t)i; s_tile[s] = (ty - v.row0) * v.gx + tx;
+        atomicAdd(&r_cnt[ty - v.row0], 1);
+      }
+      unsigned todo = __ballot_sync(0xffffffffu, cnt > 4);
+      while (todo) {
+        const int src = __ffs(todo) - 1;
+        todo &= todo - 1;
+        const int bx0 = __shfl_sync(0xffffffffu, x0, src), by0 = __shfl_sync(0xffffffffu, y0, src);
+        const int bw = __shfl_sync(0xffffffffu, w, src), bcnt = __shfl_sync(0xffffffffu, cnt, src);
+        const uint32_t bkey = __shfl_sync(0xffffffffu, key, src);
+        const uint32_t bid = (uint32_t)__shfl_sync(0xffffffffu, (int)i, src);
+        const int bh = bcnt / bw;
+        if (direct_key) {
+          for (int k = lane; k < bcnt; k += 32) {
+            const int t = (by0 + k / bw - v.row0) * v.gx + bx0 + k % bw;
+            const int64_t pos = (int64_t)tile_start[t] + atomicAdd(cursor + t * CSTRIDE, 1);
+            if (pos < capacity) { direct_key[pos] = bkey; direct_val[pos] = bid; }
+          }
+          continue;
+        }
+        for (int ry = 0; ry < bh; ry += 32) {
+          const int nr = min(32, bh - ry), r_lane = by0 + ry + lane - v.row0;
+          int rb = 0;
+          if (lane < nr) rb = tile_start[r_lane * v.gx] + atomicAdd(cursor + r_lane * v.gx * CSTRIDE + 2, bw);
+          for (int k0 = 0; k0 < nr * bw; k0 += 32) {
+            const int k = k0 + lane;
+            const int p = __shfl_sync(0xffffffffu, rb, k < nr * bw ? k / bw : 0);
+            if (k < nr * bw) {
+              const int64_t pos = (int64_t)p + k % bw;
+              if (pos < capacity) {
+                stage[pos] = composite(bkey, bid);
+                stage_tile[pos] = (by0 + ry + k / bw - v.row0) * v.gx + bx0 + k % bw;
+              }
+            }
+          }
+        }
+      }
+      __syncthreads();
+      if (__syncthreads_or(s_fill > (round == rounds - 1 ? 0 : PART_FLUSH_AT))) flush();
+    }
+  }
+}
+
+__global__ void __launch_bounds__(BIN_THREADS)
+bin_place_kernel(int gx, int ntiles, const int32_t* __restrict__ tile_start, int32_t* __restrict__ cursor,
+                 const unsigned long long* __restrict__ stage, const int32_t* __restrict__ stage_tile, uint32_t* __restrict__ inst_key,
+                 uint32_t* __restrict__ inst_val) {
+  constexpr int PER = (PLACE_WINDOW + 1) / BIN_THREADS;
+  static_assert(PER * BIN_THREADS == PLACE_WINDOW + 1, "bucket count");
+  __shared__ int s_cnt[PLACE_WINDOW + 1];
+  __shared__ int s_base[PLACE_WINDOW];
+  __shared__ unsigned long long s_e[PLACE_CHUNK];
+  __shared__ uint16_t s_b[PLACE_CHUNK];
+  __shared__ int s_wsum[BIN_THREADS / 32];
+  __shared__ int s_t0;
+  const int lane = threadIdx.x & 31, wid = threadIdx.x >> 5;
+  const int total = tile_start[ntiles];
+  for (int beg = blockIdx.x * PLACE_CHUNK; beg < total; beg += gridDim.x * PLACE_CHUNK) {
+    for (int j = threadIdx.x; j <= PLACE_WINDOW; j += BIN_THREADS) s_cnt[j] = 0;
+    if (threadIdx.x == 0) s_t0 = stage_tile[beg] - stage_tile[beg] % gx;
+    __syncthreads();
+    const int t0 = s_t0;
+    int tk[PLACE_ITEMS], rank[PLACE_ITEMS];
+#pragma unroll
+    for (int k = 0; k < PLACE_ITEMS; k++) {
+      const int idx = beg + k * BIN_THREADS + threadIdx.x;
+      tk[k] = idx < total ? stage_tile[idx] : -1;
+    }
+#pragma unroll
+    for (int k = 0; k < PLACE_ITEMS; k++) {
+      rank[k] = 0;
+      if (tk[k] >= 0) {
+        const int b = min(tk[k] - t0, PLACE_WINDOW);
+        rank[k] = b < PLACE_WINDOW ? atomicAdd(&s_cnt[b], 1) : tile_start[tk[k]] + atomicAdd(cursor + tk[k] * CSTRIDE, 1);
+        tk[k] = b;
+      }
+    }
+    __syncthreads();
+    int c[PER], sum = 0;
+    const int b0 = threadIdx.x * PER;
+    int32_t* const cur = cursor + (int64_t)(t0 + b0) * CSTRIDE;
+#pragma unroll
+    for (int q = 0; q < PER; q++) {
+      c[q] = s_cnt[b0 + q];
+      sum += c[q];
+    }
+#pragma unroll
+    for (int q = 0; q < PER; q++)
+      if (c[q] > 0 && b0 + q < PLACE_WINDOW) s_base[b0 + q] = tile_start[t0 + b0 + q] + atomicAdd(cur + q * CSTRIDE, c[q]);
+    int x = sum;
+#pragma unroll
+    for (int o = 1; o < 32; o <<= 1) { const int y = __shfl_up_sync(0xffffffffu, x, o); if (lane >= o) x += y; }
+    if (lane == 31) s_wsum[wid] = x;
+    __syncthreads();
+    int off = x - sum;
+#pragma unroll
+    for (int w = 0; w < BIN_THREADS / 32; w++) if (w < wid) off += s_wsum[w];
+#pragma unroll
+    for (int q = 0; q < PER; q++) {
+      const int b = threadIdx.x * PER + q;
+      s_cnt[b] = off;
+      if (b < PLACE_WINDOW && c[q] > 0) s_base[b] -= off;
+      off += c[q];
+    }
+    __syncthreads();
+#pragma unroll
+    for (int k = 0; k < PLACE_ITEMS; k++) {
+      if (tk[k] >= 0) {
+        const unsigned long long e = stage[beg + k * BIN_THREADS + threadIdx.x];
+        const int b = tk[k];
+        if (b < PLACE_WINDOW) {
+          const int j = s_cnt[b] + rank[k];
+          s_e[j] = e; s_b[j] = (uint16_t)b;
+        } else {
+          inst_key[rank[k]] = (uint32_t)(e >> 32); inst_val[rank[k]] = (uint32_t)e;
+        }
+      }
+    }
+    __syncthreads();
+    const int inside = s_cnt[PLACE_WINDOW];
+    for (int j = threadIdx.x; j < inside; j += BIN_THREADS) {
+      const int pos = s_base[s_b[j]] + j;
+      const unsigned long long e = s_e[j];
+      inst_key[pos] = (uint32_t)(e >> 32); inst_val[pos] = (uint32_t)e;
+    }
+    __syncthreads();
   }
 }
 
@@ -230,8 +411,6 @@
   int stack_beg[MSD_STACK], stack_len[MSD_STACK];
   int top, shift, overflow;
 };
-
-__device__ __forceinline__ unsigned long long composite(uint32_t k, uint32_t v) { return ((unsigned long long)k << 32) | v; }
 
 __device__ __forceinline__ bool sort_tile_msd(uint32_t* kA, uint32_t* vA, uint32_t* kB, uint32_t* vB, int len, MsdShared& sh) {
   const int tid = threadIdx.x, lane = tid & 31, wid = tid >> 5;
@@ -448,9 +627,9 @@
   return 0;
 }
 
-int launch_tile_scan(int ntiles, int32_t* tile_start, int32_t* cursor, int32_t* meta, bool ranked, cudaStream_t st) {
+int launch_tile_scan(int ntiles, int32_t* tile_start, int32_t* cursor, int32_t* meta, bool , cudaStream_t st) {
   ProfScope ps(K_TILE_SCAN, st);
-  tile_scan_kernel<<<1, SCAN_THREADS, 0, st>>>(ntiles, tile_start, cursor, meta, SORT_CAP_SMALL_FWD, ranked ? 1 : 0);
+  tile_scan_kernel<<<1, SCAN_THREADS, 0, st>>>(ntiles, tile_start, cursor, meta, SORT_CAP_SMALL_FWD);
   LGR_CHECK_LAUNCH();
   return 0;
 }
@@ -467,15 +646,31 @@
     LGR_CHECK_LAUNCH();
   }
   if (num_inst == 0 && v.num_owners == 0 && v.band_dsplat == nullptr) return 0;
+  if (num_inst > 0 && (!inst_tmp || !sorted_ids)) return LGR_E_BADARG;
   const int ntiles = v.gx * (v.row1 - v.row0);
-  unsigned blocks = (unsigned)((n + SCATTER_THREADS - 1) / SCATTER_THREADS);
+  const int part_smem = part_smem_bytes(v.row1 - v.row0);
+  if (part_smem > 160 * 1024) return LGR_E_UNSUPPORTED;
+  {
+    cudaError_t e = cudaFuncSetAttribute(bin_partition_kernel, cudaFuncAttributeMaxDynamicSharedMemorySize, part_smem);
+    if (e != cudaSuccess) return (int)e;
+  }
+  const int rounds = (int)max((int64_t)1, min((int64_t)PART_ROUNDS, n / ((int64_t)BIN_THREADS * 132 * 16)));
+  const int64_t chunk = (int64_t)rounds * BIN_THREADS;
+  unsigned blocks = (unsigned)((n + chunk - 1) / chunk);
   if (v.region_count && blocks > (unsigned)LGR_REGION_GRID) blocks = (unsigned)LGR_REGION_GRID;
+  unsigned long long* stage = reinterpret_cast<unsigned long long*>(inst_tmp);
   {
-    ProfScope ps(K_BIN_SCATTER, st);
-    bin_scatter_kernel<<<blocks, SCATTER_THREADS, 0, st>>>(v, n, splat, radii, tile_start, cursor, inst_key, inst_val,
-                                                           meta_dev ? num_inst : (int64_t)0x7fffffffffffffffLL);
-  }
-  LGR_CHECK_LAUNCH();
+    ProfScope ps(K_BIN_SCATTER, st, num_inst > BIN_DIRECT_MAX ? 2 : 1);
+    const bool direct = num_inst <= BIN_DIRECT_MAX;
+    bin_partition_kernel<<<blocks, BIN_THREADS, part_smem, st>>>(v, n, splat, radii, tile_start, cursor, stage, sorted_ids, num_inst,
+                                                                 rounds, direct ? inst_key : nullptr, direct ? inst_val : nullptr);
+    LGR_CHECK_LAUNCH();
+    if (num_inst > 0 && !direct) {
+      const unsigned place = (unsigned)min((int64_t)PLACE_GRID, (num_inst + PLACE_CHUNK - 1) / PLACE_CHUNK);
+      bin_place_kernel<<<place, BIN_THREADS, 0, st>>>(v.gx, ntiles, tile_start, cursor, stage, sorted_ids, inst_key, inst_val);
+      LGR_CHECK_LAUNCH();
+    }
+  }
   if (num_inst == 0) return 0;
   int id_bits = 8;
   while (id_bits < 32 && (n - 1) >> id_bits) id_bits += 8;
@@ -502,7 +697,6 @@
     tile_sort_kernel<0><<<num_long, SORT_THREADS, 16 * cap, st>>>(long_list, tile_start, inst_key, inst_val, inst_tmp, sorted_ids, SORT_CAP_SMALL, cap, id_bits, nullptr, nullptr);
     LGR_CHECK_LAUNCH();
     if (max_len > SORT_CAP_LARGE) {
-      if (!inst_tmp) return LGR_E_CAPACITY;
       tile_sort_kernel<1><<<num_long, SORT_THREADS, 0, st>>>(long_list, tile_start, inst_key, inst_val, inst_tmp, sorted_ids, SORT_CAP_LARGE, 0, id_bits, nullptr, nullptr);
       LGR_CHECK_LAUNCH();
     }
diff --git a/log_b200/csrc/lgr_capi.cu b/log_b200/csrc/lgr_capi.cu
--- a/log_b200/csrc/lgr_capi.cu
+++ b/log_b200/csrc/lgr_capi.cu
@@ -146,7 +146,7 @@
   if (rc) return rc;
   rc = launch_band_scan(v, st);
   if (rc) return rc;
-  return launch_tile_scan(ntiles, tile_start_d, tile_cursor_d, meta_d, view->tile_rank_d != nullptr, st);
+  return launch_tile_scan(ntiles, tile_start_d, tile_cursor_d, meta_d, false, st);
 }
 
 int lgr_forward_render(const lgr_view* view, int64_t n, int64_t num_instances, int32_t max_tile_len,
@@ -158,7 +158,7 @@
   if (!view_ok(view) || n < 0 || num_instances < 0 || num_long_tiles < 0 || !tile_start_d || !tile_cursor_d || !image_d || !final_T_d ||
       !n_contrib_d)
     return LGR_E_BADARG;
-  if (num_instances > 0 && (!inst_key_d || !inst_val_d || !sorted_ids_d || !splat_d || !radii_d)) return LGR_E_BADARG;
+  if (num_instances > 0 && (!inst_key_d || !inst_val_d || !inst_tmp_d || !sorted_ids_d || !splat_d || !radii_d)) return LGR_E_BADARG;
   if (const int rc6 = six_channels_check(view)) return rc6;
   if (view->want_aux && (!point_id_pixel_d || !point_weight_pixel_d || (n > 0 && !point_weight_d))) return LGR_E_BADARG;
   if (num_instances > 0x7fffffffLL) return LGR_E_UNSUPPORTED;
@@ -175,11 +175,11 @@
 int lgr_forward_render_device_sized(const lgr_view* view, int64_t n, int64_t instance_capacity, int32_t* meta_d,
                                     const float* splat_d, const int32_t* radii_d, int32_t* tile_start_d,
                                     int32_t* tile_cursor_d, uint32_t* inst_key_d, uint32_t* inst_val_d,
-                                    int32_t* sorted_ids_d, float* image_d, float* final_T_d, int32_t* n_contrib_d,
+                                    uint32_t* inst_tmp_d, int32_t* sorted_ids_d, float* image_d, float* final_T_d, int32_t* n_contrib_d,
                                     int32_t* point_id_pixel_d, float* point_weight_pixel_d, float* point_weight_d,
                                     int32_t* point_count_d, void* stream) {
   if (!view_ok(view) || n < 0 || instance_capacity <= 0 || !meta_d || !tile_start_d || !tile_cursor_d || !image_d || !final_T_d ||
-      !n_contrib_d || !inst_key_d || !inst_val_d || !sorted_ids_d)
+      !n_contrib_d || !inst_key_d || !inst_val_d || !inst_tmp_d || !sorted_ids_d)
     return LGR_E_BADARG;
   if (n > 0 && (!splat_d || !radii_d)) return LGR_E_BADARG;
   if (const int rc6 = six_channels_check(view)) return rc6;
@@ -188,7 +188,7 @@
   cudaStream_t st = (cudaStream_t)stream;
   const View v = make_view(view, n);
   int rc = launch_bin_and_sort(v, n, instance_capacity, 0, 0, splat_d, radii_d, tile_start_d, tile_cursor_d, inst_key_d, inst_val_d,
-                               nullptr, sorted_ids_d, meta_d, st);
+                               inst_tmp_d, sorted_ids_d, meta_d, st);
   if (rc) return rc;
   return launch_blend_fwd(v, tile_start_d, sorted_ids_d, splat_d, image_d, final_T_d, n_contrib_d, point_id_pixel_d,
                           point_weight_pixel_d, point_weight_d, view->want_aux ? point_count_d : nullptr, st);
@@ -426,7 +426,7 @@
   int rc = launch_shard_recv_count(v, make_layout(layout), exchange_d, dsplat_d, tile_cursor_d, meta_d, point_weight_rows_d,
                                    point_count_rows_d, st);
   if (rc) return rc;
-  return launch_tile_scan(ntiles, tile_start_d, tile_cursor_d, meta_d, view->tile_rank_d != nullptr, st);
+  return launch_tile_scan(ntiles, tile_start_d, tile_cursor_d, meta_d, false, st);
 }
 
 int lgr_blend_backward(const lgr_view* view, int64_t n, int64_t num_instances, const float* splat_d,
diff --git a/log_b200/csrc/lgr_common.cuh b/log_b200/csrc/lgr_common.cuh
--- a/log_b200/csrc/lgr_common.cuh
+++ b/log_b200/csrc/lgr_common.cuh
@@ -32,7 +32,6 @@
   int32_t* band_count;
   int32_t* band_rows;
   float* band_dsplat;
-  int32_t* tile_rank;
   const int64_t* gather;
   const int32_t* pid_map;
   int32_t* contrib_id;
@@ -56,7 +55,7 @@
 
 inline View make_view(const lgr_view* v, int64_t n = 0) {
   View o;
-  o.num_owners = v->num_owners; o.band_ids = v->band_ids_d; o.band_blk = v->band_blk_d; o.band_count = v->band_count_d; o.band_rows = v->band_rows_d; o.band_dsplat = v->band_dsplat_d; o.tile_rank = v->tile_rank_d; o.gather = v->gather_index_d; o.pid_map = v->pid_map_d; o.contrib_id = v->contrib_id_d; o.contrib_entry = v->contrib_entry_d; o.contrib_count = v->contrib_count_d; o.last_contrib = v->last_contrib_d;
+  o.num_owners = v->num_owners; o.band_ids = v->band_ids_d; o.band_blk = v->band_blk_d; o.band_count = v->band_count_d; o.band_rows = v->band_rows_d; o.band_dsplat = v->band_dsplat_d; o.gather = v->gather_index_d; o.pid_map = v->pid_map_d; o.contrib_id = v->contrib_id_d; o.contrib_entry = v->contrib_entry_d; o.contrib_count = v->contrib_count_d; o.last_contrib = v->last_contrib_d;
   o.region_count = v->region_count_d; o.region_cap = v->region_cap; o.regions = v->region_count_d ? v->num_regions : 0;
   o.cov3d = v->cov3D_precomp_d; o.dcov3d = v->dcov3D_d;
   o.owner_chunk = o.num_owners > 0 ? (int)LGR_OWNER_CHUNK(n, (int64_t)o.num_owners) : 256;
@@ -230,28 +229,17 @@
   return (int64_t)s * v.region_cap + (t - first[s]);
 }
 
-__device__ __forceinline__ bool count_small_tiles(const View& v, int32_t* __restrict__ tile_count, int64_t row, int x0, int y0, int x1,
+__device__ __forceinline__ bool count_small_tiles(const View& v, int32_t* __restrict__ tile_count, int x0, int y0, int x1,
                                                   int y1) {
   const int w = x1 - x0, cnt = w * (y1 - y0);
   if (cnt > 4) return true;
-  if (v.tile_rank == nullptr) {
-    for (int k = 0; k < cnt; k++) atomicAdd(tile_count + ((y0 + k / w - v.row0) * v.gx + x0 + k % w) * CSTRIDE, 1);
-    return false;
-  }
-  int r[4];
-#pragma unroll
-  for (int k = 0; k < 4; k++) {
-    r[k] = -1;
-    if (k < cnt) r[k] = atomicAdd(tile_count + ((y0 + k / max(w, 1) - v.row0) * v.gx + x0 + k % max(w, 1)) * CSTRIDE, 1);
-  }
-  *reinterpret_cast<int4*>(v.tile_rank + 4 * row) = make_int4(r[0], r[1], r[2], r[3]);
+  for (int k = 0; k < cnt; k++) atomicAdd(tile_count + ((y0 + k / w - v.row0) * v.gx + x0 + k % w) * CSTRIDE, 1);
   return false;
 }
 
 __device__ __forceinline__ void warp_count_big_tiles(const View& v, int32_t* __restrict__ tile_count, bool big, int x0, int y0, int x1,
                                                      int y1) {
   const int lane = threadIdx.x & 31;
-  const int slot = v.tile_rank ? 1 : 0;
   unsigned todo = __ballot_sync(0xffffffffu, big);
   while (todo) {
     const int src = __ffs(todo) - 1;
@@ -259,7 +247,7 @@
     const int bx0 = __shfl_sync(0xffffffffu, x0, src), by0 = __shfl_sync(0xffffffffu, y0, src);
     const int bx1 = __shfl_sync(0xffffffffu, x1, src), by1 = __shfl_sync(0xffffffffu, y1, src);
     const int w = bx1 - bx0, cnt = w * (by1 - by0);
-    for (int k = lane; k < cnt; k += 32) atomicAdd(tile_count + ((by0 + k / w - v.row0) * v.gx + bx0 + k % w) * CSTRIDE + slot, 1);
+    for (int k = lane; k < cnt; k += 32) atomicAdd(tile_count + ((by0 + k / w - v.row0) * v.gx + bx0 + k % w) * CSTRIDE, 1);
   }
 }
 
diff --git a/log_b200/csrc/lgr_project.cu b/log_b200/csrc/lgr_project.cu
--- a/log_b200/csrc/lgr_project.cu
+++ b/log_b200/csrc/lgr_project.cu
@@ -218,7 +218,7 @@
         if (DEPTH) r3 = make_float4(cv.t[2], p[2], 1.0f, 0.f);
         if (reach) {
           tile_rect_tight(px, py, rad, hx, hy, v.gx, v.gy, v.row0, v.row1, x0, y0, x1, y1);
-          big_splat = count_small_tiles(v, tile_count, i, x0, y0, x1, y1);
+          big_splat = count_small_tiles(v, tile_count, x0, y0, x1, y1);
           bx0 = x0; by0 = y0; bx1 = x1; by1 = y1;
         }
       }
diff --git a/log_b200/csrc/lgr_shard.cu b/log_b200/csrc/lgr_shard.cu
--- a/log_b200/csrc/lgr_shard.cu
+++ b/log_b200/csrc/lgr_shard.cu
@@ -160,7 +160,7 @@
       stock += (unsigned)((x1 - x0) * max(0, min(y1, v.row1) - max(y0, v.row0)));
       vis += 1;
       tile_rect_tight(r0.x, r0.y, rad, r1.z, r1.w, v.gx, v.gy, v.row0, v.row1, x0, y0, x1, y1);
-      big_splat = count_small_tiles(v, tile_count, slot, x0, y0, x1, y1);
+      big_splat = count_small_tiles(v, tile_count, x0, y0, x1, y1);
       bx0 = x0; by0 = y0; bx1 = x1; by1 = y1;
       float4* z = reinterpret_cast<float4*>(dsplat + slot * LGR_GRAD_FLOATS);
       z[0] = z[1] = z[2] = make_float4(0.f, 0.f, 0.f, 0.f);
diff --git a/log_b200/rasterizer.py b/log_b200/rasterizer.py
--- a/log_b200/rasterizer.py
+++ b/log_b200/rasterizer.py
@@ -8,7 +8,6 @@
 from ._capi import LGR_FILTER_ADD, LGR_FILTER_MAX, LGR_FILTER_NONE, LgrView
 
 PREZERO_DSPLAT = bool(int(__import__('os').environ.get('LGR_PREZERO_DSPLAT', '0')))
-RANKED_BIN = bool(int(__import__('os').environ.get('LGR_RANKED_BIN', '1')))
 CONTRIB_BITS = bool(int(__import__('os').environ.get('LGR_CONTRIB_BITS', '1')))
 FLAVOUR_STOCK = 'stock'
 FLAVOUR_FORK = 'fork'
@@ -55,7 +54,7 @@
 
 def _make_view(s: GaussianRasterizationSettings, filter_mode: int, want_aux: bool, sh_coeffs: int, tile_rows, keep,
                num_owners=0, band_ids=None, band_count=None, band_blk=None, band_rows=None, band_dsplat=None,
-               raw_params=False, tile_rank=None, gather_index=None, pid_map=None, cov3D_precomp=None, splat_ext=None,
+               raw_params=False, gather_index=None, pid_map=None, cov3D_precomp=None, splat_ext=None,
                log_depth=False):
     dev = s.viewmatrix.device
     vm, pm = _f32c(s.viewmatrix, 'viewmatrix'), _f32c(s.projmatrix, 'projmatrix', dev)
@@ -76,7 +75,6 @@
     v.band_blk_d = band_blk.data_ptr() if band_blk is not None else None
     v.band_rows_d = band_rows.data_ptr() if band_rows is not None else None
     v.band_dsplat_d = band_dsplat.data_ptr() if band_dsplat is not None else None
-    v.tile_rank_d = tile_rank.data_ptr() if tile_rank is not None else None
     v.gather_index_d = gather_index.data_ptr() if gather_index is not None else None
     v.pid_map_d = pid_map.data_ptr() if pid_map is not None else None
     v.cov3D_precomp_d = cov3D_precomp.data_ptr() if cov3D_precomp is not None else None
@@ -184,12 +182,10 @@
         band_ids = torch.empty((max(256 * nb, 1),), dtype=torch.int32, device=dev)
         band_blk = torch.empty((2 * nb + 1,), dtype=torch.int32, device=dev)
         band_count = torch.empty((num_owners,), dtype=torch.int32, device=dev)
-    tile_rank = torch.empty((max(n, 1), 4), dtype=torch.int32, device=dev) if RANKED_BIN else None
-    keep.append(tile_rank)
     splat_ext = torch.empty((max(n, 1), 4), dtype=torch.float32, device=dev) if channels == 6 else None
     keep.append(splat_ext)
     view = _make_view(settings, filter_mode, want_aux, K, tile_rows, keep, num_owners, band_ids, band_count, band_blk, band_rows, band_dsplat,
-                      raw_params, tile_rank, gather_index, cov3D_precomp=cov3D_precomp, splat_ext=splat_ext, log_depth=log_depth)
+                      raw_params, gather_index, cov3D_precomp=cov3D_precomp, splat_ext=splat_ext, log_depth=log_depth)
     H, W = view.image_height, view.image_width
     gx, gy = (W + 15) // 16, (H + 15) // 16
     rows = gy if tile_rows is None else int(tile_rows[1]) - int(tile_rows[0])
@@ -222,12 +218,13 @@
             raise _capi.LgrError('instance_capacity (device-sized call) is not available in band mode')
         D, max_len, num_long, stock_D, m = int(instance_capacity), None, None, None, None
         inst_key, inst_val = torch.empty((D,), **u32), torch.empty((D,), **u32)
+        inst_tmp = torch.empty((2 * D,), **u32)
         sorted_ids = torch.empty((D,), **i32)
         contrib = torch.empty((2 * D + ntiles,), **i32) if use_contrib_lists(D, None) else None
         keep.append(contrib)
         set_contrib_lists(view, contrib, D, n_contrib)
         _capi.check(lib.lgr_forward_render_device_sized(ctypes.byref(view), n, D, _ptr(meta), _ptr(splat), _ptr(radii), _ptr(tile_start),
-                                                        _ptr(tile_cursor), _ptr(inst_key), _ptr(inst_val), _ptr(sorted_ids), _ptr(image),
+                                                        _ptr(tile_cursor), _ptr(inst_key), _ptr(inst_val), _ptr(inst_tmp), _ptr(sorted_ids), _ptr(image),
                                                         _ptr(final_T), _ptr(n_contrib), _ptr(pid), _ptr(pwp), _ptr(pw), _ptr(pc), st),
                     'lgr_forward_render_device_sized')
     else:
@@ -239,7 +236,7 @@
                                  f'{m[4]} of {n} Gaussians visible, longest tile list {max_len}): more than 2^31 - 1 is unsupported')
         inst_key = torch.empty((D,), **u32)
         inst_val = torch.empty((D,), **u32)
-        inst_tmp = torch.empty((2 * D,), **u32) if max_len > lib.lgr_sort_smem_capacity() else None
+        inst_tmp = torch.empty((2 * D,), **u32)
         sorted_ids = torch.empty((D,), **i32)
         contrib = torch.empty((2 * D + ntiles,), **i32) if use_contrib_lists(D, max_len) else None
         keep.append(contrib)
diff --git a/log_b200/sharded.py b/log_b200/sharded.py
--- a/log_b200/sharded.py
+++ b/log_b200/sharded.py
@@ -232,9 +232,7 @@
         s.keep, s.n, s.want_aux, s.settings = [], n, bool(want_aux), settings
         K = 0 if sh is None else int(sh.shape[1])
         s.view_full = _make_view(settings, filter_mode, want_aux, K, None, s.keep, raw_params=raw_params)
-        from .rasterizer import RANKED_BIN
-        rank_rows = self._scratch('tile_rank', (self.world * self.cap, 4), torch.int32) if RANKED_BIN else None
-        s.view_band = _make_view(settings, filter_mode, want_aux, K, self.band, s.keep, raw_params=raw_params, tile_rank=rank_rows,
+        s.view_band = _make_view(settings, filter_mode, want_aux, K, self.band, s.keep, raw_params=raw_params,
                                  pid_map=self.recv_gid)
         s.view_band.region_count_d = self.buf.data_ptr() + 4 * int(self.layout.off_count)
         s.view_band.region_cap, s.view_band.num_regions = self.cap, self.world
@@ -293,12 +291,13 @@
             cap = self._inst_cap
             inst_key = self._scratch('inst_key', (cap,), torch.int32)
             inst_val = self._scratch('inst_val', (cap,), torch.int32)
+            inst_tmp = self._scratch('inst_tmp', (2 * cap,), torch.int32)
             s.sorted_ids = self._scratch('sorted_ids', (cap,), torch.int32)
             set_contrib_lists(v, self._scratch('contrib', (2 * cap + ntiles,), torch.int32) if use_contrib_lists(cap, None) else None,
                               cap, n_contrib)
             s.num_instances, s.max_tile_len, s.num_rows, s.stock_instances = cap, None, None, None
             _capi.check(lib.lgr_forward_render_device_sized(ctypes.byref(v), rows, cap, _ptr(meta), _ptr(self.recv_splat), _ptr(self.recv_radii),
-                                                            _ptr(s.tile_start), _ptr(cursor), _ptr(inst_key), _ptr(inst_val), _ptr(s.sorted_ids),
+                                                            _ptr(s.tile_start), _ptr(cursor), _ptr(inst_key), _ptr(inst_val), _ptr(inst_tmp), _ptr(s.sorted_ids),
                                                             _ptr(s.image), _ptr(final_T), _ptr(n_contrib), _ptr(pid), _ptr(pwp),
                                                             _ptr(s.pw_rows), _ptr(s.pc_rows), st), 'lgr_forward_render_device_sized')
             return s.image, s.radii, pid, pwp
@@ -311,7 +310,7 @@
             self._inst_cap = max(self._inst_cap, D + D // 4 + 4096)
         inst_key = self._scratch('inst_key', (D,), torch.int32)
         inst_val = self._scratch('inst_val', (D,), torch.int32)
-        inst_tmp = self._scratch('inst_tmp', (2 * D,), torch.int32) if max_len > lib.lgr_sort_smem_capacity() else None
+        inst_tmp = self._scratch('inst_tmp', (2 * D,), torch.int32)
         s.sorted_ids = self._scratch('sorted_ids', (D,), torch.int32)
         set_contrib_lists(v, self._scratch('contrib', (2 * D + ntiles,), torch.int32) if use_contrib_lists(D, max_len) else None,
                           D, n_contrib)
```

New measurement: 1.843 billion (median of 6 runs). 1.09x the previous value.
